# neka-nat/probreg

Hardware: NVIDIA H100
Metric: cpd_em_iterations_per_sec (higher is better)
Workload: dtype f32

## Files before the change

probreg_b200/csrc/cpd_b200.cu:

```cuda
#include "cpd_b200.h"
#include "kernels.cuh"
#include "lowrank.cuh"
#include "gram_i8.cuh"
#include "bcpd.cuh"

#include <cub/device/device_radix_sort.cuh>
#ifdef CPD_HOST_EMU
#include "emu_nccl.h"
#include "emu_solver.h"
#endif

#include <dlfcn.h>
#include <math.h>
#include <stdarg.h>
#include <stdio.h>
#include <stdlib.h>
#include <string.h>

#include <algorithm>
#include <vector>

using namespace cpd;

static thread_local char g_err[512] = "";
static int fail(int code, const char* fmt, ...) {
    va_list ap;
    va_start(ap, fmt);
    vsnprintf(g_err, sizeof(g_err), fmt, ap);
    va_end(ap);
    return code;
}
#define CU(call)                                                                                   \
    do {                                                                                           \
        cudaError_t e_ = (call);                                                                   \
        if (e_ != cudaSuccess)                                                                     \
            return fail(CPD_ERR_CUDA, "%s failed at %s:%d: %s", #call, __FILE__, __LINE__, cudaGetErrorString(e_)); \
    } while (0)
#define KCHECK() CU(cudaGetLastError())

extern "C" const char* cpd_last_error(void) { return g_err; }
extern "C" int cpd_version(void) { return 100; }
extern "C" int cpd_device_count(void) {
    int n = 0;
    if (cudaGetDeviceCount(&n) != cudaSuccess) { cudaGetLastError(); return 0; }
    return n;
}

namespace {
typedef struct { char internal[128]; } nccl_uid;
typedef void* nccl_comm;
struct NcclApi {
    void* lib = nullptr;
    int (*GetUniqueId)(nccl_uid*) = nullptr;
    int (*CommInitRank)(nccl_comm*, int, nccl_uid, int) = nullptr;
    int (*AllReduce)(const void*, void*, size_t, int, int, nccl_comm, cudaStream_t) = nullptr;
    int (*CommDestroy)(nccl_comm) = nullptr;
    const char* (*GetErrorString)(int) = nullptr;
};
NcclApi g_nccl;
int load_nccl() {
    if (g_nccl.lib) return CPD_OK;
#ifdef CPD_HOST_EMU
    static_assert(sizeof(nccl_uid) == sizeof(emu::nccl_uid_t), "unique id layout");
    g_nccl.GetUniqueId = reinterpret_cast<int (*)(nccl_uid*)>(emu::ncclGetUniqueId);
    g_nccl.CommInitRank = reinterpret_cast<int (*)(nccl_comm*, int, nccl_uid, int)>(emu::ncclCommInitRank);
    g_nccl.AllReduce = emu::ncclAllReduce;
    g_nccl.CommDestroy = emu::ncclCommDestroy;
    g_nccl.GetErrorString = emu::ncclGetErrorString;
    g_nccl.lib = (void*)&g_nccl;
    return CPD_OK;
#endif
    const char* names[] = {"libnccl.so.2", "libnccl.so"};
    void* lib = nullptr;
    for (const char* nm : names) { lib = dlopen(nm, RTLD_NOW | RTLD_GLOBAL); if (lib) break; }
    if (!lib) return fail(CPD_ERR_NCCL, "cannot dlopen libnccl.so.2: %s", dlerror());
    g_nccl.GetUniqueId = (int (*)(nccl_uid*))dlsym(lib, "ncclGetUniqueId");
    g_nccl.CommInitRank = (int (*)(nccl_comm*, int, nccl_uid, int))dlsym(lib, "ncclCommInitRank");
    g_nccl.AllReduce = (int (*)(const void*, void*, size_t, int, int, nccl_comm, cudaStream_t))dlsym(lib, "ncclAllReduce");
    g_nccl.CommDestroy = (int (*)(nccl_comm))dlsym(lib, "ncclCommDestroy");
    g_nccl.GetErrorString = (const char* (*)(int))dlsym(lib, "ncclGetErrorString");
    if (!g_nccl.GetUniqueId || !g_nccl.CommInitRank || !g_nccl.AllReduce || !g_nccl.CommDestroy)
        return fail(CPD_ERR_NCCL, "libnccl lacks an expected symbol");
    g_nccl.lib = lib;
    return CPD_OK;
}
constexpr int NCCL_DOUBLE = 8, NCCL_SUM = 0;

struct SolverApi {
    void* lib = nullptr;
    int (*Create)(void**) = nullptr;
    int (*Destroy)(void*) = nullptr;
    int (*SetStream)(void*, cudaStream_t) = nullptr;
    int (*CreateParams)(void**) = nullptr;
    int (*DestroyParams)(void*) = nullptr;
    int (*XgetrfBuf)(void*, void*, int64_t, int64_t, int, const void*, int64_t, int, size_t*, size_t*) = nullptr;
    int (*Xgetrf)(void*, void*, int64_t, int64_t, int, void*, int64_t, int64_t*, int, void*, size_t, void*, size_t, int*) = nullptr;
    int (*Xgetrs)(void*, void*, int, int64_t, int64_t, int, const void*, int64_t, const int64_t*, int, void*, int64_t, int*) = nullptr;
};
SolverApi g_sol;
int load_cusolver() {
    if (g_sol.lib) return CPD_OK;
#ifdef CPD_HOST_EMU
    g_sol.Create = emu::solverCreate; g_sol.Destroy = emu::solverDestroy; g_sol.SetStream = emu::solverSetStream;
    g_sol.CreateParams = emu::solverCreateParams; g_sol.DestroyParams = emu::solverDestroyParams;
    g_sol.XgetrfBuf = emu::solverXgetrfBuf; g_sol.Xgetrf = emu::solverXgetrf; g_sol.Xgetrs = emu::solverXgetrs;
    g_sol.lib = (void*)&g_sol;
    return CPD_OK;
#endif
    const char* names[] = {"libcusolver.so.11", "/usr/local/cuda/lib64/libcusolver.so.11", "libcusolver.so"};
    void* lib = nullptr;
    for (const char* nm : names) { lib = dlopen(nm, RTLD_NOW | RTLD_GLOBAL); if (lib) break; }
    if (!lib) return fail(CPD_ERR_CUDA, "cannot dlopen libcusolver.so.11: %s", dlerror());
#define SOLSYM(field, name) g_sol.field = (decltype(g_sol.field))dlsym(lib, name)
    SOLSYM(Create, "cusolverDnCreate");
    SOLSYM(Destroy, "cusolverDnDestroy");
    SOLSYM(SetStream, "cusolverDnSetStream");
    SOLSYM(CreateParams, "cusolverDnCreateParams");
    SOLSYM(DestroyParams, "cusolverDnDestroyParams");
    SOLSYM(XgetrfBuf, "cusolverDnXgetrf_bufferSize");
    SOLSYM(Xgetrf, "cusolverDnXgetrf");
    SOLSYM(Xgetrs, "cusolverDnXgetrs");
#undef SOLSYM
    if (!g_sol.Create || !g_sol.SetStream || !g_sol.CreateParams || !g_sol.XgetrfBuf || !g_sol.Xgetrf || !g_sol.Xgetrs)
        return fail(CPD_ERR_CUDA, "libcusolver lacks an expected symbol");
    g_sol.lib = lib;
    return CPD_OK;
}
constexpr int CUDA_R_64F_ = 1, CUBLAS_OP_T_ = 1;
}
#define SOLV(call)                                                                          \
    do {                                                                                    \
        int r_ = (call);                                                                    \
        if (r_ != 0) return fail(CPD_ERR_CUDA, "%s failed with cusolverStatus %d", #call, r_); \
    } while (0)
#define NC(call)                                                                                                   \
    do {                                                                                                           \
        int r_ = (call);                                                                                           \
        if (r_ != 0)                                                                                               \
            return fail(CPD_ERR_NCCL, "%s failed: %s", #call, g_nccl.GetErrorString ? g_nccl.GetErrorString(r_) : "?"); \
    } while (0)

struct cpd_ctx {
    int device = 0, dim = 3, sm_count = 132, slots1 = 264, slots2 = 264;
    cudaStream_t stream = nullptr;
    bool own_stream = false;
    long long m = 0, mpad = 0, n = 0, npad = 0, n_global = 0;
    double *d_yc = nullptr, *d_ts = nullptr, *d_xc = nullptr, *d_raw = nullptr;
    size_t raw_cap = 0;
    float4 *d_srcP = nullptr, *d_srcJ = nullptr, *d_tgtP = nullptr, *d_tgtQ = nullptr;
    P1Part* d_part1 = nullptr;
    double* d_part2 = nullptr;
    size_t part1_cap = 0, part2_cap = 0;
    double *d_pt1 = nullptr, *d_p1 = nullptr, *d_pxc = nullptr, *d_px = nullptr;
    double *d_mom_src = nullptr, *d_mom_tgt = nullptr, *d_mom = nullptr, *d_sums = nullptr;
    size_t mom_src_cap = 0, mom_tgt_cap = 0, sums_cap = 0;
    DevState* d_state = nullptr;
    DevState h_state;
    double* h_pin = nullptr;
    double* d_frame = nullptr;
    double* h_stats = nullptr;
    cudaEvent_t stats_ev = nullptr, copy_ev = nullptr;
    int stats_pending = 0;
    long long stats_count[2] = {0, 0};
    bool origin_given = false;
    int it1 = 0, it2 = 0, j1 = 1, j2 = 1, g1 = 1, g2 = 1;
    float4 *d_sbox = nullptr, *d_tbox = nullptr, *d_ssub = nullptr, *d_tsub = nullptr;
    float *d_omax = nullptr, *d_omax_sub = nullptr;
    bool cull_on = true, cull_active = false;
    double extent = 0.0;
    int4 *d_work1 = nullptr, *d_work2 = nullptr;
    int *d_slots1 = nullptr, *d_slots2 = nullptr;
    bool have_source = false, have_target = false, have_state = false, prepared = false;
    nccl_comm comm = nullptr;
    int world = 1, rank = 0;
    int *d_perm_src = nullptr, *d_perm_tgt = nullptr, *d_idx_tmp = nullptr;
    unsigned *d_codes = nullptr, *d_codes_out = nullptr;
    size_t sort_cap = 0, sort_tmp_cap = 0;
    void* d_sort_tmp = nullptr;
    double *d_outN = nullptr, *d_outM = nullptr;
    float* d_G = nullptr;
    double *d_W = nullptr, *d_A = nullptr, *d_B = nullptr, *d_ts2 = nullptr, *d_nrpart = nullptr;
    int64_t* d_ipiv = nullptr;
    int* d_info = nullptr;
    void *d_work = nullptr, *h_work = nullptr, *sol = nullptr, *sol_params = nullptr;
    size_t work_dev = 0, work_host = 0;
    long long nr_m = 0;
    double nr_lmd = 0.0;
    bool nr_ready = false;
    float* d_la = nullptr;
    double *d_la64 = nullptr, *d_la_part = nullptr, *d_bc_es = nullptr;
    size_t la_cap = 0;
    double* d_log2c = nullptr;
    bool wgt_on = false;
    BcpdState* d_bc = nullptr;
    float* d_bc_ginv = nullptr;
    double *d_bc_A = nullptr, *d_bc_S = nullptr, *d_bc_v = nullptr, *d_bc_r = nullptr, *d_bc_alpha = nullptr, *d_bc_sdiag = nullptr,
           *d_bc_part = nullptr, *d_bc_sums = nullptr;
    int64_t* d_bc_ipiv = nullptr;
    int* d_bc_info = nullptr;
    long long bc_m = 0;
    size_t bc_part_cap = 0;
    double bc_sigma2 = 0.0;
    bool bc_ready = false;
    bool bc_stopped = false;
    cudaEvent_t bc_ev[6] = {nullptr, nullptr, nullptr, nullptr, nullptr, nullptr};
    float bc_ms[5] = {0.f, 0.f, 0.f, 0.f, 0.f};
    double *d_wgt = nullptr, *d_p1t = nullptr, *d_pxt = nullptr;
    long long prior_m = 0;
    double prior_alpha = 1.0;
    bool prior_on = false;
    int lr_rank = 0;
    bool lr_w_stale = false;
    float lr_setup_ms[3] = {0.f, 0.f, 0.f};
    long long lr_m = 0;
    int lr_cap = 0;
    float4* d_lr_pts = nullptr;
    double *d_lr_Q = nullptr, *d_lr_X = nullptr, *d_lr_coef = nullptr, *d_lr_part = nullptr, *d_lr_Bc = nullptr, *d_lr_S = nullptr,
           *d_lr_R = nullptr, *d_lr_sys = nullptr, *d_lr_rhs = nullptr, *d_lr_c = nullptr, *d_lr_out = nullptr, *d_lr_panel = nullptr, *d_lr_Lt = nullptr;
    bool lr_spd = true;
    size_t lr_part_cap = 0;
    unsigned char* d_gi_planes = nullptr;
    double *d_gi_part = nullptr, *d_gi_colmax = nullptr;
    size_t gi_planes_cap = 0, gi_part_cap = 0, gi_colmax_cap = 0;
    size_t lr_out_cap = 0;
    P2PMailbox* d_box = nullptr;
    P2PInfo* d_p2p = nullptr;
    void* peer_ptr[P2P_MAX] = {nullptr};
    cudaEvent_t ev0 = nullptr, ev1 = nullptr, sev[7] = {nullptr, nullptr, nullptr, nullptr, nullptr, nullptr, nullptr};
    bool profiling = false;
    int64_t launches = 0;
    DevState* h_state_ring = nullptr;
    cudaEvent_t state_ev[8] = {nullptr, nullptr, nullptr, nullptr, nullptr, nullptr, nullptr, nullptr};
    int state_slot = 0;
    bool graph_on = true;
    cudaGraphExec_t em_graph = nullptr;
    int em_graph_key = -1, em_graph_launches = 0, prepare_gen = 0;
    void* d_flush = nullptr;
    size_t flush_cap = 0;
    std::vector<cudaEvent_t> pool;
};

namespace {
constexpr int STATE_RING = 8;
template <typename T>
int dev_alloc(T** p, size_t count) {
    if (*p) { cudaFree(*p); *p = nullptr; }
    cudaError_t e = cudaMalloc((void**)p, std::max<size_t>(count, 1) * sizeof(T));
    if (e != cudaSuccess) return fail(CPD_ERR_CUDA, "cudaMalloc(%zu bytes) failed: %s", count * sizeof(T), cudaGetErrorString(e));
    return CPD_OK;
}
#define TRY(x) do { int r__ = (x); if (r__ != CPD_OK) return r__; } while (0)
template <typename T>
struct DevBuf {
    T* p = nullptr;
    ~DevBuf() { if (p) cudaFree(p); }
    int alloc(size_t count) { return dev_alloc(&p, count); }
};

inline unsigned blocks_for(long long n) { return (unsigned)((n + THREADS - 1) / THREADS); }

struct WorkList {
    std::vector<int4> items;
    std::vector<int> tile_slots;
    int max_slots = 1;
};
WorkList build_work(int ntiles, int nunits, int slots, double last_cost, double overhead) {
    const double OVERHEAD = overhead;
    WorkList w;
    nunits = std::max(1, nunits);
    auto cost_of = [&](int t) { return t == ntiles - 1 ? last_cost : 1.0; };
    auto span_of = [&](int t, int j) { return cost_of(t) * (double)((nunits + j - 1) / j) + OVERHEAD; };
    int best_j = 1;
    double best = 1e300;
    for (int j = 1; j <= nunits; ++j) {
        const long long items = (long long)ntiles * j;
        const double waves = ceil((double)items / slots);
        const double span = waves * ((double)((nunits + j - 1) / j) + OVERHEAD);
        if (span < best - 1e-9) { best = span; best_j = j; }
        if (items > 8LL * slots) break;
    }
    w.tile_slots.assign(ntiles, best_j);
    if (ntiles <= slots) {
        std::vector<int> cuts(ntiles, 1);
        int used = ntiles;
        while (used < slots) {
            int worst = -1;
            double wv = -1.0;
            for (int t = 0; t < ntiles; ++t) {
                const double v = span_of(t, cuts[t]);
                if (cuts[t] < nunits && v > wv) { wv = v; worst = t; }
            }
            if (worst < 0) break;
            ++cuts[worst];
            ++used;
        }
        double span = 0.0;
        for (int t = 0; t < ntiles; ++t) span = std::max(span, span_of(t, cuts[t]));
        if (span <= best + 1e-9) w.tile_slots = cuts;
    }
    for (int t = 0; t < ntiles; ++t) {
        const int j = w.tile_slots[t];
        for (int s = 0; s < j; ++s) {
            const int a = (int)((long long)nunits * s / j), b = (int)((long long)nunits * (s + 1) / j);
            w.items.push_back(make_int4(t, a, b, s));
        }
        w.max_slots = std::max(w.max_slots, j);
    }
    std::stable_sort(w.items.begin(), w.items.end(), [&](const int4& a, const int4& b) {
        return cost_of(a.x) * (a.z - a.y) > cost_of(b.x) * (b.z - b.y);
    });
    return w;
}

int ensure_stats(cpd_ctx* h);
int upload_state(cpd_ctx* h) {
    TRY(ensure_stats(h));
    if (!h->h_state_ring) {
        CU(cudaMallocHost((void**)&h->h_state_ring, STATE_RING * sizeof(DevState)));
        for (int k = 0; k < STATE_RING; ++k) CU(cudaEventCreateWithFlags(&h->state_ev[k], cudaEventDisableTiming));
    }
    const int k = h->state_slot;
    h->state_slot = (k + 1) % STATE_RING;
    CU(cudaEventSynchronize(h->state_ev[k]));
    h->h_state_ring[k] = h->h_state;
    CU(cudaMemcpyAsync(h->d_state, &h->h_state_ring[k], sizeof(DevState), cudaMemcpyHostToDevice, h->stream));
    CU(cudaEventRecord(h->state_ev[k], h->stream));
    return CPD_OK;
}

int upload_cloud(cpd_ctx* h, const double* src, long long count, double* dst3) {
    if (h->dim == 3) {
        CU(cudaMemcpyAsync(dst3, src, (size_t)count * 3 * sizeof(double), cudaMemcpyHostToDevice, h->stream));
    } else {
        CU(cudaMemsetAsync(dst3, 0, (size_t)count * 3 * sizeof(double), h->stream));
        CU(cudaMemcpy2DAsync(dst3, 3 * sizeof(double), src, 2 * sizeof(double), 2 * sizeof(double), (size_t)count,
                             cudaMemcpyHostToDevice, h->stream));
    }
    return CPD_OK;
}
int download_cloud(cpd_ctx* h, const double* src3, long long count, double* dst) {
    if (h->dim == 3) {
        CU(cudaMemcpyAsync(dst, src3, (size_t)count * 3 * sizeof(double), cudaMemcpyDeviceToHost, h->stream));
    } else {
        CU(cudaMemcpy2DAsync(dst, 2 * sizeof(double), src3, 3 * sizeof(double), 2 * sizeof(double), (size_t)count,
                             cudaMemcpyDeviceToHost, h->stream));
    }
    return CPD_OK;
}

int cloud_sums_dev(cpd_ctx* h, const double* d_pts, long long count, double* part, double* d_out) {
    const unsigned nb = blocks_for(count);
    cloud_sums_kernel<<<nb, THREADS, 0, h->stream>>>(d_pts, count, part);
    reduce_cols_kernel<<<1, 4 * 32, 0, h->stream>>>(part, (int)nb, 4, d_out);
    KCHECK();
    h->launches += 2;
    return CPD_OK;
}

int ingest_cloud(cpd_ctx* h, const double* host_pts, long long count, int is_target, long long n_global, const double* origin,
                 int* d_perm, double* d_out) {
    if (h->raw_cap < (size_t)count * 3) { TRY(dev_alloc(&h->d_raw, (size_t)count * 3)); h->raw_cap = (size_t)count * 3; }
    const unsigned nb = blocks_for(count);
    if (h->sums_cap < (size_t)nb * 9 + 16) {
        TRY(dev_alloc(&h->d_sums, (size_t)nb * 9 + 16));
        h->sums_cap = (size_t)nb * 9 + 16;
    }
    if (h->sort_cap < (size_t)count) {
        TRY(dev_alloc(&h->d_codes, (size_t)count));
        TRY(dev_alloc(&h->d_codes_out, (size_t)count));
        TRY(dev_alloc(&h->d_idx_tmp, (size_t)count));
        h->sort_cap = (size_t)count;
    }
    size_t need = 0;
    CU(cub::DeviceRadixSort::SortPairs(nullptr, need, h->d_codes, h->d_codes_out, h->d_idx_tmp, d_perm, (int)count, 0, 30, h->stream));
    if (need > h->sort_tmp_cap) {
        if (h->d_sort_tmp) cudaFree(h->d_sort_tmp);
        h->d_sort_tmp = nullptr;
        CU(cudaMalloc(&h->d_sort_tmp, need));
        h->sort_tmp_cap = need;
    }
    TRY(upload_cloud(h, host_pts, count, h->d_raw));
    CU(cudaEventRecord(h->copy_ev, h->stream));
    double* frame = h->d_frame + 8 * is_target;
    stats_kernel<<<nb, THREADS, 0, h->stream>>>(h->d_raw, count, h->d_sums + 16);
    stats_fold_kernel<<<1, 288, 0, h->stream>>>(h->d_sums + 16, (int)nb, h->d_sums);
    cloud_frame_kernel<<<1, 32, 0, h->stream>>>(h->d_sums, count, is_target, n_global, origin != nullptr, origin ? origin[0] : 0.0,
                                                origin ? origin[1] : 0.0, origin ? origin[2] : 0.0, h->d_state, frame);
    CU(cudaMemcpyAsync(h->h_stats + 9 * is_target, h->d_sums, 9 * sizeof(double), cudaMemcpyDeviceToHost, h->stream));
    CU(cudaEventRecord(h->stats_ev, h->stream));
    h->stats_pending |= 1 << is_target;
    h->stats_count[is_target] = count;
    morton_frame_kernel<<<nb, THREADS, 0, h->stream>>>(h->d_raw, count, frame, h->d_codes, h->d_idx_tmp);
    CU(cub::DeviceRadixSort::SortPairs(h->d_sort_tmp, need, h->d_codes, h->d_codes_out, h->d_idx_tmp, d_perm, (int)count, 0, 30,
                                       h->stream));
    gather3_frame_kernel<<<nb, THREADS, 0, h->stream>>>(h->d_raw, d_perm, count, frame, d_out);
    KCHECK();
    h->launches += 6;
    CU(cudaEventSynchronize(h->copy_ev));
    return CPD_OK;
}

int ensure_stats(cpd_ctx* h) {
    if (!h->stats_pending) return CPD_OK;
    CU(cudaEventSynchronize(h->stats_ev));
    if (h->stats_pending & 1)
        for (int a = 0; a < 3; ++a) h->h_state.cy[a] = h->h_stats[a] / (double)h->stats_count[0];
    if (h->stats_pending & 2) {
        const double* t = h->h_stats + 9;
        if (!h->origin_given) for (int a = 0; a < 3; ++a) h->h_state.cx[a] = t[a] / (double)h->stats_count[1];
        h->extent = std::max(t[6] - t[3], std::max(t[7] - t[4], t[8] - t[5]));
    }
    h->stats_pending = 0;
    return CPD_OK;
}

int prepare(cpd_ctx* h) {
    TRY(ensure_stats(h));
    if (h->prepared) return CPD_OK;
    if (!h->have_source || !h->have_target) return fail(CPD_ERR_STATE, "source and target must both be set");
    h->it1 = (int)((h->n + ITILE1 - 1) / ITILE1);
    h->it2 = (int)((h->m + ITILE2 - 1) / ITILE2);
    const long long in_last = h->n - (long long)(h->it1 - 1) * ITILE1;
    const int live = (int)((in_last + 32 * RI1 - 1) / (32 * RI1));
    double last_cost = live < THREADS / 32 ? std::max(0.6, live / (double)(THREADS / 32)) : 1.0;
    if (const char* e = getenv("CPD_B200_PLAN_LAST_COST")) { const double v = atof(e); if (v > 0.0 && v <= 1.0) last_cost = v; }
    WorkList w1;
    if (const char* e = getenv("CPD_B200_PLAN_UNIT"); e && !strcmp(e, "stage")) {
        w1 = build_work(h->it1, (int)(h->mpad / P1_STAGE), h->slots1, last_cost, 0.5);
        for (int4& it : w1.items) { it.y *= P1_STAGE / SUB; it.z *= P1_STAGE / SUB; }
    } else {
        w1 = build_work(h->it1, (int)(h->mpad / SUB), h->slots1, last_cost, 0.5 * (P1_STAGE / SUB));
    }
    const WorkList w2 = build_work(h->it2, (int)(h->npad / P2_STAGE), h->slots2, 1.0, 0.5);
    h->j1 = w1.max_slots; h->g1 = (int)w1.items.size();
    h->j2 = w2.max_slots; h->g2 = (int)w2.items.size();
    TRY(dev_alloc(&h->d_work1, w1.items.size()));
    TRY(dev_alloc(&h->d_work2, w2.items.size()));
    TRY(dev_alloc(&h->d_slots1, w1.tile_slots.size()));
    TRY(dev_alloc(&h->d_slots2, w2.tile_slots.size()));
    CU(cudaMemcpyAsync(h->d_work1, w1.items.data(), w1.items.size() * sizeof(int4), cudaMemcpyHostToDevice, h->stream));
    CU(cudaMemcpyAsync(h->d_work2, w2.items.data(), w2.items.size() * sizeof(int4), cudaMemcpyHostToDevice, h->stream));
    CU(cudaMemcpyAsync(h->d_slots1, w1.tile_slots.data(), w1.tile_slots.size() * sizeof(int), cudaMemcpyHostToDevice, h->stream));
    CU(cudaMemcpyAsync(h->d_slots2, w2.tile_slots.data(), w2.tile_slots.size() * sizeof(int), cudaMemcpyHostToDevice, h->stream));
    CU(cudaStreamSynchronize(h->stream));
    TRY(dev_alloc(&h->d_sbox, (size_t)(h->mpad / P1_STAGE) * 2));
    TRY(dev_alloc(&h->d_tbox, (size_t)(h->npad / P2_STAGE) * 2));
    TRY(dev_alloc(&h->d_omax, (size_t)(h->npad / P2_STAGE)));
    TRY(dev_alloc(&h->d_ssub, (size_t)(h->mpad / SUB) * 2));
    TRY(dev_alloc(&h->d_tsub, (size_t)(h->npad / SUB) * 2));
    TRY(dev_alloc(&h->d_omax_sub, (size_t)(h->npad / SUB)));
    const size_t need1 = (size_t)h->j1 * h->n, need2 = (size_t)h->j2 * h->m * 4;
    if (need1 > h->part1_cap) { TRY(dev_alloc(&h->d_part1, need1)); h->part1_cap = need1; }
    if (need2 > h->part2_cap) { TRY(dev_alloc(&h->d_part2, need2)); h->part2_cap = need2; }
    const size_t ms = (size_t)blocks_for(h->m) * MOM_SRC, mt = (size_t)blocks_for(h->npad) * MOM_TGT;
    if (ms > h->mom_src_cap) { TRY(dev_alloc(&h->d_mom_src, ms)); h->mom_src_cap = ms; }
    if (mt > h->mom_tgt_cap) { TRY(dev_alloc(&h->d_mom_tgt, mt)); h->mom_tgt_cap = mt; }
    h->prepared = true;
    h->prepare_gen += 1;
    return CPD_OK;
}

int allreduce(cpd_ctx* h, double* buf, size_t count) {
    if (!h->comm) return CPD_OK;
    NC(g_nccl.AllReduce(buf, buf, count, NCCL_DOUBLE, NCCL_SUM, h->comm, h->stream));
    return CPD_OK;
}

inline void mark(cpd_ctx* h, int k) {
    if (h->profiling) cudaEventRecord(h->sev[k], h->stream);
}

int launch_estep(cpd_ctx* h, const double* d_sigma2, const double* d_w, const double* d_ts) {
    TRY(prepare(h));
    const long long cover = std::max(h->mpad, h->n);
    mark(h, 0);
    pack_kernel<<<blocks_for(cover), THREADS, 0, h->stream>>>(h->d_state, d_sigma2, h->d_yc, d_ts, h->d_xc, h->m, h->mpad,
                                                              h->n, h->d_srcP, h->d_srcJ, h->d_tgtP);
    mark(h, 1);
    const bool cull = h->cull_on && h->cull_active;
    const int nst1 = (int)(h->mpad / P1_STAGE);
    stage_bbox_kernel<<<(unsigned)nst1, THREADS, 0, h->stream>>>(h->d_srcP, (int)h->m, P1_STAGE, h->d_sbox);
    h->launches += 1;
    const int nsub1 = (int)(h->mpad / SUB), nsub2 = (int)(h->npad / SUB);
    if (cull) {
        stage_bbox_kernel<<<(unsigned)(h->npad / P2_STAGE), THREADS, 0, h->stream>>>(h->d_tgtP, (int)h->n, P2_STAGE, h->d_tbox);
        sub_bbox_kernel<<<(unsigned)((nsub1 + 7) / 8), THREADS, 0, h->stream>>>(h->d_srcP, (int)h->m, nsub1, h->d_ssub);
        sub_bbox_kernel<<<(unsigned)((nsub2 + 7) / 8), THREADS, 0, h->stream>>>(h->d_tgtP, (int)h->n, nsub2, h->d_tsub);
        h->launches += 3;
    }
    const bool wgt = h->wgt_on;
    if (wgt) {
        weight_patch_kernel<<<blocks_for(h->m), THREADS, 0, h->stream>>>(h->d_la, h->m, h->d_srcP, h->d_srcJ);
        h->launches += 1;
    }
#define CPD_PASS1(C, W) pass1_kernel<C, W><<<h->g1, THREADS, PASS1_SMEM, h->stream>>>(h->d_tgtP, (int)h->n, h->d_srcJ, h->d_work1, h->d_part1, h->d_sbox, nst1, (C) ? h->d_ssub : nullptr)
    if (cull) { if (wgt) CPD_PASS1(true, true); else CPD_PASS1(true, false); }
    else { if (wgt) CPD_PASS1(false, true); else CPD_PASS1(false, false); }
#undef CPD_PASS1
    mark(h, 2);
    finalize1_kernel<<<blocks_for(h->npad), THREADS, 0, h->stream>>>(h->d_state, d_sigma2, d_w, h->d_part1, h->d_slots1, (int)h->n,
                                                                     h->d_tgtP, h->d_tgtQ, h->npad, h->d_pt1, h->d_mom_tgt,
                                                                     wgt ? h->d_log2c : nullptr);
    mark(h, 3);
    if (cull) {
        stage_omax_kernel<<<(unsigned)(h->npad / P2_STAGE), THREADS, 0, h->stream>>>(h->d_tgtQ, h->d_omax);
        sub_omax_kernel<<<(unsigned)((nsub2 + 7) / 8), THREADS, 0, h->stream>>>(h->d_tgtQ, nsub2, h->d_omax_sub);
        h->launches += 2;
    }
#define CPD_PASS2(C, W) pass2_kernel<C, W><<<h->g2, THREADS, PASS2_SMEM, h->stream>>>(h->d_srcP, (int)h->m, h->d_tgtQ, h->d_work2, h->d_part2, (C) ? h->d_tbox : nullptr, (C) ? h->d_omax : nullptr, (C) ? h->d_tsub : nullptr, (C) ? h->d_omax_sub : nullptr)
    if (cull) { if (wgt) CPD_PASS2(true, true); else CPD_PASS2(true, false); }
    else { if (wgt) CPD_PASS2(false, true); else CPD_PASS2(false, false); }
#undef CPD_PASS2
    mark(h, 4);
    finalize2_kernel<<<blocks_for(h->m), THREADS, 0, h->stream>>>(h->d_state, d_sigma2, h->d_part2, h->d_slots2, (int)h->m, h->d_yc,
                                                                  d_ts, h->d_p1, h->d_pxc, h->d_mom_src);
    mark(h, 5);
    mark(h, 6);
    KCHECK();
    h->launches += 5;
    return CPD_OK;
}

int read_params(cpd_ctx* h, cpd_params* out) {
    static_assert(sizeof(DevState) <= 48 * sizeof(double), "DevState outgrew the pinned staging buffer");
    CU(cudaMemcpyAsync(h->h_pin, h->d_state, sizeof(DevState), cudaMemcpyDeviceToHost, h->stream));
    CU(cudaStreamSynchronize(h->stream));
    if (reinterpret_cast<const DevState*>(h->h_pin)->err)
        return fail(CPD_ERR_STATE, "a peer rank did not deliver its moments within the P2P exchange timeout");
    const int d = h->dim;
    for (int i = 0; i < 9; ++i) out->lin[i] = 0.0;
    for (int i = 0; i < d; ++i)
        for (int j = 0; j < d; ++j) out->lin[i * d + j] = h->h_pin[3 * i + j];
    for (int i = 0; i < 3; ++i) out->t[i] = (i < d) ? h->h_pin[9 + i] : 0.0;
    out->scale = h->h_pin[12];
    out->sigma2 = h->h_pin[13];
    TRY(ensure_stats(h));
    h->cull_active = h->extent > 0.0 && 13.3 * sqrt(out->sigma2) < 0.25 * h->extent;
    out->q = h->h_pin[14];
    out->n_p = h->h_pin[15];
    return CPD_OK;
}
}

extern "C" int cpd_plan_work(int ntiles, int nunits, int slots, double last_tile_cost, int* items ,
                             int capacity, int* n_items, int* max_slots) {
    if (ntiles < 1 || nunits < 1 || slots < 1 || !(last_tile_cost > 0.0 && last_tile_cost <= 1.0) || !n_items || !max_slots)
        return fail(CPD_ERR_ARG, "bad argument");
    const WorkList w = build_work(ntiles, nunits, slots, last_tile_cost, 0.5 * (P1_STAGE / SUB));
    *n_items = (int)w.items.size();
    *max_slots = w.max_slots;
    if (items) {
        if (capacity < (int)w.items.size()) return fail(CPD_ERR_ARG, "capacity %d < %d work items", capacity, (int)w.items.size());
        for (size_t i = 0; i < w.items.size(); ++i) {
            items[4 * i] = w.items[i].x; items[4 * i + 1] = w.items[i].y; items[4 * i + 2] = w.items[i].z; items[4 * i + 3] = w.items[i].w;
        }
    }
    return CPD_OK;
}

extern "C" int cpd_create(cpd_ctx** out, int device, int dim, void* stream) {
    if (!out) return fail(CPD_ERR_ARG, "out is NULL");
    if (dim != 2 && dim != 3) return fail(CPD_ERR_ARG, "dim must be 2 or 3, got %d", dim);
    int ndev = 0;
    if (cudaGetDeviceCount(&ndev) != cudaSuccess || ndev == 0) {
        cudaGetLastError();
        return fail(CPD_ERR_CUDA, "no CUDA device: this library has no CPU path");
    }
    if (device < 0 || device >= ndev) return fail(CPD_ERR_ARG, "device %d out of range (%d visible)", device, ndev);
    CU(cudaSetDevice(device));
    cudaDeviceProp prop;
    CU(cudaGetDeviceProperties(&prop, device));
    if (prop.major != 9 || prop.minor != 0)
        return fail(CPD_ERR_CUDA, "device %d is sm_%d%d; this library is built for sm_90a (Hopper) only", device, prop.major, prop.minor);
    cpd_ctx* h = new cpd_ctx();
    h->device = device;
    h->dim = dim;
    h->sm_count = prop.multiProcessorCount;
    if (stream) { h->stream = (cudaStream_t)stream; h->own_stream = false; }
    else { CU(cudaStreamCreateWithFlags(&h->stream, cudaStreamNonBlocking)); h->own_stream = true; }
    CU(cudaFuncSetAttribute(pass1_kernel<false, false>, cudaFuncAttributeMaxDynamicSharedMemorySize, PASS1_SMEM));
    CU(cudaFuncSetAttribute(pass2_kernel<false, false>, cudaFuncAttributeMaxDynamicSharedMemorySize, PASS2_SMEM));
    CU(cudaFuncSetAttribute(pass1_kernel<true, false>, cudaFuncAttributeMaxDynamicSharedMemorySize, PASS1_SMEM));
    CU(cudaFuncSetAttribute(pass2_kernel<true, false>, cudaFuncAttributeMaxDynamicSharedMemorySize, PASS2_SMEM));
    CU(cudaFuncSetAttribute(pass1_kernel<false, true>, cudaFuncAttributeMaxDynamicSharedMemorySize, PASS1_SMEM));
    CU(cudaFuncSetAttribute(pass2_kernel<false, true>, cudaFuncAttributeMaxDynamicSharedMemorySize, PASS2_SMEM));
    CU(cudaFuncSetAttribute(pass1_kernel<true, true>, cudaFuncAttributeMaxDynamicSharedMemorySize, PASS1_SMEM));
    CU(cudaFuncSetAttribute(pass2_kernel<true, true>, cudaFuncAttributeMaxDynamicSharedMemorySize, PASS2_SMEM));
    int occ1 = 0, occ2 = 0;
    CU(cudaOccupancyMaxActiveBlocksPerMultiprocessor(&occ1, pass1_kernel<false, false>, THREADS, PASS1_SMEM));
    CU(cudaOccupancyMaxActiveBlocksPerMultiprocessor(&occ2, pass2_kernel<false, false>, THREADS, PASS2_SMEM));
    h->slots1 = h->sm_count * std::max(1, occ1);
    h->slots2 = h->sm_count * std::max(1, occ2);
    TRY(dev_alloc(&h->d_state, 1));
    TRY(dev_alloc(&h->d_mom, (size_t)MOM_PAD));
    CU(cudaMallocHost((void**)&h->h_pin, 64 * sizeof(double)));
    TRY(dev_alloc(&h->d_frame, 16));
    CU(cudaMallocHost((void**)&h->h_stats, 18 * sizeof(double)));
    CU(cudaEventCreateWithFlags(&h->stats_ev, cudaEventDisableTiming));
    CU(cudaEventCreateWithFlags(&h->copy_ev, cudaEventDisableTiming));
    CU(cudaEventCreate(&h->ev0));
    CU(cudaEventCreate(&h->ev1));
    for (int k = 0; k < 7; ++k) CU(cudaEventCreate(&h->sev[k]));
    { const char* e = getenv("CPD_B200_NO_CULL"); h->cull_on = !(e && e[0] == '1'); }
    { const char* e = getenv("CPD_B200_NO_GRAPH"); h->graph_on = !(e && e[0] == '1'); }
    memset(&h->h_state, 0, sizeof(DevState));
    h->h_state.dim = dim;
    h->h_state.scale = 1.0;
    h->h_state.lin[0] = h->h_state.lin[4] = h->h_state.lin[8] = 1.0;
    h->h_state.update_scale = 1;
    *out = h;
    return upload_state(h);
}

extern "C" void cpd_destroy(cpd_ctx* h) {
    if (!h) return;
    cudaSetDevice(h->device);
    cudaStreamSynchronize(h->stream);
    void* wl[] = {h->d_work1, h->d_work2, h->d_slots1, h->d_slots2, h->d_sbox, h->d_tbox, h->d_omax, h->d_ssub, h->d_tsub, h->d_omax_sub};
    for (void* p : wl) if (p) cudaFree(p);
    void* srt[] = {h->d_perm_src, h->d_perm_tgt, h->d_idx_tmp, h->d_codes, h->d_codes_out, h->d_sort_tmp, h->d_outN, h->d_outM};
    for (void* p : srt) if (p) cudaFree(p);
    void* nrp[] = {h->d_G, h->d_W, h->d_A, h->d_B, h->d_ts2, h->d_nrpart, h->d_ipiv, h->d_info, h->d_work};
    for (void* p : nrp) if (p) cudaFree(p);
    void* lrp[] = {h->d_lr_pts, h->d_lr_Q, h->d_lr_X, h->d_lr_coef, h->d_lr_part, h->d_lr_Bc, h->d_lr_S, h->d_lr_R, h->d_lr_sys, h->d_lr_rhs,
                   h->d_lr_c, h->d_lr_out, h->d_lr_panel, h->d_lr_Lt, h->d_gi_planes, h->d_gi_part, h->d_gi_colmax, h->d_wgt, h->d_p1t, h->d_pxt, h->d_la, h->d_log2c,
                   h->d_la64, h->d_la_part, h->d_bc_es};
    for (void* p : lrp) if (p) cudaFree(p);
    void* bcp[] = {h->d_bc, h->d_bc_ginv, h->d_bc_A, h->d_bc_S, h->d_bc_v, h->d_bc_r, h->d_bc_alpha, h->d_bc_sdiag, h->d_bc_part, h->d_bc_sums,
                   h->d_bc_ipiv, h->d_bc_info};
    for (void* p : bcp) if (p) cudaFree(p);
    for (cudaEvent_t e : h->bc_ev) if (e) cudaEventDestroy(e);
    if (h->h_work) free(h->h_work);
    if (h->sol_params && g_sol.DestroyParams) g_sol.DestroyParams(h->sol_params);
    if (h->sol && g_sol.Destroy) g_sol.Destroy(h->sol);
    for (int r = 0; r < P2P_MAX; ++r) if (h->peer_ptr[r]) cudaIpcCloseMemHandle(h->peer_ptr[r]);
    if (h->d_box) cudaFree(h->d_box);
    if (h->d_p2p) cudaFree(h->d_p2p);
    void* ptrs[] = {h->d_yc, h->d_ts, h->d_xc, h->d_raw, h->d_srcP, h->d_srcJ, h->d_tgtP, h->d_tgtQ, h->d_part1, h->d_part2, h->d_pt1, h->d_p1,
                    h->d_pxc, h->d_px, h->d_mom_src, h->d_mom_tgt, h->d_mom, h->d_sums, h->d_state, h->d_flush};
    for (void* p : ptrs) if (p) cudaFree(p);
    if (h->h_pin) cudaFreeHost(h->h_pin);
    if (h->h_stats) cudaFreeHost(h->h_stats);
    if (h->d_frame) cudaFree(h->d_frame);
    if (h->stats_ev) cudaEventDestroy(h->stats_ev);
    if (h->copy_ev) cudaEventDestroy(h->copy_ev);
#ifndef CPD_HOST_EMU
    if (h->em_graph) cudaGraphExecDestroy(h->em_graph);
#endif
    if (h->h_state_ring) cudaFreeHost(h->h_state_ring);
    for (int k = 0; k < 8; ++k) if (h->state_ev[k]) cudaEventDestroy(h->state_ev[k]);
    if (h->ev0) cudaEventDestroy(h->ev0);
    if (h->ev1) cudaEventDestroy(h->ev1);
    for (int k = 0; k < 7; ++k) if (h->sev[k]) cudaEventDestroy(h->sev[k]);
    for (cudaEvent_t e : h->pool) if (e) cudaEventDestroy(e);
    if (h->own_stream) cudaStreamDestroy(h->stream);
    delete h;
}

extern "C" int cpd_set_source(cpd_ctx* h, const double* source, int64_t m) {
    if (!h || !source) return fail(CPD_ERR_ARG, "null argument");
    if (m < 1 || m > 0x7fffffffLL - 65536) return fail(CPD_ERR_ARG, "source count %lld out of range", (long long)m);
    CU(cudaSetDevice(h->device));
    if (m != h->m || !h->d_yc) {
        h->m = m;
        h->mpad = (m + P1_STAGE - 1) / P1_STAGE * P1_STAGE;
        TRY(dev_alloc(&h->d_yc, (size_t)m * 3));
        TRY(dev_alloc(&h->d_ts, (size_t)m * 3));
        TRY(dev_alloc(&h->d_srcP, (size_t)h->mpad));
        TRY(dev_alloc(&h->d_srcJ, (size_t)h->mpad * 2));
        TRY(dev_alloc(&h->d_p1, (size_t)m));
        TRY(dev_alloc(&h->d_pxc, (size_t)m * 3));
        TRY(dev_alloc(&h->d_px, (size_t)m * 3));
        TRY(dev_alloc(&h->d_perm_src, (size_t)m));
        TRY(dev_alloc(&h->d_outM, (size_t)m * 3));
        h->prepared = false;
        h->nr_ready = false;
    }
    TRY(ingest_cloud(h, source, m, 0, 0, nullptr, h->d_perm_src, h->d_yc));
    h->bc_ready = false;
    h->bc_stopped = false;
    h->h_state.m = m;
    h->have_source = true;
    return CPD_OK;
}

extern "C" int cpd_set_target(cpd_ctx* h, const double* target, int64_t n_local, int64_t n_global, const double* frame_origin) {
    if (!h || !target) return fail(CPD_ERR_ARG, "null argument");
    if (n_local < 1 || n_local > 0x7fffffffLL - 65536) return fail(CPD_ERR_ARG, "target count %lld out of range", (long long)n_local);
    if (n_global < n_local) return fail(CPD_ERR_ARG, "n_global (%lld) < n_local (%lld)", (long long)n_global, (long long)n_local);
    if (!frame_origin && n_global != n_local) return fail(CPD_ERR_ARG, "a sharded target needs an explicit frame_origin");
    CU(cudaSetDevice(h->device));
    if (n_local != h->n || !h->d_xc) {
        h->n = n_local;
        h->npad = (n_local + P2_STAGE - 1) / P2_STAGE * P2_STAGE;
        TRY(dev_alloc(&h->d_xc, (size_t)n_local * 3));
        TRY(dev_alloc(&h->d_tgtP, (size_t)n_local));
        TRY(dev_alloc(&h->d_tgtQ, (size_t)h->npad * 3));
        TRY(dev_alloc(&h->d_pt1, (size_t)n_local));
        TRY(dev_alloc(&h->d_perm_tgt, (size_t)n_local));
        TRY(dev_alloc(&h->d_outN, (size_t)n_local));
        h->prepared = false;
    }
    h->n_global = n_global;
    double origin[3] = {0.0, 0.0, 0.0};
    if (frame_origin) for (int a = 0; a < h->dim; ++a) origin[a] = frame_origin[a];
    h->origin_given = frame_origin != nullptr;
    if (h->origin_given) for (int a = 0; a < 3; ++a) h->h_state.cx[a] = origin[a];
    TRY(ingest_cloud(h, target, n_local, 1, n_global, frame_origin ? origin : nullptr, h->d_perm_tgt, h->d_xc));
    h->h_state.n_global = n_global;
    h->have_target = true;
    return CPD_OK;
}

extern "C" int cpd_sigma2_init(cpd_ctx* h, double* sigma2) {
    if (!h || !sigma2) return fail(CPD_ERR_ARG, "null argument");
    if (!h->have_source || !h->have_target) return fail(CPD_ERR_STATE, "source and target must both be set");
    CU(cudaSetDevice(h->device));
    double sx[4], sy[4];
    const size_t pn = (size_t)blocks_for(h->n) * 4, pm = (size_t)blocks_for(h->m) * 4;
    if (h->sums_cap < 16 + pn + pm) { TRY(dev_alloc(&h->d_sums, 16 + pn + pm)); h->sums_cap = 16 + pn + pm; }
    TRY(cloud_sums_dev(h, h->d_xc, h->n, h->d_sums + 16, h->d_sums));
    if (h->comm) TRY(allreduce(h, h->d_sums, 4));
    TRY(cloud_sums_dev(h, h->d_yc, h->m, h->d_sums + 16 + pn, h->d_sums + 4));
    CU(cudaMemcpyAsync(h->h_pin, h->d_sums, 8 * sizeof(double), cudaMemcpyDeviceToHost, h->stream));
    CU(cudaStreamSynchronize(h->stream));
    TRY(ensure_stats(h));
    for (int k = 0; k < 4; ++k) { sx[k] = h->h_pin[k]; sy[k] = h->h_pin[4 + k]; }
    double dlt[3], d2 = 0.0, dsy = 0.0;
    for (int a = 0; a < 3; ++a) { dlt[a] = h->h_state.cy[a] - h->h_state.cx[a]; d2 += dlt[a] * dlt[a]; dsy += dlt[a] * sy[1 + a]; }
    const double M = (double)h->m, N = (double)h->n_global;
    const double syy = sy[0] + 2.0 * dsy + M * d2;
    double cross = 0.0;
    for (int a = 0; a < 3; ++a) cross += sx[1 + a] * (sy[1 + a] + M * dlt[a]);
    *sigma2 = (M * sx[0] + N * syy - 2.0 * cross) / (M * N * h->dim);
    return CPD_OK;
}

extern "C" int cpd_set_state(cpd_ctx* h, int tf_kind, int update_scale, double w, const cpd_params* init) {
    if (!h || !init) return fail(CPD_ERR_ARG, "null argument");
    if (tf_kind != CPD_TF_RIGID && tf_kind != CPD_TF_AFFINE) return fail(CPD_ERR_ARG, "tf_kind %d not supported by the fused EM loop", tf_kind);
    if (!(w >= 0.0 && w < 1.0)) return fail(CPD_ERR_ARG, "w must be in [0, 1), got %g", w);
    if (!(init->sigma2 > 0.0)) return fail(CPD_ERR_ARG, "sigma2 must be positive, got %g", init->sigma2);
    CU(cudaSetDevice(h->device));
    DevState& s = h->h_state;
    const int d = h->dim;
    for (int i = 0; i < 3; ++i)
        for (int j = 0; j < 3; ++j) s.lin[3 * i + j] = (i < d && j < d) ? init->lin[i * d + j] : (i == j ? 1.0 : 0.0);
    for (int i = 0; i < 3; ++i) s.t[i] = (i < d) ? init->t[i] : 0.0;
    s.scale = (tf_kind == CPD_TF_RIGID) ? init->scale : 1.0;
    s.sigma2 = init->sigma2;
    s.q = init->q;
    s.n_p = 0.0;
    s.w = w;
    s.tf_kind = tf_kind;
    s.update_scale = update_scale ? 1 : 0;
    s.dim = d;
    TRY(ensure_stats(h));
    h->cull_active = h->extent > 0.0 && 13.3 * sqrt(init->sigma2) < 0.25 * h->extent;
    h->have_state = true;
    return upload_state(h);
}

namespace {
int em_step_launches(cpd_ctx* h) {
    TRY(launch_estep(h, &h->d_state->sigma2, &h->d_state->w, nullptr));
    const int nbs = (int)blocks_for(h->m), nbt = (int)blocks_for(h->npad);
    if (h->d_p2p) {
        moments_p2p_kernel<<<1, 256, 0, h->stream>>>(h->d_state, h->d_mom_src, nbs, RM_SRC, h->d_mom_tgt, nbt, RM_TGT, h->d_mom,
                                                     h->d_p2p);
        h->launches += 1;
    } else if (h->comm) {
        moments_kernel<0><<<1, 256, 0, h->stream>>>(h->d_state, h->d_mom_src, nbs, RM_SRC, h->d_mom_tgt, nbt, RM_TGT, h->d_mom);
        TRY(allreduce(h, h->d_mom, MOM_PAD));
        mstep_residual_kernel<<<1, 32, 0, h->stream>>>(h->d_state, h->d_mom);
        h->launches += 2;
    } else {
        moments_kernel<1><<<1, 256, 0, h->stream>>>(h->d_state, h->d_mom_src, nbs, RM_SRC, h->d_mom_tgt, nbt, RM_TGT, h->d_mom);
        h->launches += 1;
    }
    mark(h, 6);
    KCHECK();
    return CPD_OK;
}
}

extern "C" int cpd_em_step(cpd_ctx* h, cpd_params* out) {
    if (!h) return fail(CPD_ERR_ARG, "null handle");
    if (!h->have_state) return fail(CPD_ERR_STATE, "cpd_set_state has not been called");
    CU(cudaSetDevice(h->device));
#ifndef CPD_HOST_EMU
    const bool use_graph = h->graph_on && !h->profiling && !(h->comm && !h->d_p2p) && !h->wgt_on;
#else
    const bool use_graph = false;
#endif
    if (!use_graph) {
        TRY(em_step_launches(h));
    }
#ifndef CPD_HOST_EMU
    else {
        TRY(prepare(h));
        const int key = h->prepare_gen * 2 + ((h->cull_on && h->cull_active) ? 1 : 0);
        if (!h->em_graph || h->em_graph_key != key) {
            if (h->em_graph) { cudaGraphExecDestroy(h->em_graph); h->em_graph = nullptr; }
            const int64_t before = h->launches;
            cudaGraph_t g = nullptr;
            CU(cudaStreamBeginCapture(h->stream, cudaStreamCaptureModeThreadLocal));
            const int rc = em_step_launches(h);
            const cudaError_t ce = cudaStreamEndCapture(h->stream, &g);
            h->em_graph_launches = (int)(h->launches - before);
            h->launches = before;
            if (rc != CPD_OK) { if (g) cudaGraphDestroy(g); return rc; }
            if (ce != cudaSuccess) return fail(CPD_ERR_CUDA, "cudaStreamEndCapture failed: %s", cudaGetErrorString(ce));
            const cudaError_t ie = cudaGraphInstantiate(&h->em_graph, g, 0);
            cudaGraphDestroy(g);
            if (ie != cudaSuccess) { h->em_graph = nullptr; return fail(CPD_ERR_CUDA, "cudaGraphInstantiate failed: %s", cudaGetErrorString(ie)); }
            h->em_graph_key = key;
        }
        CU(cudaGraphLaunch(h->em_graph, h->stream));
        h->launches += h->em_graph_launches;
    }
#endif
    if (out) return read_params(h, out);
    return CPD_OK;
}

extern "C" int cpd_em_run(cpd_ctx* h, int maxiter, double tol, cpd_params* out, int* iters_run, double* trace) {
    if (!h || !out) return fail(CPD_ERR_ARG, "null argument");
    if (!h->have_state) return fail(CPD_ERR_STATE, "cpd_set_state has not been called");
    double q = h->h_state.q;
    int it = 0;
    cpd_params cur;
    memset(&cur, 0, sizeof(cur));
    for (it = 0; it < maxiter; ++it) {
        TRY(cpd_em_step(h, &cur));
        if (trace) { trace[2 * it] = cur.sigma2; trace[2 * it + 1] = cur.q; }
        if (fabs(cur.q - q) < tol) { ++it; break; }
        q = cur.q;
    }
    if (maxiter <= 0) TRY(read_params(h, &cur));
    *out = cur;
    if (iters_run) *iters_run = it;
    return CPD_OK;
}

extern "C" int cpd_estep(cpd_ctx* h, const double* t_source, double sigma2, double w, double* pt1, double* p1, double* px, double* n_p) {
    if (!h || !t_source) return fail(CPD_ERR_ARG, "null argument");
    if (!(sigma2 > 0.0)) return fail(CPD_ERR_ARG, "sigma2 must be positive, got %g", sigma2);
    if (!(w >= 0.0 && w < 1.0)) return fail(CPD_ERR_ARG, "w must be in [0, 1), got %g", w);
    if (!h->have_source || !h->have_target) return fail(CPD_ERR_STATE, "source and target must both be set");
    CU(cudaSetDevice(h->device));
    if (h->raw_cap < (size_t)h->m * 3) { TRY(dev_alloc(&h->d_raw, (size_t)h->m * 3)); h->raw_cap = (size_t)h->m * 3; }
    TRY(upload_cloud(h, t_source, h->m, h->d_raw));
    gather3_kernel<<<blocks_for(h->m), THREADS, 0, h->stream>>>(h->d_raw, h->d_perm_src, h->m, 0.0, 0.0, 0.0, h->d_ts);
    h->launches += 1;
    TRY(ensure_stats(h));
    h->cull_active = h->extent > 0.0 && 13.3 * sqrt(sigma2) < 0.25 * h->extent;
    h->h_pin[32] = sigma2;
    h->h_pin[33] = w;
    CU(cudaMemcpyAsync(&h->d_state->es_sigma2, h->h_pin + 32, 2 * sizeof(double), cudaMemcpyHostToDevice, h->stream));
    TRY(launch_estep(h, &h->d_state->es_sigma2, &h->d_state->es_w, h->d_ts));
    if (h->comm) {
        TRY(allreduce(h, h->d_p1, (size_t)h->m));
        TRY(allreduce(h, h->d_pxc, (size_t)h->m * 3));
    }
    return cpd_last_estep(h, pt1, p1, px, n_p);
}

namespace {
int bcpd_weights(cpd_ctx* h, const double* alpha, const double* sdiag, const int* perm, const double* ssw) {
    const long long m = h->m;
    const unsigned nb = blocks_for(m);
    bcpd_la_kernel<<<nb, THREADS, 0, h->stream>>>(alpha, sdiag, m, ssw, h->dim, h->d_la64, h->d_la_part);
    bcpd_la_finish_kernel<<<1, 32, 0, h->stream>>>(h->d_la_part, (int)nb, ssw, h->dim, h->n_global, h->d_log2c);
    bcpd_la_apply_kernel<<<nb, THREADS, 0, h->stream>>>(h->d_la64, perm, m, h->d_log2c, h->d_la);
    KCHECK();
    h->launches += 3;
    return CPD_OK;
}
int ensure_weight_buffers(cpd_ctx* h) {
    const long long m = h->m;
    if (h->la_cap < (size_t)m) {
        TRY(dev_alloc(&h->d_la, (size_t)m));
        TRY(dev_alloc(&h->d_la64, (size_t)m));
        TRY(dev_alloc(&h->d_la_part, (size_t)blocks_for(m)));
        h->la_cap = (size_t)m;
    }
    if (!h->d_log2c) TRY(dev_alloc(&h->d_log2c, 3));
    if (!h->d_bc_es) TRY(dev_alloc(&h->d_bc_es, 3));
    return CPD_OK;
}
}

extern "C" int cpd_bcpd_estep(cpd_ctx* h, const double* t_source, double scale, const double* alpha, const double* sigma_diag,
                              double sigma2, double w, double* nu_d, double* nu, double* px, double* n_p) {
    if (!h || !t_source || !alpha || !sigma_diag) return fail(CPD_ERR_ARG, "null argument");
    if (!(sigma2 > 0.0)) return fail(CPD_ERR_ARG, "sigma2 must be positive, got %g", sigma2);
    if (!(w >= 0.0 && w < 1.0)) return fail(CPD_ERR_ARG, "w must be in [0, 1), got %g", w);
    if (!h->have_source || !h->have_target) return fail(CPD_ERR_STATE, "source and target must both be set");
    CU(cudaSetDevice(h->device));
    const long long m = h->m;
    bool any_weight = false;
    for (long long i = 0; i < m; ++i) {
        if (!(alpha[i] >= 0.0) || !(sigma_diag[i] >= 0.0)) return fail(CPD_ERR_ARG, "alpha and diag(sigma_mat) must be non-negative");
        any_weight = any_weight || (alpha[i] > 0.0 && sigma_diag[i] < INFINITY);
    }
    if (!any_weight) return fail(CPD_ERR_ARG, "every source has zero weight");
    TRY(ensure_weight_buffers(h));
    h->h_pin[44] = scale;
    h->h_pin[45] = sigma2;
    h->h_pin[46] = w;
    CU(cudaMemcpyAsync(h->d_bc_es, h->h_pin + 44, 3 * sizeof(double), cudaMemcpyHostToDevice, h->stream));
    CU(cudaMemcpyAsync(h->d_outM, alpha, (size_t)m * sizeof(double), cudaMemcpyHostToDevice, h->stream));
    CU(cudaMemcpyAsync(h->d_outM + m, sigma_diag, (size_t)m * sizeof(double), cudaMemcpyHostToDevice, h->stream));
    TRY(bcpd_weights(h, h->d_outM, h->d_outM + m, h->d_perm_src, h->d_bc_es));
    if (h->raw_cap < (size_t)m * 3) { TRY(dev_alloc(&h->d_raw, (size_t)m * 3)); h->raw_cap = (size_t)m * 3; }
    TRY(upload_cloud(h, t_source, m, h->d_raw));
    gather3_kernel<<<blocks_for(m), THREADS, 0, h->stream>>>(h->d_raw, h->d_perm_src, m, 0.0, 0.0, 0.0, h->d_ts);
    h->launches += 1;
    TRY(ensure_stats(h));
    h->cull_active = h->extent > 0.0 && 13.3 * sqrt(sigma2) < 0.25 * h->extent;
    h->h_pin[32] = sigma2;
    h->h_pin[33] = w;
    CU(cudaMemcpyAsync(&h->d_state->es_sigma2, h->h_pin + 32, 2 * sizeof(double), cudaMemcpyHostToDevice, h->stream));
    h->wgt_on = true;
    const int r = launch_estep(h, &h->d_state->es_sigma2, &h->d_state->es_w, h->d_ts);
    h->wgt_on = false;
    TRY(r);
    if (h->comm) {
        TRY(allreduce(h, h->d_p1, (size_t)m));
        TRY(allreduce(h, h->d_pxc, (size_t)m * 3));
    }
    return cpd_last_estep(h, nu_d, nu, px, n_p);
}

extern "C" int cpd_last_estep(cpd_ctx* h, double* pt1, double* p1, double* px, double* n_p) {
    if (!h) return fail(CPD_ERR_ARG, "null handle");
    if (!h->prepared) return fail(CPD_ERR_STATE, "no E-step has run on this handle");
    CU(cudaSetDevice(h->device));
    if (pt1) {
        scatter_kernel<<<blocks_for(h->n), THREADS, 0, h->stream>>>(h->d_pt1, h->d_perm_tgt, h->n, 1, h->d_outN);
        CU(cudaMemcpyAsync(pt1, h->d_outN, (size_t)h->n * sizeof(double), cudaMemcpyDeviceToHost, h->stream));
        h->launches += 1;
    }
    if (p1) {
        scatter_kernel<<<blocks_for(h->m), THREADS, 0, h->stream>>>(h->d_p1, h->d_perm_src, h->m, 1, h->d_outM);
        CU(cudaMemcpyAsync(p1, h->d_outM, (size_t)h->m * sizeof(double), cudaMemcpyDeviceToHost, h->stream));
        CU(cudaStreamSynchronize(h->stream));
        h->launches += 1;
    }
    if (px) {
        uncentre_px_kernel<<<blocks_for(h->m), THREADS, 0, h->stream>>>(h->d_state, h->d_p1, h->d_pxc, (int)h->m, h->d_px);
        scatter_kernel<<<blocks_for(h->m), THREADS, 0, h->stream>>>(h->d_px, h->d_perm_src, h->m, 3, h->d_outM);
        KCHECK();
        h->launches += 2;
        TRY(download_cloud(h, h->d_outM, h->m, px));
    }
    if (n_p) {
        const unsigned nb = blocks_for(h->m);
        if (h->sums_cap < (size_t)nb * 4 + 4) { TRY(dev_alloc(&h->d_sums, (size_t)nb * 4 + 4)); h->sums_cap = (size_t)nb * 4 + 4; }
        src_moments_api_kernel<<<nb, THREADS, 0, h->stream>>>((int)h->m, h->d_yc, h->d_p1, h->d_pxc, h->d_mom_src);
        reduce_cols_kernel<<<1, MOM_SRC * 32, 0, h->stream>>>(h->d_mom_src, (int)nb, MOM_SRC, h->d_mom);
        KCHECK();
        h->launches += 2;
        CU(cudaMemcpyAsync(h->h_pin + 40, h->d_mom, sizeof(double), cudaMemcpyDeviceToHost, h->stream));
    }
    CU(cudaStreamSynchronize(h->stream));
    if (n_p) *n_p = h->h_pin[40];
    return CPD_OK;
}

extern "C" int cpd_mstep(cpd_ctx* h, int tf_kind, int update_scale, const double* pt1, const double* p1, const double* px, double n_p,
                         cpd_params* out) {
    (void)n_p;
    if (!h || !pt1 || !p1 || !px || !out) return fail(CPD_ERR_ARG, "null argument");
    if (tf_kind != CPD_TF_RIGID && tf_kind != CPD_TF_AFFINE) return fail(CPD_ERR_ARG, "tf_kind %d not supported", tf_kind);
    if (!h->have_source || !h->have_target) return fail(CPD_ERR_STATE, "source and target must both be set");
    CU(cudaSetDevice(h->device));
    TRY(prepare(h));
    h->h_state.tf_kind = tf_kind;
    h->h_state.update_scale = update_scale ? 1 : 0;
    CU(cudaMemcpyAsync(&h->d_state->tf_kind, &h->h_state.tf_kind, 2 * sizeof(int), cudaMemcpyHostToDevice, h->stream));
    CU(cudaMemcpyAsync(h->d_outN, pt1, (size_t)h->n * sizeof(double), cudaMemcpyHostToDevice, h->stream));
    gather1_kernel<<<blocks_for(h->n), THREADS, 0, h->stream>>>(h->d_outN, h->d_perm_tgt, h->n, h->d_pt1);
    CU(cudaMemcpyAsync(h->d_outM, p1, (size_t)h->m * sizeof(double), cudaMemcpyHostToDevice, h->stream));
    gather1_kernel<<<blocks_for(h->m), THREADS, 0, h->stream>>>(h->d_outM, h->d_perm_src, h->m, h->d_p1);
    if (h->raw_cap < (size_t)h->m * 3) { TRY(dev_alloc(&h->d_raw, (size_t)h->m * 3)); h->raw_cap = (size_t)h->m * 3; }
    TRY(upload_cloud(h, px, h->m, h->d_raw));
    gather3_kernel<<<blocks_for(h->m), THREADS, 0, h->stream>>>(h->d_raw, h->d_perm_src, h->m, 0.0, 0.0, 0.0, h->d_px);
    h->launches += 3;
    const int nbs = (int)blocks_for(h->m), nbt = (int)blocks_for(h->n);
    centre_px_kernel<<<nbs, THREADS, 0, h->stream>>>(h->d_state, h->d_p1, h->d_px, (int)h->m, h->d_pxc);
    src_moments_api_kernel<<<nbs, THREADS, 0, h->stream>>>((int)h->m, h->d_yc, h->d_p1, h->d_pxc, h->d_mom_src);
    tgt_moments_api_kernel<<<nbt, THREADS, 0, h->stream>>>(h->d_pt1, h->d_xc, (int)h->n, h->d_mom_tgt);
    moments_kernel<0><<<1, 256, 0, h->stream>>>(h->d_state, h->d_mom_src, nbs, MOM_SRC, h->d_mom_tgt, nbt, MOM_TGT, h->d_mom);
    KCHECK();
    if (h->comm) TRY(allreduce(h, h->d_mom + MOM_SRC, MOM_TGT));
    mstep_api_kernel<<<1, 32, 0, h->stream>>>(h->d_state, h->d_mom);
    KCHECK();
    h->launches += 5;
    return read_params(h, out);
}

#include "host_nonrigid.inl"
#include "host_bcpd.inl"
#include "host_stateless.inl"
#include "host_multi.inl"
#include "host_measure.inl"
```

probreg_b200/csrc/kernels.cuh:

```cuda
#pragma once
#include <cuda_runtime.h>
#include <stdint.h>

namespace cpd {

#ifndef CPD_RI1
#define CPD_RI1 4
#endif
#ifndef CPD_RI2
#define CPD_RI2 4
#endif
#ifndef CPD_MINB1
#define CPD_MINB1 2
#endif
#ifndef CPD_MINB2
#define CPD_MINB2 2
#endif
#ifndef CPD_UNROLL1
#define CPD_UNROLL1 4
#endif
#ifndef CPD_UNROLL2
#define CPD_UNROLL2 4
#endif
#ifndef CPD_SUB
#define CPD_SUB 64
#endif
#ifndef CPD_GRP
#define CPD_GRP 8
#endif
constexpr int UNROLL1 = CPD_UNROLL1, UNROLL2 = CPD_UNROLL2;
constexpr int THREADS = 256;
constexpr int RI1 = CPD_RI1, RI2 = CPD_RI2;
constexpr int ITILE1 = THREADS * RI1, ITILE2 = THREADS * RI2;
constexpr int NPAIR1 = RI1 / 2, NPAIR2 = RI2 / 2;
#ifndef CPD_P1_STAGE
#define CPD_P1_STAGE 512
#endif
#ifndef CPD_P2_STAGE
#define CPD_P2_STAGE 512
#endif
constexpr int P1_STAGE = CPD_P1_STAGE;
constexpr int P2_STAGE = CPD_P2_STAGE;
static_assert(P1_STAGE % 256 == 0 && P2_STAGE % 256 == 0 && P1_STAGE >= 256 && P2_STAGE >= 256, "stage sizes are multiples of 256");
constexpr int P1_REC = 32, P2_REC = 48;
#ifndef CPD_NSTAGE
#define CPD_NSTAGE 3
#endif
constexpr int NSTAGE = CPD_NSTAGE;
constexpr int P1_STAGE_BYTES = P1_STAGE * P1_REC, P2_STAGE_BYTES = P2_STAGE * P2_REC;
constexpr int SUB = CPD_SUB;
constexpr int GRP = CPD_GRP;
constexpr int PASS1_SMEM = NSTAGE * P1_STAGE_BYTES + 64, PASS2_SMEM = NSTAGE * P2_STAGE_BYTES + 64;

#ifdef CPD_HOST_EMU
#define CPD_DYN_SMEM(name) unsigned char* const name = emu::g_dyn_smem
#else
#define CPD_DYN_SMEM(name) extern __shared__ __align__(128) unsigned char name[]
#endif

constexpr float O_INIT = 1048576.0f;
constexpr float TWO100 = 1.2676506002282294e30f;
constexpr float FAR_COORD = 1.0e18f;

constexpr double LOG2E = 1.4426950408889634074;
constexpr double DEAD_LOG2 = -1075.0;
constexpr double EPS32 = 1.1920928955078125e-07;

enum { RM_NP = 0, RM_SY = 1, RM_C = 4, RM_V1 = 10, RM_VY = 13, RM_SRC = 22, RM_SRR = 22, RM_NPT = 23, RM_TGT = 2,
       RM_COUNT = 24, MOM_PAD = 32 };
enum { MOM_NP = 0, MOM_SX = 1, MOM_SY = 4, MOM_B = 7, MOM_C = 16, MOM_NPT = 22, MOM_SXT = 23, MOM_TXX = 26,
       MOM_COUNT = 27, MOM_SRC = 22, MOM_TGT = 5 };

struct P1Part {
    double S;
    double SU;
    float o;
    float pad;
};

struct DevState {
    double lin[9];
    double t[3];
    double scale;
    double sigma2;
    double q;
    double n_p;
    double cx[3];
    double cy[3];
    double w;
    double es_sigma2;
    double es_w;
    long long m;
    long long n_global;
    int tf_kind;
    int update_scale;
    int dim;
    int err;
};

constexpr int P2P_MAX = 16;
struct P2PMailbox {
    double slots[2][P2P_MAX][MOM_PAD];
    unsigned long long flags[2][P2P_MAX];
};
struct P2PInfo {
    P2PMailbox* box[P2P_MAX];
    int world, rank;
    unsigned long long seq;
    unsigned long long timeout_ns;
};

#ifdef CPD_HOST_EMU
}
#include "emu_device.h"
namespace cpd {
#else
__device__ __forceinline__ float ex2(float x) {
    float y;
    asm("ex2.approx.ftz.f32 %0, %1;" : "=f"(y) : "f"(x));
    return y;
}
typedef unsigned long long u64;
__device__ __forceinline__ u64 pack2(float lo, float hi) { u64 r; asm("mov.b64 %0, {%1, %2};" : "=l"(r) : "f"(lo), "f"(hi)); return r; }
__device__ __forceinline__ float2 unpack2(u64 v) { float2 r; asm("mov.b64 {%0, %1}, %2;" : "=f"(r.x), "=f"(r.y) : "l"(v)); return r; }
__device__ __forceinline__ u64 fsub2(u64 a, u64 b) {
    const float2 x = unpack2(a), y = unpack2(b);
    return pack2(__fsub_rn(x.x, y.x), __fsub_rn(x.y, y.y));
}
__device__ __forceinline__ u64 fadd2(u64 a, u64 b) {
    const float2 x = unpack2(a), y = unpack2(b);
    return pack2(__fadd_rn(x.x, y.x), __fadd_rn(x.y, y.y));
}
__device__ __forceinline__ u64 fmul2(u64 a, u64 b) {
    const float2 x = unpack2(a), y = unpack2(b);
    return pack2(__fmul_rn(x.x, y.x), __fmul_rn(x.y, y.y));
}
__device__ __forceinline__ u64 ffma2(u64 a, u64 b, u64 c) {
    const float2 x = unpack2(a), y = unpack2(b), z = unpack2(c);
    return pack2(__fmaf_rn(x.x, y.x, z.x), __fmaf_rn(x.y, y.y, z.y));
}
__device__ __forceinline__ unsigned long long globaltimer_ns() {
    unsigned long long t;
    asm volatile("mov.u64 %0, %%globaltimer;" : "=l"(t));
    return t;
}
__device__ __forceinline__ uint32_t smem_u32(const void* p) { return (uint32_t)__cvta_generic_to_shared(p); }
__device__ __forceinline__ void mbar_init(uint64_t* bar, uint32_t count) {
    asm volatile("mbarrier.init.shared::cta.b64 [%0], %1;" ::"r"(smem_u32(bar)), "r"(count));
}
__device__ __forceinline__ void mbar_fence_init() { asm volatile("fence.mbarrier_init.release.cluster;" ::: "memory"); }
__device__ __forceinline__ void mbar_expect_tx(uint64_t* bar, uint32_t bytes) {
    asm volatile("mbarrier.arrive.expect_tx.shared::cta.b64 _, [%0], %1;" ::"r"(smem_u32(bar)), "r"(bytes) : "memory");
}
__device__ __forceinline__ void tma_load_1d(void* dst, const void* src, uint32_t bytes, uint64_t* bar) {
    asm volatile("cp.async.bulk.shared::cluster.global.mbarrier::complete_tx::bytes [%0], [%1], %2, [%3];" ::"r"(
                     smem_u32(dst)),
                 "l"(src), "r"(bytes), "r"(smem_u32(bar))
                 : "memory");
}
__device__ __forceinline__ void mbar_wait(uint64_t* bar, uint32_t parity) {
    asm volatile(
        "{\n"
        ".reg .pred P1;\n"
        "LAB_WAIT:\n"
        "mbarrier.try_wait.parity.shared::cta.b64 P1, [%0], %1;\n"
        "@P1 bra DONE;\n"
        "bra LAB_WAIT;\n"
        "DONE:\n"
        "}" ::"r"(smem_u32(bar)),
        "r"(parity)
        : "memory");
}
#endif
__device__ __forceinline__ double warp_sum(double v) {
#pragma unroll
    for (int o = 16; o > 0; o >>= 1) v += __shfl_xor_sync(0xffffffffu, v, o);
    return v;
}
template <int K>
__device__ __forceinline__ void block_reduce_store(double (&v)[K], double* out) {
    __shared__ double sh[K][THREADS / 32];
    const int lane = threadIdx.x & 31, wid = threadIdx.x >> 5;
#pragma unroll
    for (int k = 0; k < K; ++k) {
        double s = warp_sum(v[k]);
        if (lane == 0) sh[k][wid] = s;
    }
    __syncthreads();
    if (threadIdx.x < K) {
        double s = 0.0;
#pragma unroll
        for (int w = 0; w < THREADS / 32; ++w) s += sh[threadIdx.x][w];
        out[threadIdx.x] = s;
    }
}

__global__ void __launch_bounds__(THREADS)
pack_kernel(const DevState* __restrict__ st, const double* __restrict__ sigma2_ptr,
            const double* __restrict__ yc , const double* __restrict__ ts ,
            const double* __restrict__ xc , long long m, long long mpad, long long n,
            float4* __restrict__ srcP , float4* __restrict__ srcJ ,
            float4* __restrict__ tgtP ) {
    const long long i = (long long)blockIdx.x * THREADS + threadIdx.x;
    const double sk = sqrt(LOG2E / (2.0 * *sigma2_ptr));
    if (i < mpad) {
        float4 o;
        if (i < m) {
            double px, py, pz;
            if (ts != nullptr) {
                px = ts[3 * i + 0] - st->cx[0];
                py = ts[3 * i + 1] - st->cx[1];
                pz = ts[3 * i + 2] - st->cx[2];
            } else {
                const double s = (st->tf_kind == 0) ? st->scale : 1.0;
                double l[9], tp[3];
#pragma unroll
                for (int k = 0; k < 9; ++k) l[k] = s * st->lin[k];
#pragma unroll
                for (int a = 0; a < 3; ++a)
                    tp[a] = l[3 * a] * st->cy[0] + l[3 * a + 1] * st->cy[1] + l[3 * a + 2] * st->cy[2] + st->t[a] - st->cx[a];
                const double y0 = yc[3 * i], y1 = yc[3 * i + 1], y2 = yc[3 * i + 2];
                px = l[0] * y0 + l[1] * y1 + l[2] * y2 + tp[0];
                py = l[3] * y0 + l[4] * y1 + l[5] * y2 + tp[1];
                pz = l[6] * y0 + l[7] * y1 + l[8] * y2 + tp[2];
            }
            o = make_float4((float)(sk * px), (float)(sk * py), (float)(sk * pz), 0.0f);
        } else {
            o = make_float4(FAR_COORD, FAR_COORD, FAR_COORD, 0.0f);
        }
        srcP[i] = o;
        srcJ[2 * i] = make_float4(o.x, o.x, o.y, o.y);
        srcJ[2 * i + 1] = make_float4(o.z, o.z, 0.0f, 0.0f);
    }
    if (i < n) {
        tgtP[i] = make_float4((float)(sk * xc[3 * i]), (float)(sk * xc[3 * i + 1]), (float)(sk * xc[3 * i + 2]), 0.0f);
    }
}

__global__ void __launch_bounds__(THREADS)
weight_patch_kernel(const float* __restrict__ la, long long m, float4* __restrict__ srcP, float4* __restrict__ srcJ) {
    const long long i = (long long)blockIdx.x * THREADS + threadIdx.x;
    if (i < m) {
        const float v = la[i];
        srcP[i].w = v;
        float4 r = srcJ[2 * i + 1];
        r.z = v; r.w = v;
        srcJ[2 * i + 1] = r;
    }
}

constexpr float CULL_GAP = 130.0f;
__global__ void __launch_bounds__(THREADS)
stage_bbox_kernel(const float4* __restrict__ pts, int n, int blk, float4* __restrict__ box) {
    __shared__ float sh[6][THREADS / 32];
    const int b = blockIdx.x;
    float lo[3] = {3.0e38f, 3.0e38f, 3.0e38f}, hi[3] = {-3.0e38f, -3.0e38f, -3.0e38f};
    for (int i = b * blk + threadIdx.x; i < min(n, (b + 1) * blk); i += THREADS) {
        const float4 p = pts[i];
        lo[0] = fminf(lo[0], p.x); lo[1] = fminf(lo[1], p.y); lo[2] = fminf(lo[2], p.z);
        hi[0] = fmaxf(hi[0], p.x); hi[1] = fmaxf(hi[1], p.y); hi[2] = fmaxf(hi[2], p.z);
    }
    const int lane = threadIdx.x & 31, wid = threadIdx.x >> 5;
#pragma unroll
    for (int a = 0; a < 3; ++a) {
#pragma unroll
        for (int o = 16; o > 0; o >>= 1) {
            lo[a] = fminf(lo[a], __shfl_xor_sync(0xffffffffu, lo[a], o));
            hi[a] = fmaxf(hi[a], __shfl_xor_sync(0xffffffffu, hi[a], o));
        }
        if (lane == 0) { sh[a][wid] = lo[a]; sh[3 + a][wid] = hi[a]; }
    }
    __syncthreads();
    if (threadIdx.x == 0) {
        float l[3], h[3];
        for (int a = 0; a < 3; ++a) {
            l[a] = sh[a][0]; h[a] = sh[3 + a][0];
            for (int w = 1; w < THREADS / 32; ++w) { l[a] = fminf(l[a], sh[a][w]); h[a] = fmaxf(h[a], sh[3 + a][w]); }
        }
        box[2 * b] = make_float4(l[0], l[1], l[2], 0.f);
        box[2 * b + 1] = make_float4(h[0], h[1], h[2], 0.f);
    }
}
__global__ void __launch_bounds__(THREADS)
stage_omax_kernel(const float4* __restrict__ tgtQ, float* __restrict__ omax) {
    __shared__ float sh[THREADS / 32];
    const int b = blockIdx.x;
    float m = 3.0e38f;
    for (int i = threadIdx.x; i < P2_STAGE; i += THREADS) m = fminf(m, tgtQ[3 * ((size_t)b * P2_STAGE + i) + 1].z);
#pragma unroll
    for (int o = 16; o > 0; o >>= 1) m = fminf(m, __shfl_xor_sync(0xffffffffu, m, o));
    if ((threadIdx.x & 31) == 0) sh[threadIdx.x >> 5] = m;
    __syncthreads();
    if (threadIdx.x == 0) {
        for (int w = 1; w < THREADS / 32; ++w) m = fminf(m, sh[w]);
        omax[b] = -m;
    }
}
__global__ void __launch_bounds__(THREADS)
sub_bbox_kernel(const float4* __restrict__ pts, int n, int nsub, float4* __restrict__ box) {
    const int b = blockIdx.x * (THREADS / 32) + (threadIdx.x >> 5), lane = threadIdx.x & 31;
    if (b >= nsub) return;
    float lo[3] = {3.0e38f, 3.0e38f, 3.0e38f}, hi[3] = {-3.0e38f, -3.0e38f, -3.0e38f};
    for (int i = b * SUB + lane; i < min(n, (b + 1) * SUB); i += 32) {
        const float4 p = pts[i];
        lo[0] = fminf(lo[0], p.x); lo[1] = fminf(lo[1], p.y); lo[2] = fminf(lo[2], p.z);
        hi[0] = fmaxf(hi[0], p.x); hi[1] = fmaxf(hi[1], p.y); hi[2] = fmaxf(hi[2], p.z);
    }
#pragma unroll
    for (int a = 0; a < 3; ++a) {
#pragma unroll
        for (int o = 16; o > 0; o >>= 1) {
            lo[a] = fminf(lo[a], __shfl_xor_sync(0xffffffffu, lo[a], o));
            hi[a] = fmaxf(hi[a], __shfl_xor_sync(0xffffffffu, hi[a], o));
        }
    }
    if (lane == 0) {
        box[2 * b] = make_float4(lo[0], lo[1], lo[2], 0.f);
        box[2 * b + 1] = make_float4(hi[0], hi[1], hi[2], 0.f);
    }
}
__global__ void __launch_bounds__(THREADS)
sub_omax_kernel(const float4* __restrict__ tgtQ, int nsub, float* __restrict__ omax) {
    const int b = blockIdx.x * (THREADS / 32) + (threadIdx.x >> 5), lane = threadIdx.x & 31;
    if (b >= nsub) return;
    float m = 3.0e38f;
    for (int i = lane; i < SUB; i += 32) m = fminf(m, tgtQ[3 * ((size_t)b * SUB + i) + 1].z);
#pragma unroll
    for (int o = 16; o > 0; o >>= 1) m = fminf(m, __shfl_xor_sync(0xffffffffu, m, o));
    if (lane == 0) omax[b] = -m;
}
template <int NP>
__device__ __forceinline__ void warp_bbox(const u64 (&ax)[NP], const u64 (&ay)[NP], const u64 (&az)[NP], float* __restrict__ wbox) {
    float lo[3] = {3.0e38f, 3.0e38f, 3.0e38f}, hi[3] = {-3.0e38f, -3.0e38f, -3.0e38f};
#pragma unroll
    for (int p = 0; p < NP; ++p) {
        const float2 x = unpack2(ax[p]), y = unpack2(ay[p]), z = unpack2(az[p]);
        lo[0] = fminf(lo[0], fminf(x.x, x.y)); hi[0] = fmaxf(hi[0], fmaxf(x.x, x.y));
        lo[1] = fminf(lo[1], fminf(y.x, y.y)); hi[1] = fmaxf(hi[1], fmaxf(y.x, y.y));
        lo[2] = fminf(lo[2], fminf(z.x, z.y)); hi[2] = fmaxf(hi[2], fmaxf(z.x, z.y));
    }
#pragma unroll
    for (int a = 0; a < 3; ++a) {
#pragma unroll
        for (int o = 16; o > 0; o >>= 1) {
            lo[a] = fminf(lo[a], __shfl_xor_sync(0xffffffffu, lo[a], o));
            hi[a] = fmaxf(hi[a], __shfl_xor_sync(0xffffffffu, hi[a], o));
        }
    }
    if ((threadIdx.x & 31) == 0) {
#pragma unroll
        for (int a = 0; a < 3; ++a) { wbox[a] = lo[a]; wbox[3 + a] = hi[a]; }
    }
    __syncwarp();
}
__device__ __forceinline__ float box_gap2(const float* __restrict__ wbox, const float4 blo, const float4 bhi) {
    const float gx = fmaxf(0.f, fmaxf(blo.x - wbox[3], wbox[0] - bhi.x));
    const float gy = fmaxf(0.f, fmaxf(blo.y - wbox[4], wbox[1] - bhi.y));
    const float gz = fmaxf(0.f, fmaxf(blo.z - wbox[5], wbox[2] - bhi.z));
    return fmaf(gz, gz, fmaf(gy, gy, gx * gx)) * 0.9999f;
}

template <bool WGT>
__device__ __forceinline__ void pass1_sum(const ulonglong2* __restrict__ q, const u64 (&ax)[NPAIR1], const u64 (&ay)[NPAIR1],
                                          const u64 (&az)[NPAIR1], const u64 (&no)[NPAIR1], u64 (&Sc)[NPAIR1], u64 (&Uc)[NPAIR1]) {
    if (GRP > 0) {
#pragma unroll 1
        for (int g0 = 0; g0 < SUB; g0 += (GRP > 0 ? GRP : SUB)) {
            u64 gs[NPAIR1], gu[NPAIR1];
#pragma unroll
            for (int jj = 0; jj < (GRP > 0 ? GRP : 1); ++jj) {
                const ulonglong2 bxy = q[2 * (g0 + jj)];
                const u64 bz = q[2 * (g0 + jj) + 1].x;
                u64 la = 0ull;
                if (WGT) la = q[2 * (g0 + jj) + 1].y;
#pragma unroll
                for (int p = 0; p < NPAIR1; ++p) {
                    const u64 dx = fsub2(ax[p], bxy.x), dy = fsub2(ay[p], bxy.y), dz = fsub2(az[p], bz);
                    u64 t = ffma2(dx, dx, no[p]);
                    t = ffma2(dy, dy, t);
                    t = ffma2(dz, dz, t);
                    if (WGT) t = fadd2(t, la);
                    const float2 tt = unpack2(t);
                    const u64 e = pack2(ex2(-tt.x), ex2(-tt.y));
                    gs[p] = jj == 0 ? e : fadd2(gs[p], e);
                    gu[p] = jj == 0 ? fmul2(e, t) : ffma2(e, t, gu[p]);
                }
            }
#pragma unroll
            for (int p = 0; p < NPAIR1; ++p) { Sc[p] = fadd2(Sc[p], gs[p]); Uc[p] = fadd2(Uc[p], gu[p]); }
        }
    } else {
#pragma unroll UNROLL1
        for (int jj = 0; jj < SUB; ++jj) {
            const ulonglong2 bxy = q[2 * jj];
            const u64 bz = q[2 * jj + 1].x;
            u64 la = 0ull;
            if (WGT) la = q[2 * jj + 1].y;
#pragma unroll
            for (int p = 0; p < NPAIR1; ++p) {
                const u64 dx = fsub2(ax[p], bxy.x), dy = fsub2(ay[p], bxy.y), dz = fsub2(az[p], bz);
                u64 t = ffma2(dx, dx, no[p]);
                t = ffma2(dy, dy, t);
                t = ffma2(dz, dz, t);
                if (WGT) t = fadd2(t, la);
                const float2 tt = unpack2(t);
                const u64 e = pack2(ex2(-tt.x), ex2(-tt.y));
                Sc[p] = fadd2(Sc[p], e);
                Uc[p] = ffma2(e, t, Uc[p]);
            }
        }
    }
}

template <bool CULL, bool WGT>
__global__ void __launch_bounds__(THREADS, CPD_MINB1)
pass1_kernel(const float4* __restrict__ ipts, int ni, const float4* __restrict__ jrec, const int4* __restrict__ work,
             P1Part* __restrict__ part, const float4* __restrict__ sbox ,
             int nstages_total, const float4* __restrict__ ssub ) {
    __shared__ float wbox[THREADS / 32][8];
    CPD_DYN_SMEM(smraw);
    uint64_t* full = reinterpret_cast<uint64_t*>(smraw + NSTAGE * P1_STAGE_BYTES);
    const int tid = threadIdx.x;
    const int4 wk = work[blockIdx.x];
    constexpr int SPS = P1_STAGE / SUB;
    const int itile = wk.x, split = wk.w;
    const int st0 = wk.y / SPS, nst = (wk.z + SPS - 1) / SPS - st0;
    const int sc_first = wk.y - st0 * SPS, sc_last = wk.z - (st0 + nst - 1) * SPS;
    const unsigned char* jbytes = reinterpret_cast<const unsigned char*>(jrec);
    if (tid == 0) {
        for (int s = 0; s < NSTAGE; ++s) mbar_init(&full[s], 1);
        mbar_fence_init();
    }
    __syncthreads();
    if (tid == 0) {
        for (int s = 0; s < NSTAGE && s < nst; ++s) {
            mbar_expect_tx(&full[s], P1_STAGE_BYTES);
            tma_load_1d(smraw + s * P1_STAGE_BYTES, jbytes + (size_t)(st0 + s) * P1_STAGE_BYTES, P1_STAGE_BYTES, &full[s]);
        }
    }
    if (itile * ITILE1 + (tid >> 5) * (32 * RI1) >= ni) return;
    u64 ax[NPAIR1], ay[NPAIR1], az[NPAIR1], no[NPAIR1];
    double S[RI1], SU[RI1];
#pragma unroll
    for (int p = 0; p < NPAIR1; ++p) {
        int n0 = itile * ITILE1 + (tid >> 5) * (32 * RI1) + (2 * p) * 32 + (tid & 31), n1 = n0 + 32;
        n0 = n0 < ni ? n0 : ni - 1;
        n1 = n1 < ni ? n1 : ni - 1;
        const float4 p0 = ipts[n0], p1 = ipts[n1];
        ax[p] = pack2(p0.x, p1.x); ay[p] = pack2(p0.y, p1.y); az[p] = pack2(p0.z, p1.z);
        no[p] = pack2(-O_INIT, -O_INIT);
    }
    float* const mybox = wbox[tid >> 5];
    warp_bbox<NPAIR1>(ax, ay, az, mybox);
    {
        const int lane = tid & 31;
        float best = 3.0e38f;
        int bi = 0;
        for (int sidx = lane; sidx < nstages_total; sidx += 32) {
            const float g2 = box_gap2(mybox, sbox[2 * sidx], sbox[2 * sidx + 1]);
            if (g2 < best) { best = g2; bi = sidx; }
        }
#pragma unroll
        for (int o = 16; o > 0; o >>= 1) {
            const float ob = __shfl_xor_sync(0xffffffffu, best, o);
            const int oi = __shfl_xor_sync(0xffffffffu, bi, o);
            if (ob < best || (ob == best && oi < bi)) { best = ob; bi = oi; }
        }
        const ulonglong2* near = reinterpret_cast<const ulonglong2*>(jbytes + (size_t)bi * P1_STAGE_BYTES);
        float cm[RI1];
#pragma unroll
        for (int r = 0; r < RI1; ++r) cm[r] = 3.0e38f;
#pragma unroll 4
        for (int jj = 0; jj < 128; ++jj) {
            const ulonglong2 bxy = near[2 * jj];
            const u64 bz = near[2 * jj + 1].x;
            u64 la = 0ull;
            if (WGT) la = near[2 * jj + 1].y;
#pragma unroll
            for (int p = 0; p < NPAIR1; ++p) {
                const u64 dx = fsub2(ax[p], bxy.x), dy = fsub2(ay[p], bxy.y), dz = fsub2(az[p], bz);
                u64 uu = ffma2(dz, dz, ffma2(dy, dy, fmul2(dx, dx)));
                if (WGT) uu = fadd2(uu, la);
                const float2 u = unpack2(uu);
                cm[2 * p] = fminf(cm[2 * p], u.x);
                cm[2 * p + 1] = fminf(cm[2 * p + 1], u.y);
            }
        }
#pragma unroll
        for (int p = 0; p < NPAIR1; ++p)
            no[p] = pack2(-fminf(O_INIT, floorf(cm[2 * p])), -fminf(O_INIT, floorf(cm[2 * p + 1])));
    }
    float omax_w = O_INIT;
    if (CULL) {
        float om = -3.0e38f;
#pragma unroll
        for (int p = 0; p < NPAIR1; ++p) { const float2 nv = unpack2(no[p]); om = fmaxf(om, fmaxf(-nv.x, -nv.y)); }
#pragma unroll
        for (int o = 16; o > 0; o >>= 1) om = fmaxf(om, __shfl_xor_sync(0xffffffffu, om, o));
        omax_w = om;
    }
#pragma unroll
    for (int r = 0; r < RI1; ++r) { S[r] = 0.0; SU[r] = 0.0; }
    for (int it = 0; it < nst; ++it) {
        const int s = it % NSTAGE;
        mbar_wait(&full[s], (uint32_t)((it / NSTAGE) & 1));
        const ulonglong2* sp = reinterpret_cast<const ulonglong2*>(smraw + s * P1_STAGE_BYTES);
        bool skip = false;
        if (CULL) {
            const float4 blo = sbox[2 * (st0 + it)], bhi = sbox[2 * (st0 + it) + 1];
            skip = box_gap2(mybox, blo, bhi) - omax_w >= CULL_GAP;
        }
#pragma unroll 1
        for (int sc = (it == 0 ? sc_first : 0); sc < (skip ? 0 : (it == nst - 1 ? sc_last : SPS)); ++sc) {
            if (CULL) {
                const int sb = (st0 + it) * (P1_STAGE / SUB) + sc;
                if (box_gap2(mybox, ssub[2 * sb], ssub[2 * sb + 1]) - omax_w >= CULL_GAP) continue;
            }
            const ulonglong2* q = sp + sc * (2 * SUB);
            u64 Sc[NPAIR1], Uc[NPAIR1];
#pragma unroll
            for (int p = 0; p < NPAIR1; ++p) { Sc[p] = 0ull; Uc[p] = 0ull; }
            pass1_sum<WGT>(q, ax, ay, az, no, Sc, Uc);
            bool bad = false;
#pragma unroll
            for (int p = 0; p < NPAIR1; ++p) {
                const float2 v = unpack2(Sc[p]);
                bad |= !(v.x < TWO100) | !(v.y < TWO100);
            }
            if (__any_sync(0xffffffffu, bad)) {
                float cm[RI1];
#pragma unroll
                for (int r = 0; r < RI1; ++r) cm[r] = 3.0e38f;
#pragma unroll UNROLL1
                for (int jj = 0; jj < SUB; ++jj) {
                    const ulonglong2 bxy = q[2 * jj];
                    const u64 bz = q[2 * jj + 1].x;
                    u64 la = 0ull;
                    if (WGT) la = q[2 * jj + 1].y;
#pragma unroll
                    for (int p = 0; p < NPAIR1; ++p) {
                        const u64 dx = fsub2(ax[p], bxy.x), dy = fsub2(ay[p], bxy.y), dz = fsub2(az[p], bz);
                        u64 uu = ffma2(dz, dz, ffma2(dy, dy, fmul2(dx, dx)));
                        if (WGT) uu = fadd2(uu, la);
                        const float2 u = unpack2(uu);
                        cm[2 * p] = fminf(cm[2 * p], u.x);
                        cm[2 * p + 1] = fminf(cm[2 * p + 1], u.y);
                    }
                }
#pragma unroll
                for (int p = 0; p < NPAIR1; ++p) {
                    const float2 nv = unpack2(no[p]);
                    const float o0 = -nv.x, o1 = -nv.y;
                    const float on0 = fminf(o0, floorf(cm[2 * p])), on1 = fminf(o1, floorf(cm[2 * p + 1]));
                    const int sh0 = (int)fmaxf(on0 - o0, -4000.0f), sh1 = (int)fmaxf(on1 - o1, -4000.0f);
                    S[2 * p] = ldexp(S[2 * p], sh0); SU[2 * p] = ldexp(SU[2 * p], sh0);
                    S[2 * p + 1] = ldexp(S[2 * p + 1], sh1); SU[2 * p + 1] = ldexp(SU[2 * p + 1], sh1);
                    no[p] = pack2(-on0, -on1);
                    Sc[p] = 0ull; Uc[p] = 0ull;
                }
                if (CULL) {
                    float om = -3.0e38f;
#pragma unroll
                    for (int p = 0; p < NPAIR1; ++p) { const float2 nv = unpack2(no[p]); om = fmaxf(om, fmaxf(-nv.x, -nv.y)); }
#pragma unroll
                    for (int o = 16; o > 0; o >>= 1) om = fmaxf(om, __shfl_xor_sync(0xffffffffu, om, o));
                    omax_w = om;
                }
                pass1_sum<WGT>(q, ax, ay, az, no, Sc, Uc);
            }
#pragma unroll
            for (int p = 0; p < NPAIR1; ++p) {
                const float2 sv = unpack2(Sc[p]), uv = unpack2(Uc[p]), nv = unpack2(no[p]);
                S[2 * p] += (double)sv.x;
                S[2 * p + 1] += (double)sv.y;
                SU[2 * p] += (double)uv.x - (double)nv.x * (double)sv.x;
                SU[2 * p + 1] += (double)uv.y - (double)nv.y * (double)sv.y;
            }
        }
        __syncthreads();
        if (tid == 0 && it + NSTAGE < nst) {
            mbar_expect_tx(&full[s], P1_STAGE_BYTES);
            tma_load_1d(smraw + s * P1_STAGE_BYTES, jbytes + (size_t)(st0 + it + NSTAGE) * P1_STAGE_BYTES, P1_STAGE_BYTES, &full[s]);
        }
    }
#pragma unroll
    for (int p = 0; p < NPAIR1; ++p) {
        const float2 nv = unpack2(no[p]);
#pragma unroll
        for (int h = 0; h < 2; ++h) {
            const int n = itile * ITILE1 + (tid >> 5) * (32 * RI1) + (2 * p + h) * 32 + (tid & 31);
            if (n < ni) {
                P1Part out;
                out.S = S[2 * p + h]; out.SU = SU[2 * p + h]; out.o = h ? -nv.y : -nv.x; out.pad = 0.0f;
                part[(size_t)split * ni + n] = out;
            }
        }
    }
}

__global__ void __launch_bounds__(THREADS)
finalize1_kernel(const DevState* __restrict__ st, const double* __restrict__ sigma2_ptr, const double* __restrict__ w_ptr,
                 const P1Part* __restrict__ part, const int* __restrict__ tile_slots, int n, const float4* __restrict__ tgtP,
                 float4* __restrict__ tgtQ, long long npad, double* __restrict__ pt1, double* __restrict__ mom_part,
                 const double* __restrict__ log2c_ptr ) {
    const int i = blockIdx.x * THREADS + threadIdx.x;
    double v[RM_TGT] = {0.0, 0.0};
    if (i < n) {
        const int nsplit = tile_slots[i / ITILE1];
        float omin = 3.0e38f;
        for (int s = 0; s < nsplit; ++s) {
            const P1Part p = part[(size_t)s * n + i];
            if (p.S > 0.0) omin = fminf(omin, p.o);
        }
        double log2S = -INFINITY, SU = 0.0;
        if (omin < 3.0e38f) {
            double S = 0.0;
            for (int s = 0; s < nsplit; ++s) {
                const P1Part p = part[(size_t)s * n + i];
                if (p.S > 0.0) {
                    const int sh = (int)fmaxf(omin - p.o, -4000.0f);
                    S += ldexp(p.S, sh);
                    SU += ldexp(p.SU, sh);
                }
            }
            log2S = log2(S) - (double)omin;
        }
        const double sigma2 = *sigma2_ptr, w = *w_ptr;
        double c = 0.0;
        if (w > 0.0) {
            const double tps = 2.0 * 3.14159265358979323846 * sigma2;
            c = (st->dim == 3 ? tps * sqrt(tps) : tps) * (w / (1.0 - w) * (double)st->m / (double)st->n_global);
        }
        double lc = c > 0.0 ? log2(c) : -INFINITY, dead_shift = 0.0;
        if (log2c_ptr != nullptr) { lc = log2c_ptr[0]; dead_shift = log2c_ptr[1]; c = (lc > -INFINITY) ? 1.0 : 0.0; }
        const bool dead = !(log2S + dead_shift >= DEAD_LOG2);
        double L = 0.0, p1n = 0.0;
        if (!dead) {
            if (c > 0.0) {
                const double hi = fmax(log2S, lc), lo = fmin(log2S, lc);
                L = hi + log2(1.0 + exp2(lo - hi));
                p1n = exp2(log2S - L);
            } else {
                L = log2S; p1n = 1.0;
            }
        }
        pt1[i] = p1n;
        const float4 b = tgtP[i];
        float no = INFINITY, rnf = 0.0f;
        if (!dead) {
            const double rn = exp2(-(L + (double)omin));
            no = -omin;
            rnf = (float)rn;
            v[0] = SU * (double)rnf;
        }
        v[1] = p1n;
        tgtQ[3 * (size_t)i] = make_float4(b.x, b.x, b.y, b.y);
        tgtQ[3 * (size_t)i + 1] = make_float4(b.z, b.z, no, no);
        tgtQ[3 * (size_t)i + 2] = make_float4(rnf, rnf, 0.f, 0.f);
    } else if (i < npad) {
        tgtQ[3 * (size_t)i] = make_float4(0.f, 0.f, 0.f, 0.f);
        tgtQ[3 * (size_t)i + 1] = make_float4(0.f, 0.f, INFINITY, INFINITY);
        tgtQ[3 * (size_t)i + 2] = make_float4(0.f, 0.f, 0.f, 0.f);
    }
    block_reduce_store<RM_TGT>(v, mom_part + (size_t)blockIdx.x * RM_TGT);
}

template <bool CULL, bool WGT>
__global__ void __launch_bounds__(THREADS, CPD_MINB2)
pass2_kernel(const float4* __restrict__ ipts, int ni, const float4* __restrict__ jrec, const int4* __restrict__ work,
             double* __restrict__ part , const float4* __restrict__ tbox ,
             const float* __restrict__ omax_stage, const float4* __restrict__ tsub, const float* __restrict__ omax_sub) {
    __shared__ float wbox[THREADS / 32][8];
    CPD_DYN_SMEM(smraw);
    uint64_t* full = reinterpret_cast<uint64_t*>(smraw + NSTAGE * P2_STAGE_BYTES);
    const int tid = threadIdx.x;
    const int4 wk = work[blockIdx.x];
    const int itile = wk.x, st0 = wk.y, split = wk.w;
    const int nst = wk.z - wk.y;
    const unsigned char* jbytes = reinterpret_cast<const unsigned char*>(jrec);
    if (tid == 0) {
        for (int s = 0; s < NSTAGE; ++s) mbar_init(&full[s], 1);
        mbar_fence_init();
    }
    __syncthreads();
    if (tid == 0) {
        for (int s = 0; s < NSTAGE && s < nst; ++s) {
            mbar_expect_tx(&full[s], P2_STAGE_BYTES);
            tma_load_1d(smraw + s * P2_STAGE_BYTES, jbytes + (size_t)(st0 + s) * P2_STAGE_BYTES, P2_STAGE_BYTES, &full[s]);
        }
    }
    u64 ax[NPAIR2], ay[NPAIR2], az[NPAIR2], al[NPAIR2];
    double A1[RI2], AX[RI2], AY[RI2], AZ[RI2];
#pragma unroll
    for (int p = 0; p < NPAIR2; ++p) {
        int m0 = itile * ITILE2 + (tid >> 5) * (32 * RI2) + (2 * p) * 32 + (tid & 31), m1 = m0 + 32;
        m0 = m0 < ni ? m0 : ni - 1;
        m1 = m1 < ni ? m1 : ni - 1;
        const float4 p0 = ipts[m0], p1 = ipts[m1];
        ax[p] = pack2(p0.x, p1.x); ay[p] = pack2(p0.y, p1.y); az[p] = pack2(p0.z, p1.z);
        if (WGT) al[p] = pack2(p0.w, p1.w);
    }
    float* const mybox = wbox[tid >> 5];
    if (CULL) warp_bbox<NPAIR2>(ax, ay, az, mybox);
#pragma unroll
    for (int r = 0; r < RI2; ++r) { A1[r] = 0.0; AX[r] = 0.0; AY[r] = 0.0; AZ[r] = 0.0; }
    for (int it = 0; it < nst; ++it) {
        const int s = it % NSTAGE;
        mbar_wait(&full[s], (uint32_t)((it / NSTAGE) & 1));
        const ulonglong2* sp = reinterpret_cast<const ulonglong2*>(smraw + s * P2_STAGE_BYTES);
        bool skip = false;
        if (CULL) {
            const float4 blo = tbox[2 * (st0 + it)], bhi = tbox[2 * (st0 + it) + 1];
            skip = box_gap2(mybox, blo, bhi) - omax_stage[st0 + it] >= CULL_GAP;
        }
#pragma unroll 1
        for (int sc = 0; sc < (skip ? 0 : P2_STAGE / SUB); ++sc) {
            if (CULL) {
                const int sb = (st0 + it) * (P2_STAGE / SUB) + sc;
                if (box_gap2(mybox, tsub[2 * sb], tsub[2 * sb + 1]) - omax_sub[sb] >= CULL_GAP) continue;
            }
            const ulonglong2* q = sp + sc * (3 * SUB);
            u64 s1[NPAIR2], sx[NPAIR2], sy[NPAIR2], sz[NPAIR2];
#pragma unroll
            for (int p = 0; p < NPAIR2; ++p) { s1[p] = 0ull; sx[p] = 0ull; sy[p] = 0ull; sz[p] = 0ull; }
            if (GRP > 0) {
#pragma unroll 1
                for (int g0 = 0; g0 < SUB; g0 += (GRP > 0 ? GRP : SUB)) {
                    u64 g1[NPAIR2], gx[NPAIR2], gy[NPAIR2], gz[NPAIR2];
#pragma unroll
                    for (int jj = 0; jj < (GRP > 0 ? GRP : 1); ++jj) {
                        const ulonglong2 bxy = q[3 * (g0 + jj)];
                        const ulonglong2 bzo = q[3 * (g0 + jj) + 1];
                        const u64 rn = q[3 * (g0 + jj) + 2].x;
#pragma unroll
                        for (int p = 0; p < NPAIR2; ++p) {
                            const u64 dx = fsub2(ax[p], bxy.x), dy = fsub2(ay[p], bxy.y), dz = fsub2(az[p], bzo.x);
                            u64 t = ffma2(dx, dx, bzo.y);
                            t = ffma2(dy, dy, t);
                            t = ffma2(dz, dz, t);
                            if (WGT) t = fadd2(t, al[p]);
                            const float2 tt = unpack2(t);
                            const u64 pr = fmul2(pack2(ex2(-tt.x), ex2(-tt.y)), rn);
                            g1[p] = jj == 0 ? pr : fadd2(g1[p], pr);
                            gx[p] = jj == 0 ? fmul2(pr, dx) : ffma2(pr, dx, gx[p]);
                            gy[p] = jj == 0 ? fmul2(pr, dy) : ffma2(pr, dy, gy[p]);
                            gz[p] = jj == 0 ? fmul2(pr, dz) : ffma2(pr, dz, gz[p]);
                        }
                    }
#pragma unroll
                    for (int p = 0; p < NPAIR2; ++p) {
                        s1[p] = fadd2(s1[p], g1[p]); sx[p] = fadd2(sx[p], gx[p]);
                        sy[p] = fadd2(sy[p], gy[p]); sz[p] = fadd2(sz[p], gz[p]);
                    }
                }
            } else {
#pragma unroll UNROLL2
                for (int jj = 0; jj < SUB; ++jj) {
                    const ulonglong2 bxy = q[3 * jj];
                    const ulonglong2 bzo = q[3 * jj + 1];
                    const u64 rn = q[3 * jj + 2].x;
#pragma unroll
                    for (int p = 0; p < NPAIR2; ++p) {
                        const u64 dx = fsub2(ax[p], bxy.x), dy = fsub2(ay[p], bxy.y), dz = fsub2(az[p], bzo.x);
                        u64 t = ffma2(dx, dx, bzo.y);
                        t = ffma2(dy, dy, t);
                        t = ffma2(dz, dz, t);
                        if (WGT) t = fadd2(t, al[p]);
                        const float2 tt = unpack2(t);
                        const u64 pr = fmul2(pack2(ex2(-tt.x), ex2(-tt.y)), rn);
                        s1[p] = fadd2(s1[p], pr);
                        sx[p] = ffma2(pr, dx, sx[p]);
                        sy[p] = ffma2(pr, dy, sy[p]);
                        sz[p] = ffma2(pr, dz, sz[p]);
                    }
                }
            }
#pragma unroll
            for (int p = 0; p < NPAIR2; ++p) {
                const float2 v1 = unpack2(s1[p]), vx = unpack2(sx[p]), vy = unpack2(sy[p]), vz = unpack2(sz[p]);
                A1[2 * p] += (double)v1.x; AX[2 * p] += (double)vx.x; AY[2 * p] += (double)vy.x; AZ[2 * p] += (double)vz.x;
                A1[2 * p + 1] += (double)v1.y; AX[2 * p + 1] += (double)vx.y; AY[2 * p + 1] += (double)vy.y; AZ[2 * p + 1] += (double)vz.y;
            }
        }
        __syncthreads();
        if (tid == 0 && it + NSTAGE < nst) {
            mbar_expect_tx(&full[s], P2_STAGE_BYTES);
            tma_load_1d(smraw + s * P2_STAGE_BYTES, jbytes + (size_t)(st0 + it + NSTAGE) * P2_STAGE_BYTES, P2_STAGE_BYTES, &full[s]);
        }
    }
#pragma unroll
    for (int r = 0; r < RI2; ++r) {
        const int m = itile * ITILE2 + (tid >> 5) * (32 * RI2) + r * 32 + (tid & 31);
        if (m < ni) {
            double2* dst = reinterpret_cast<double2*>(part + ((size_t)split * ni + m) * 4);
            dst[0] = make_double2(A1[r], AX[r]);
            dst[1] = make_double2(AY[r], AZ[r]);
        }
    }
}

__global__ void __launch_bounds__(THREADS)
finalize2_kernel(const DevState* __restrict__ st, const double* __restrict__ sigma2_ptr, const double* __restrict__ part,
                 const int* __restrict__ tile_slots, int m, const double* __restrict__ yc, const double* __restrict__ ts, double* __restrict__ p1,
                 double* __restrict__ pxc, double* __restrict__ mom_part) {
    const int i = blockIdx.x * THREADS + threadIdx.x;
    double v[RM_SRC];
#pragma unroll
    for (int k = 0; k < RM_SRC; ++k) v[k] = 0.0;
    if (i < m) {
        double a1 = 0.0, a[3] = {0.0, 0.0, 0.0};
        const int nsplit = tile_slots[i / ITILE2];
        for (int s = 0; s < nsplit; ++s) {
            const double2* src = reinterpret_cast<const double2*>(part + ((size_t)s * m + i) * 4);
            const double2 u0 = src[0], u1 = src[1];
            a1 += u0.x; a[0] += u0.y; a[1] += u1.x; a[2] += u1.y;
        }
        const double inv_sk = 1.0 / sqrt(LOG2E / (2.0 * *sigma2_ptr));
        const double vv[3] = {-a[0] * inv_sk, -a[1] * inv_sk, -a[2] * inv_sk};
        const double y[3] = {yc[3 * (size_t)i], yc[3 * (size_t)i + 1], yc[3 * (size_t)i + 2]};
        double z[3];
        if (ts != nullptr) {
#pragma unroll
            for (int d = 0; d < 3; ++d) z[d] = ts[3 * (size_t)i + d] - st->cx[d];
        } else {
            const double sc = (st->tf_kind == 0) ? st->scale : 1.0;
#pragma unroll
            for (int d = 0; d < 3; ++d) {
                const double l0 = sc * st->lin[3 * d], l1 = sc * st->lin[3 * d + 1], l2 = sc * st->lin[3 * d + 2];
                const double tp = l0 * st->cy[0] + l1 * st->cy[1] + l2 * st->cy[2] + st->t[d] - st->cx[d];
                z[d] = l0 * y[0] + l1 * y[1] + l2 * y[2] + tp;
            }
        }
        p1[i] = a1;
#pragma unroll
        for (int d = 0; d < 3; ++d) pxc[3 * (size_t)i + d] = a1 * z[d] + vv[d];
        v[RM_NP] = a1;
#pragma unroll
        for (int d = 0; d < 3; ++d) {
            v[RM_SY + d] = a1 * y[d];
            v[RM_V1 + d] = vv[d];
#pragma unroll
            for (int e = 0; e < 3; ++e) v[RM_VY + 3 * d + e] = vv[d] * y[e];
        }
        v[RM_C + 0] = a1 * y[0] * y[0]; v[RM_C + 1] = a1 * y[0] * y[1]; v[RM_C + 2] = a1 * y[0] * y[2];
        v[RM_C + 3] = a1 * y[1] * y[1]; v[RM_C + 4] = a1 * y[1] * y[2]; v[RM_C + 5] = a1 * y[2] * y[2];
    }
    block_reduce_store<RM_SRC>(v, mom_part + (size_t)blockIdx.x * RM_SRC);
}

__global__ void __launch_bounds__(THREADS)
src_moments_api_kernel(int m, const double* __restrict__ yc, const double* __restrict__ p1, const double* __restrict__ pxc,
                       double* __restrict__ mom_part) {
    const int i = blockIdx.x * THREADS + threadIdx.x;
    double v[MOM_SRC];
#pragma unroll
    for (int k = 0; k < MOM_SRC; ++k) v[k] = 0.0;
    if (i < m) {
        const double a1 = p1[i];
        const double a[3] = {pxc[3 * (size_t)i], pxc[3 * (size_t)i + 1], pxc[3 * (size_t)i + 2]};
        const double y[3] = {yc[3 * (size_t)i], yc[3 * (size_t)i + 1], yc[3 * (size_t)i + 2]};
        v[MOM_NP] = a1;
#pragma unroll
        for (int d = 0; d < 3; ++d) {
            v[MOM_SX + d] = a[d];
            v[MOM_SY + d] = a1 * y[d];
#pragma unroll
            for (int e = 0; e < 3; ++e) v[MOM_B + 3 * d + e] = a[d] * y[e];
        }
        v[MOM_C + 0] = a1 * y[0] * y[0]; v[MOM_C + 1] = a1 * y[0] * y[1]; v[MOM_C + 2] = a1 * y[0] * y[2];
        v[MOM_C + 3] = a1 * y[1] * y[1]; v[MOM_C + 4] = a1 * y[1] * y[2]; v[MOM_C + 5] = a1 * y[2] * y[2];
    }
    block_reduce_store<MOM_SRC>(v, mom_part + (size_t)blockIdx.x * MOM_SRC);
}

__global__ void __launch_bounds__(THREADS)
tgt_moments_api_kernel(const double* __restrict__ pt1, const double* __restrict__ xc, int n, double* __restrict__ mom_part) {
    const int i = blockIdx.x * THREADS + threadIdx.x;
    double v[MOM_TGT] = {0.0, 0.0, 0.0, 0.0, 0.0};
    if (i < n) {
        const double p = pt1[i], x0 = xc[3 * (size_t)i], x1 = xc[3 * (size_t)i + 1], x2 = xc[3 * (size_t)i + 2];
        v[0] = p; v[1] = p * x0; v[2] = p * x1; v[3] = p * x2; v[4] = p * (x0 * x0 + x1 * x1 + x2 * x2);
    }
    block_reduce_store<MOM_TGT>(v, mom_part + (size_t)blockIdx.x * MOM_TGT);
}

__device__ inline void jacobi_svd(int n, const double a[3][3], double U[3][3], double s[3], double V[3][3]) {
    double W[3][3];
    for (int i = 0; i < 3; ++i)
        for (int j = 0; j < 3; ++j) { W[i][j] = (i < n && j < n) ? a[i][j] : 0.0; V[i][j] = (i == j) ? 1.0 : 0.0; }
    for (int sweep = 0; sweep < 60; ++sweep) {
        double off = 0.0;
        for (int p = 0; p < n - 1; ++p)
            for (int q = p + 1; q < n; ++q) {
                double al = 0, be = 0, ga = 0;
                for (int i = 0; i < n; ++i) { al += W[i][p] * W[i][p]; be += W[i][q] * W[i][q]; ga += W[i][p] * W[i][q]; }
                if (ga == 0.0) continue;
                const double lim = 1e-32 * al * be;
                if (ga * ga <= lim) continue;
                off = fmax(off, ga * ga / (al * be));
                const double zeta = (be - al) / (2.0 * ga);
                const double t = (zeta >= 0 ? 1.0 : -1.0) / (fabs(zeta) + sqrt(1.0 + zeta * zeta));
                const double c = 1.0 / sqrt(1.0 + t * t), sn = c * t;
                for (int i = 0; i < n; ++i) {
                    const double wp = W[i][p], wq = W[i][q];
                    W[i][p] = c * wp - sn * wq; W[i][q] = sn * wp + c * wq;
                    const double vp = V[i][p], vq = V[i][q];
                    V[i][p] = c * vp - sn * vq; V[i][q] = sn * vp + c * vq;
                }
            }
        if (off == 0.0) break;
    }
    int ord[3] = {0, 1, 2};
    double nrm[3] = {0, 0, 0};
    for (int j = 0; j < n; ++j) { double t = 0; for (int i = 0; i < n; ++i) t += W[i][j] * W[i][j]; nrm[j] = sqrt(t); }
    for (int i = 0; i < n - 1; ++i)
        for (int j = 0; j < n - 1 - i; ++j)
            if (nrm[ord[j]] < nrm[ord[j + 1]]) { int t = ord[j]; ord[j] = ord[j + 1]; ord[j + 1] = t; }
    double Vs[3][3];
    for (int j = 0; j < 3; ++j)
        for (int i = 0; i < 3; ++i) { U[i][j] = (i == j) ? 1.0 : 0.0; Vs[i][j] = (i == j) ? 1.0 : 0.0; }
    const double tiny = nrm[ord[0]] * 1e-300;
    for (int j = 0; j < n; ++j) {
        const int c = ord[j];
        s[j] = nrm[c];
        for (int i = 0; i < n; ++i) { Vs[i][j] = V[i][c]; U[i][j] = (nrm[c] > tiny) ? W[i][c] / nrm[c] : 0.0; }
    }
    for (int j = n; j < 3; ++j) s[j] = 0.0;
    if (n == 3) {
        if (!(s[2] > tiny) && s[1] > tiny) {
            U[0][2] = U[1][0] * U[2][1] - U[2][0] * U[1][1];
            U[1][2] = U[2][0] * U[0][1] - U[0][0] * U[2][1];
            U[2][2] = U[0][0] * U[1][1] - U[1][0] * U[0][1];
        }
    } else if (n == 2) {
        if (!(s[1] > tiny) && s[0] > tiny) { U[0][1] = -U[1][0]; U[1][1] = U[0][0]; }
    }
    for (int i = 0; i < 3; ++i) for (int j = 0; j < 3; ++j) V[i][j] = Vs[i][j];
}

__device__ inline double det_n(int n, const double a[3][3]) {
    if (n == 2) return a[0][0] * a[1][1] - a[0][1] * a[1][0];
    return a[0][0] * (a[1][1] * a[2][2] - a[1][2] * a[2][1]) - a[0][1] * (a[1][0] * a[2][2] - a[1][2] * a[2][0]) +
           a[0][2] * (a[1][0] * a[2][1] - a[1][1] * a[2][0]);
}

__device__ inline void solve_affine(int n, const double Y[3][3], const double A[3][3], double B[3][3]) {
    double Mx[3][6];
    for (int i = 0; i < n; ++i)
        for (int j = 0; j < n; ++j) { Mx[i][j] = Y[j][i]; Mx[i][n + j] = A[j][i]; }
    for (int k = 0; k < n; ++k) {
        int piv = k;
        for (int i = k + 1; i < n; ++i) if (fabs(Mx[i][k]) > fabs(Mx[piv][k])) piv = i;
        if (piv != k) for (int j = 0; j < 2 * n; ++j) { const double t = Mx[k][j]; Mx[k][j] = Mx[piv][j]; Mx[piv][j] = t; }
        for (int i = k + 1; i < n; ++i) {
            const double f = Mx[i][k] / Mx[k][k];
            for (int j = k; j < 2 * n; ++j) Mx[i][j] -= f * Mx[k][j];
        }
    }
    double Z[3][3];
    for (int c = 0; c < n; ++c)
        for (int i = n - 1; i >= 0; --i) {
            double t = Mx[i][n + c];
            for (int j = i + 1; j < n; ++j) t -= Mx[i][j] * Z[j][c];
            Z[i][c] = t / Mx[i][i];
        }
    for (int i = 0; i < 3; ++i) for (int j = 0; j < 3; ++j) B[i][j] = (i < n && j < n) ? Z[j][i] : (i == j ? 1.0 : 0.0);
}

__device__ inline void mstep_solve_api(DevState* st, const double* __restrict__ mom) {
    const int n = st->dim;
    const double Np = mom[MOM_NP];
    double mux[3], muy[3], A[3][3], Y[3][3];
    for (int a = 0; a < 3; ++a) { mux[a] = mom[MOM_SX + a] / Np; muy[a] = mom[MOM_SY + a] / Np; }
    const double Cs[3][3] = {{mom[MOM_C + 0], mom[MOM_C + 1], mom[MOM_C + 2]},
                             {mom[MOM_C + 1], mom[MOM_C + 3], mom[MOM_C + 4]},
                             {mom[MOM_C + 2], mom[MOM_C + 4], mom[MOM_C + 5]}};
    for (int a = 0; a < 3; ++a)
        for (int b = 0; b < 3; ++b) {
            A[a][b] = mom[MOM_B + 3 * a + b] - mom[MOM_SX + a] * mom[MOM_SY + b] / Np;
            Y[a][b] = Cs[a][b] - mom[MOM_SY + a] * mom[MOM_SY + b] / Np;
        }
    double tr_yp1y = 0.0;
    for (int a = 0; a < n; ++a) tr_yp1y += Y[a][a];
    double tr_xp1x = mom[MOM_TXX] + mom[MOM_NPT] * (mux[0] * mux[0] + mux[1] * mux[1] + mux[2] * mux[2]) -
                     2.0 * (mux[0] * mom[MOM_SXT] + mux[1] * mom[MOM_SXT + 1] + mux[2] * mom[MOM_SXT + 2]);
    double lin[3][3], scale = 1.0, sigma2, q;
    if (st->tf_kind == 0) {
        double U[3][3], s[3], V[3][3], UVt[3][3];
        jacobi_svd(n, A, U, s, V);
        for (int i = 0; i < 3; ++i)
            for (int j = 0; j < 3; ++j) { double t = 0; for (int k = 0; k < n; ++k) t += U[i][k] * V[j][k]; UVt[i][j] = t; }
        const double dt = det_n(n, UVt);
        for (int i = 0; i < 3; ++i)
            for (int j = 0; j < 3; ++j) {
                double t = 0;
                for (int k = 0; k < n; ++k) t += U[i][k] * (k == n - 1 ? dt : 1.0) * V[j][k];
                lin[i][j] = (i < n && j < n) ? t : (i == j ? 1.0 : 0.0);
            }
        double tr_atr = 0.0;
        for (int i = 0; i < n; ++i) for (int j = 0; j < n; ++j) tr_atr += A[i][j] * lin[i][j];
        scale = st->update_scale ? tr_atr / tr_yp1y : 1.0;
        if (st->update_scale) sigma2 = (tr_xp1x - scale * tr_atr) / (Np * n);
        else sigma2 = (tr_xp1x + tr_yp1y - scale * tr_atr) / (Np * n);
        sigma2 = fmax(sigma2, EPS32);
        q = (tr_xp1x - 2.0 * scale * tr_atr + scale * scale * tr_yp1y) / (2.0 * sigma2) + n * Np * 0.5 * log(sigma2);
    } else {
        solve_affine(n, Y, A, lin);
        double tr_abt = 0.0;
        for (int i = 0; i < n; ++i) for (int j = 0; j < n; ++j) tr_abt += A[i][j] * lin[i][j];
        sigma2 = fmax((tr_xp1x - tr_abt) / (Np * n), EPS32);
        q = (tr_xp1x - 2.0 * tr_abt + tr_abt) / (2.0 * sigma2) + n * Np * 0.5 * log(sigma2);
    }
    for (int a = 0; a < 3; ++a) {
        double r = 0.0;
        for (int b = 0; b < 3; ++b) r += lin[a][b] * (st->cy[b] + muy[b]);
        st->t[a] = (a < n) ? (st->cx[a] + mux[a]) - scale * r : 0.0;
        for (int b = 0; b < 3; ++b) st->lin[3 * a + b] = lin[a][b];
    }
    st->scale = scale; st->sigma2 = sigma2; st->q = q; st->n_p = Np;
}

__device__ inline void mstep_solve_residual(DevState* st, const double* __restrict__ mom) {
    const int n = st->dim;
    const double Np = mom[RM_NP];
    const double sk2 = LOG2E / (2.0 * st->sigma2);
    const double Srr = mom[RM_SRR] / sk2;
    double muy[3], V1[3], Aold[3][3], Y[3][3], Vc[3][3], Am[3][3], told[3];
    const double sc = (st->tf_kind == 0) ? st->scale : 1.0;
    for (int a = 0; a < 3; ++a) {
        muy[a] = mom[RM_SY + a] / Np;
        V1[a] = mom[RM_V1 + a];
        for (int b = 0; b < 3; ++b) Aold[a][b] = sc * st->lin[3 * a + b];
    }
    for (int a = 0; a < 3; ++a)
        told[a] = Aold[a][0] * st->cy[0] + Aold[a][1] * st->cy[1] + Aold[a][2] * st->cy[2] + st->t[a] - st->cx[a];
    const double Cs[3][3] = {{mom[RM_C + 0], mom[RM_C + 1], mom[RM_C + 2]},
                             {mom[RM_C + 1], mom[RM_C + 3], mom[RM_C + 4]},
                             {mom[RM_C + 2], mom[RM_C + 4], mom[RM_C + 5]}};
    for (int a = 0; a < 3; ++a)
        for (int b = 0; b < 3; ++b) {
            Y[a][b] = Cs[a][b] - mom[RM_SY + a] * mom[RM_SY + b] / Np;
            Vc[a][b] = mom[RM_VY + 3 * a + b] - V1[a] * mom[RM_SY + b] / Np;
        }
    for (int a = 0; a < 3; ++a)
        for (int b = 0; b < 3; ++b) {
            double t = Vc[a][b];
            for (int k = 0; k < 3; ++k) t += Aold[a][k] * Y[k][b];
            Am[a][b] = (a < n && b < n) ? t : 0.0;
        }
    double tr_yp1y = 0.0;
    for (int a = 0; a < n; ++a) tr_yp1y += Y[a][a];
    double lin[3][3], Anew[3][3], scale = 1.0, tr_atr = 0.0;
    if (st->tf_kind == 0) {
        double U[3][3], s[3], V[3][3], UVt[3][3];
        jacobi_svd(n, Am, U, s, V);
        for (int i = 0; i < 3; ++i)
            for (int j = 0; j < 3; ++j) { double t = 0; for (int k = 0; k < n; ++k) t += U[i][k] * V[j][k]; UVt[i][j] = t; }
        const double dt = det_n(n, UVt);
        for (int i = 0; i < 3; ++i)
            for (int j = 0; j < 3; ++j) {
                double t = 0;
                for (int k = 0; k < n; ++k) t += U[i][k] * (k == n - 1 ? dt : 1.0) * V[j][k];
                lin[i][j] = (i < n && j < n) ? t : (i == j ? 1.0 : 0.0);
            }
        for (int i = 0; i < n; ++i) for (int j = 0; j < n; ++j) tr_atr += Am[i][j] * lin[i][j];
        scale = st->update_scale ? tr_atr / tr_yp1y : 1.0;
    } else {
        solve_affine(n, Y, Am, lin);
    }
    for (int i = 0; i < 3; ++i) for (int j = 0; j < 3; ++j) Anew[i][j] = scale * lin[i][j];
    double Q = Srr - (V1[0] * V1[0] + V1[1] * V1[1] + V1[2] * V1[2]) / Np;
    for (int a = 0; a < n; ++a)
        for (int b = 0; b < n; ++b) {
            const double dab = Aold[a][b] - Anew[a][b];
            Q += 2.0 * dab * Vc[a][b];
            double t = 0.0;
            for (int k = 0; k < n; ++k) t += (Aold[a][k] - Anew[a][k]) * Y[k][b];
            Q += t * dab;
        }
    double sigma2;
    if (st->tf_kind == 0 && !st->update_scale) sigma2 = (Q + tr_atr) / (Np * n);
    else sigma2 = Q / (Np * n);
    sigma2 = fmax(sigma2, EPS32);
    const double q = Q / (2.0 * sigma2) + n * Np * 0.5 * log(sigma2);
    for (int a = 0; a < 3; ++a) {
        double mux = st->cx[a] + told[a] + V1[a] / Np, r = 0.0;
        for (int b = 0; b < 3; ++b) { mux += Aold[a][b] * muy[b]; r += Anew[a][b] * (st->cy[b] + muy[b]); }
        st->t[a] = (a < n) ? mux - r : 0.0;
    }
    for (int a = 0; a < 3; ++a) for (int b = 0; b < 3; ++b) st->lin[3 * a + b] = lin[a][b];
    st->scale = scale; st->sigma2 = sigma2; st->q = q; st->n_p = Np;
}

__device__ __forceinline__ void mstep_staged(DevState* st, const double* mom) {
    __shared__ DevState sst;
    __shared__ double smom[MOM_PAD];
    static_assert(sizeof(DevState) % 8 == 0, "DevState is copied as 8-byte words");
    const int nw = (int)(sizeof(DevState) / 8);
    for (int e = threadIdx.x; e < nw; e += blockDim.x) reinterpret_cast<double*>(&sst)[e] = reinterpret_cast<const double*>(st)[e];
    for (int e = threadIdx.x; e < MOM_PAD; e += blockDim.x) smom[e] = mom[e];
    __syncthreads();
    if (threadIdx.x == 0) mstep_solve_residual(&sst, smom);
    __syncthreads();
    if (threadIdx.x < 16) reinterpret_cast<double*>(st)[threadIdx.x] = reinterpret_cast<const double*>(&sst)[threadIdx.x];
}

template <int SOLVE>
__global__ void __launch_bounds__(256)
moments_kernel(DevState* st, const double* __restrict__ part_a, int nb_a, int ka, const double* __restrict__ part_b, int nb_b,
               int kb, double* __restrict__ mom) {
    __shared__ double sh[8][32];
    const int k = threadIdx.x & 31, w = threadIdx.x >> 5;
    double s = 0.0;
    if (k < ka) {
#pragma unroll 8
        for (int b = w; b < nb_a; b += 8) s += part_a[(size_t)b * ka + k];
    } else if (k < ka + kb) {
#pragma unroll 8
        for (int b = w; b < nb_b; b += 8) s += part_b[(size_t)b * kb + (k - ka)];
    }
    sh[w][k] = s;
    __syncthreads();
    if (w == 0) {
        double t = 0.0;
#pragma unroll
        for (int i = 0; i < 8; ++i) t += sh[i][k];
        mom[k] = t;
    }
    if (SOLVE) {
        __syncthreads();
        mstep_staged(st, mom);
    }
}
__global__ void mstep_residual_kernel(DevState* st, const double* __restrict__ mom) {
    mstep_staged(st, mom);
}
__global__ void mstep_api_kernel(DevState* st, const double* __restrict__ mom) {
    if (threadIdx.x == 0) mstep_solve_api(st, mom);
}

#ifndef CPD_HOST_EMU
__device__ __forceinline__ void st_release_sys(unsigned long long* p, unsigned long long v) {
    asm volatile("st.release.sys.global.u64 [%0], %1;" ::"l"(p), "l"(v) : "memory");
}
__device__ __forceinline__ unsigned long long ld_acquire_sys(const unsigned long long* p) {
    unsigned long long v;
    asm volatile("ld.acquire.sys.global.u64 %0, [%1];" : "=l"(v) : "l"(p) : "memory");
    return v;
}
__device__ __forceinline__ double ld_relaxed_sys(const double* p) {
    double v;
    asm volatile("ld.relaxed.sys.global.f64 %0, [%1];" : "=d"(v) : "l"(p) : "memory");
    return v;
}
#endif
__global__ void __launch_bounds__(256)
moments_p2p_kernel(DevState* st, const double* __restrict__ part_a, int nb_a, int ka, const double* __restrict__ part_b,
                   int nb_b, int kb, double* __restrict__ mom, P2PInfo* info) {
    __shared__ double sh[8][32];
    __shared__ double loc[32];
    __shared__ int timeout;
    const int k = threadIdx.x & 31, w = threadIdx.x >> 5;
    double s = 0.0;
    if (k < ka) {
#pragma unroll 8
        for (int b = w; b < nb_a; b += 8) s += part_a[(size_t)b * ka + k];
    } else if (k < ka + kb) {
#pragma unroll 8
        for (int b = w; b < nb_b; b += 8) s += part_b[(size_t)b * kb + (k - ka)];
    }
    sh[w][k] = s;
    if (threadIdx.x == 0) timeout = 0;
    __syncthreads();
    if (w == 0) {
        double t = 0.0;
#pragma unroll
        for (int i = 0; i < 8; ++i) t += sh[i][k];
        loc[k] = t;
    }
    __syncthreads();
    const int world = info->world, rank = info->rank;
    const unsigned long long seq = info->seq + 1;
    const int par = (int)(seq & 1ull);
    for (int r = w; r < world; r += 8) info->box[r]->slots[par][rank][k] = loc[k];
    __threadfence_system();
    __syncthreads();
    if ((int)threadIdx.x < world) {
        st_release_sys(&info->box[threadIdx.x]->flags[par][rank], seq);
        const unsigned long long* f = &info->box[rank]->flags[par][threadIdx.x];
        const unsigned long long t0 = globaltimer_ns(), limit = info->timeout_ns;
        while (ld_acquire_sys(f) < seq) {
            __nanosleep(64);
            if (globaltimer_ns() - t0 > limit) { timeout = 1; break; }
        }
    }
    __syncthreads();
    if (w == 0) {
        double t = 0.0;
        for (int r = 0; r < world; ++r) t += ld_relaxed_sys(&info->box[rank]->slots[par][r][k]);
        mom[k] = t;
        if (k == 0) {
            info->seq = seq;
            if (timeout) st->err = 1;
        }
    }
    __syncthreads();
    if (!timeout && st->err == 0) mstep_staged(st, mom);
}

__device__ __forceinline__ unsigned spread3(unsigned v) {
    v &= 0x3ffu;
    v = (v | (v << 16)) & 0x030000ffu;
    v = (v | (v << 8)) & 0x0300f00fu;
    v = (v | (v << 4)) & 0x030c30c3u;
    v = (v | (v << 2)) & 0x09249249u;
    return v;
}
__global__ void __launch_bounds__(THREADS)
morton_kernel(const double* __restrict__ pts, long long n, double lo0, double lo1, double lo2, double inv_range,
              unsigned* __restrict__ codes, int* __restrict__ idx) {
    const long long i = (long long)blockIdx.x * THREADS + threadIdx.x;
    if (i < n) {
        const double q0 = (pts[3 * i] - lo0) * inv_range, q1 = (pts[3 * i + 1] - lo1) * inv_range, q2 = (pts[3 * i + 2] - lo2) * inv_range;
        const unsigned a = (unsigned)fmin(fmax(q0 * 1023.0, 0.0), 1023.0), b = (unsigned)fmin(fmax(q1 * 1023.0, 0.0), 1023.0),
                       c = (unsigned)fmin(fmax(q2 * 1023.0, 0.0), 1023.0);
        codes[i] = spread3(a) | (spread3(b) << 1) | (spread3(c) << 2);
        idx[i] = (int)i;
    }
}
__global__ void __launch_bounds__(THREADS)
morton_frame_kernel(const double* __restrict__ pts, long long n, const double* __restrict__ frame, unsigned* __restrict__ codes,
                    int* __restrict__ idx) {
    const long long i = (long long)blockIdx.x * THREADS + threadIdx.x;
    if (i < n) {
        const double inv_range = frame[3];
        const double q0 = (pts[3 * i] - frame[0]) * inv_range, q1 = (pts[3 * i + 1] - frame[1]) * inv_range,
                     q2 = (pts[3 * i + 2] - frame[2]) * inv_range;
        const unsigned a = (unsigned)fmin(fmax(q0 * 1023.0, 0.0), 1023.0), b = (unsigned)fmin(fmax(q1 * 1023.0, 0.0), 1023.0),
                       c = (unsigned)fmin(fmax(q2 * 1023.0, 0.0), 1023.0);
        codes[i] = spread3(a) | (spread3(b) << 1) | (spread3(c) << 2);
        idx[i] = (int)i;
    }
}
__global__ void __launch_bounds__(THREADS)
gather3_frame_kernel(const double* __restrict__ in, const int* __restrict__ perm, long long n, const double* __restrict__ frame,
                     double* __restrict__ out) {
    const long long k = (long long)blockIdx.x * THREADS + threadIdx.x;
    if (k < n) {
        const long long j = perm[k];
        out[3 * k] = in[3 * j] - frame[4]; out[3 * k + 1] = in[3 * j + 1] - frame[5]; out[3 * k + 2] = in[3 * j + 2] - frame[6];
    }
}
__global__ void __launch_bounds__(THREADS)
gather3_kernel(const double* __restrict__ in, const int* __restrict__ perm, long long n, double o0, double o1, double o2,
               double* __restrict__ out) {
    const long long k = (long long)blockIdx.x * THREADS + threadIdx.x;
    if (k < n) {
        const long long j = perm[k];
        out[3 * k] = in[3 * j] - o0; out[3 * k + 1] = in[3 * j + 1] - o1; out[3 * k + 2] = in[3 * j + 2] - o2;
    }
}
__global__ void __launch_bounds__(THREADS)
gather1_kernel(const double* __restrict__ in, const int* __restrict__ perm, long long n, double* __restrict__ out) {
    const long long k = (long long)blockIdx.x * THREADS + threadIdx.x;
    if (k < n) out[k] = in[perm[k]];
}
__global__ void __launch_bounds__(THREADS)
gather_f32_kernel(const double* __restrict__ in, const int* __restrict__ perm, long long n, float* __restrict__ out) {
    const long long k = (long long)blockIdx.x * THREADS + threadIdx.x;
    if (k < n) out[k] = (float)in[perm[k]];
}
__global__ void __launch_bounds__(THREADS)
scatter_kernel(const double* __restrict__ in, const int* __restrict__ perm, long long n, int ncomp, double* __restrict__ out) {
    const long long k = (long long)blockIdx.x * THREADS + threadIdx.x;
    if (k < n) {
        const long long j = perm[k];
        for (int c = 0; c < ncomp; ++c) out[ncomp * j + c] = in[ncomp * k + c];
    }
}

__global__ void __launch_bounds__(THREADS)
stats_kernel(const double* __restrict__ pts, long long n, double* __restrict__ part) {
    __shared__ double sh[9][THREADS / 32];
    const long long i = (long long)blockIdx.x * THREADS + threadIdx.x;
    double v[9];
    if (i < n) {
        for (int a = 0; a < 3; ++a) { v[a] = pts[3 * i + a]; v[3 + a] = v[a]; v[6 + a] = v[a]; }
    } else {
        for (int a = 0; a < 3; ++a) { v[a] = 0.0; v[3 + a] = 1.0e300; v[6 + a] = -1.0e300; }
    }
    const int lane = threadIdx.x & 31, wid = threadIdx.x >> 5;
#pragma unroll
    for (int k = 0; k < 9; ++k) {
        double x = v[k];
#pragma unroll
        for (int o = 16; o > 0; o >>= 1) {
            const double y = __shfl_xor_sync(0xffffffffu, x, o);
            x = k < 3 ? x + y : (k < 6 ? fmin(x, y) : fmax(x, y));
        }
        if (lane == 0) sh[k][wid] = x;
    }
    __syncthreads();
    if (threadIdx.x < 9) {
        const int k = threadIdx.x;
        double x = sh[k][0];
        for (int w = 1; w < THREADS / 32; ++w) x = k < 3 ? x + sh[k][w] : (k < 6 ? fmin(x, sh[k][w]) : fmax(x, sh[k][w]));
        part[(size_t)blockIdx.x * 9 + k] = x;
    }
}
__global__ void __launch_bounds__(288)
stats_fold_kernel(const double* __restrict__ part, int nb, double* __restrict__ out) {
    const int k = threadIdx.x >> 5, lane = threadIdx.x & 31;
    double x = k < 3 ? 0.0 : (k < 6 ? 1.0e300 : -1.0e300);
    for (int b = lane; b < nb; b += 32) {
        const double y = part[(size_t)b * 9 + k];
        x = k < 3 ? x + y : (k < 6 ? fmin(x, y) : fmax(x, y));
    }
#pragma unroll
    for (int o = 16; o > 0; o >>= 1) {
        const double y = __shfl_xor_sync(0xffffffffu, x, o);
        x = k < 3 ? x + y : (k < 6 ? fmin(x, y) : fmax(x, y));
    }
    if (lane == 0) out[k] = x;
}

__global__ void cloud_frame_kernel(const double* __restrict__ sums9, long long count, int is_target, long long n_global, int origin_given,
                                   double o0, double o1, double o2, DevState* __restrict__ st, double* __restrict__ frame) {
    if (threadIdx.x != 0 || blockIdx.x != 0) return;
    double range = 0.0;
    for (int a = 0; a < 3; ++a) { frame[a] = sums9[3 + a]; range = fmax(range, sums9[6 + a] - sums9[3 + a]); }
    frame[3] = range > 0.0 ? 1.0 / range : 0.0;
    const double og[3] = {o0, o1, o2};
    for (int a = 0; a < 3; ++a) {
        const double o = origin_given ? og[a] : sums9[a] / (double)count;
        frame[4 + a] = o;
        if (is_target) st->cx[a] = o; else st->cy[a] = o;
    }
    if (is_target) st->n_global = n_global; else st->m = count;
}

__global__ void __launch_bounds__(THREADS)
cloud_sums_kernel(const double* __restrict__ pts, long long n, double* __restrict__ out) {
    const long long i = (long long)blockIdx.x * THREADS + threadIdx.x;
    double v[4] = {0.0, 0.0, 0.0, 0.0};
    if (i < n) {
        const double a = pts[3 * i], b = pts[3 * i + 1], c = pts[3 * i + 2];
        v[0] = a * a + b * b + c * c; v[1] = a; v[2] = b; v[3] = c;
    }
    block_reduce_store<4>(v, out + (size_t)blockIdx.x * 4);
}
__global__ void __launch_bounds__(1024)
reduce_cols_kernel(const double* __restrict__ part, int nb, int k, double* __restrict__ out) {
    const int c = threadIdx.x >> 5, lane = threadIdx.x & 31;
    if (c >= k) return;
    double s = 0.0;
    for (int b = lane; b < nb; b += 32) s += part[(size_t)b * k + c];
#pragma unroll
    for (int o = 16; o > 0; o >>= 1) s += __shfl_xor_sync(0xffffffffu, s, o);
    if (lane == 0) out[c] = s;
}

__global__ void __launch_bounds__(THREADS)
uncentre_px_kernel(const DevState* __restrict__ st, const double* __restrict__ p1, const double* __restrict__ pxc, int m,
                   double* __restrict__ px) {
    const int i = blockIdx.x * THREADS + threadIdx.x;
    if (i < m) {
#pragma unroll
        for (int d = 0; d < 3; ++d) px[3 * (size_t)i + d] = pxc[3 * (size_t)i + d] + st->cx[d] * p1[i];
    }
}
__global__ void __launch_bounds__(THREADS)
centre_px_kernel(const DevState* __restrict__ st, const double* __restrict__ p1, const double* __restrict__ px, int m,
                 double* __restrict__ pxc) {
    const int i = blockIdx.x * THREADS + threadIdx.x;
    if (i < m) {
#pragma unroll
        for (int d = 0; d < 3; ++d) pxc[3 * (size_t)i + d] = px[3 * (size_t)i + d] - st->cx[d] * p1[i];
    }
}
__global__ void __launch_bounds__(THREADS)
rbf_kernel_kernel(const float* __restrict__ x, long long nx, const float* __restrict__ y, long long ny, int dim, float two_beta,
                  float* __restrict__ out) {
    const long long j = (long long)blockIdx.y * THREADS + threadIdx.x;
    const long long i = blockIdx.x;
    if (j < ny) {
        float d2 = 0.f;
        for (int a = 0; a < dim; ++a) { const float d = x[i * dim + a] - y[j * dim + a]; d2 += d * d; }
        out[i * ny + j] = expf(-d2 / two_beta);
    }
}

__global__ void __launch_bounds__(THREADS)
imq_kernel_kernel(const float* __restrict__ x, long long nx, const float* __restrict__ y, long long ny, int dim, float c,
                  float* __restrict__ out) {
    const long long j = (long long)blockIdx.y * THREADS + threadIdx.x;
    const long long i = blockIdx.x;
    if (j < ny) {
        float d2 = 0.f;
        for (int a = 0; a < dim; ++a) { const float d = __fsub_rn(x[i * dim + a], y[j * dim + a]); d2 = __fadd_rn(d2, __fmul_rn(d, d)); }
        out[i * ny + j] = __fdiv_rn(1.0f, __fsqrt_rn(__fadd_rn(d2, c)));
    }
}

__global__ void __launch_bounds__(THREADS)
nr_gram_kernel(const double* __restrict__ yc, double c0, double c1, double c2, long long m, int dim, float two_beta,
               float* __restrict__ G) {
    const long long j = (long long)blockIdx.y * THREADS + threadIdx.x;
    const long long i = blockIdx.x;
    if (j < m) {
        const double cc[3] = {c0, c1, c2};
        float d2 = 0.f;
        for (int a = 0; a < dim; ++a) {
            const float d = (float)(yc[3 * i + a] + cc[a]) - (float)(yc[3 * j + a] + cc[a]);
            d2 += d * d;
        }
        G[i * m + j] = expf(-d2 / two_beta);
    }
}
__global__ void __launch_bounds__(THREADS)
nr_apply_kernel(const float* __restrict__ G, const double* __restrict__ W, const double* __restrict__ yc, double c0, double c1,
                double c2, long long m, double* __restrict__ ts) {
    const long long i = (long long)blockIdx.x * (THREADS / 32) + (threadIdx.x >> 5);
    const int lane = threadIdx.x & 31;
    if (i >= m) return;
    const float* row = G + i * m;
    double a0 = 0.0, a1 = 0.0, a2 = 0.0;
    for (long long j = lane; j < m; j += 32) {
        const double g = (double)row[j];
        a0 += g * W[3 * j]; a1 += g * W[3 * j + 1]; a2 += g * W[3 * j + 2];
    }
    a0 = warp_sum(a0); a1 = warp_sum(a1); a2 = warp_sum(a2);
    if (lane == 0) {
        ts[3 * i] = yc[3 * i] + c0 + a0;
        ts[3 * i + 1] = yc[3 * i + 1] + c1 + a1;
        ts[3 * i + 2] = yc[3 * i + 2] + c2 + a2;
    }
}
__global__ void __launch_bounds__(THREADS)
nr_system_kernel(const float* __restrict__ G, const double* __restrict__ wgt ,
                 const double* __restrict__ sigma2_ptr, double lmd, long long m, double* __restrict__ A) {
    const long long j = (long long)blockIdx.y * THREADS + threadIdx.x;
    const long long i = blockIdx.x;
    if (j < m) A[i * m + j] = wgt[i] * (double)G[i * m + j] + (i == j ? lmd * *sigma2_ptr : 0.0);
}
__global__ void __launch_bounds__(THREADS)
nr_rhs_kernel(const DevState* __restrict__ st, const double* __restrict__ p1, const double* __restrict__ pxc,
              const double* __restrict__ yc, const double* __restrict__ p1t, const double* __restrict__ pxt, double alpha, long long m,
              double* __restrict__ B) {
    const long long i = (long long)blockIdx.x * THREADS + threadIdx.x;
    if (i < m) {
        const double k = p1t ? st->sigma2 / alpha : 0.0;
#pragma unroll
        for (int c = 0; c < 3; ++c) {
            const double y = yc[3 * i + c] + st->cy[c];
            double r = pxc[3 * i + c] + p1[i] * (st->cx[c] - y);
            if (p1t) r += k * (pxt[3 * i + c] - p1t[i] * y);
            B[c * m + i] = r;
        }
    }
}
__global__ void __launch_bounds__(THREADS)
nr_weight_kernel(const double* __restrict__ p1, const double* __restrict__ p1t, const double* __restrict__ sigma2_ptr, double alpha,
                 long long m, double* __restrict__ wgt) {
    const long long i = (long long)blockIdx.x * THREADS + threadIdx.x;
    if (i < m) wgt[i] = p1[i] + (*sigma2_ptr / alpha) * p1t[i];
}
__global__ void __launch_bounds__(THREADS)
nr_identity_kernel(const double* __restrict__ yc, double c0, double c1, double c2, long long m, double* __restrict__ ts) {
    const long long i = (long long)blockIdx.x * THREADS + threadIdx.x;
    if (i < m) { ts[3 * i] = yc[3 * i] + c0; ts[3 * i + 1] = yc[3 * i + 1] + c1; ts[3 * i + 2] = yc[3 * i + 2] + c2; }
}
__global__ void __launch_bounds__(THREADS)
nr_unpack_kernel(const double* __restrict__ B, long long m, double* __restrict__ W) {
    const long long i = (long long)blockIdx.x * THREADS + threadIdx.x;
    if (i < m) { W[3 * i] = B[i]; W[3 * i + 1] = B[m + i]; W[3 * i + 2] = B[2 * m + i]; }
}
__global__ void __launch_bounds__(THREADS)
nr_resid_kernel(const DevState* __restrict__ st, const double* __restrict__ p1, const double* __restrict__ pxc,
                const double* __restrict__ ts_old, const double* __restrict__ ts_new, long long m, double* __restrict__ part) {
    const long long i = (long long)blockIdx.x * THREADS + threadIdx.x;
    double v[2] = {0.0, 0.0};
    if (i < m) {
        double acc = 0.0;
#pragma unroll
        for (int c = 0; c < 3; ++c) {
            const double e = ts_old[3 * i + c] - ts_new[3 * i + c];
            const double vv = pxc[3 * i + c] - p1[i] * (ts_old[3 * i + c] - st->cx[c]);
            acc += 2.0 * e * vv + p1[i] * e * e;
        }
        v[0] = acc; v[1] = p1[i];
    }
    block_reduce_store<2>(v, part + (size_t)blockIdx.x * 2);
}
__global__ void __launch_bounds__(THREADS)
nr_traces_kernel(const DevState* __restrict__ st, const double* __restrict__ pt1, const double* __restrict__ xc, long long n,
                 const double* __restrict__ p1, const double* __restrict__ pxc, const double* __restrict__ ts, long long m,
                 double* __restrict__ part) {
    const long long i = (long long)blockIdx.x * THREADS + threadIdx.x;
    double v[4] = {0.0, 0.0, 0.0, 0.0};
    if (i < n) {
        double x2 = 0.0;
#pragma unroll
        for (int c = 0; c < 3; ++c) { const double x = xc[3 * i + c] + st->cx[c]; x2 += x * x; }
        v[0] = pt1[i] * x2;
    }
    if (i < m) {
        double pt = 0.0, t2 = 0.0;
#pragma unroll
        for (int c = 0; c < 3; ++c) {
            const double t = ts[3 * i + c];
            pt += (pxc[3 * i + c] + st->cx[c] * p1[i]) * t;
            t2 += t * t;
        }
        v[1] = pt; v[2] = p1[i] * t2; v[3] = p1[i];
    }
    block_reduce_store<4>(v, part + (size_t)blockIdx.x * 4);
}
__global__ void __launch_bounds__(32)
nr_sigma_api_kernel(DevState* st, const double* __restrict__ tr) {
    if (threadIdx.x == 0) {
        st->sigma2 = (tr[0] - 2.0 * tr[1] + tr[2]) / (tr[3] * st->dim);
        st->q = st->sigma2;
        st->n_p = tr[3];
    }
}
__global__ void __launch_bounds__(32)
nr_sigma_kernel(DevState* st, const double* __restrict__ part, int nb, const double* __restrict__ mom) {
    if (threadIdx.x == 0) {
        double a = 0.0, np_ = 0.0;
        for (int b = 0; b < nb; ++b) { a += part[2 * (size_t)b]; np_ += part[2 * (size_t)b + 1]; }
        const double sk2 = LOG2E / (2.0 * st->sigma2);
        const double q = mom[RM_SRR] / sk2 + a;
        st->sigma2 = q / (np_ * st->dim);
        st->q = st->sigma2;
        st->n_p = np_;
    }
}

constexpr int GT_K = 4, GT_TILE = 256;
__global__ void __launch_bounds__(THREADS)
gauss_transform_kernel(const float4* __restrict__ tg, int n, const float4* __restrict__ sc, const float* __restrict__ wts, int mpad,
                       int k0, int kn, double* __restrict__ out) {
    __shared__ float4 sp[GT_TILE];
    __shared__ float sw[GT_K][GT_TILE];
    const int i = blockIdx.x * THREADS + threadIdx.x;
    const float4 t = tg[i < n ? i : n - 1];
    double acc[GT_K];
#pragma unroll
    for (int c = 0; c < GT_K; ++c) acc[c] = 0.0;
    for (int j0 = 0; j0 < mpad; j0 += GT_TILE) {
        __syncthreads();
        sp[threadIdx.x] = sc[j0 + threadIdx.x];
#pragma unroll
        for (int c = 0; c < GT_K; ++c) sw[c][threadIdx.x] = c < kn ? wts[(size_t)(k0 + c) * mpad + j0 + threadIdx.x] : 0.0f;
        __syncthreads();
#pragma unroll 1
        for (int g = 0; g < GT_TILE; g += 32) {
            float a[GT_K];
#pragma unroll
            for (int c = 0; c < GT_K; ++c) a[c] = 0.0f;
#pragma unroll 8
            for (int jj = 0; jj < 32; ++jj) {
                const float4 b = sp[g + jj];
                const float dx = t.x - b.x, dy = t.y - b.y, dz = t.z - b.z;
                const float e = ex2(-fmaf(dz, dz, fmaf(dy, dy, dx * dx)));
#pragma unroll
                for (int c = 0; c < GT_K; ++c) a[c] = fmaf(e, sw[c][g + jj], a[c]);
            }
#pragma unroll
            for (int c = 0; c < GT_K; ++c) acc[c] += (double)a[c];
        }
    }
    if (i < n)
        for (int c = 0; c < kn; ++c) out[(size_t)(k0 + c) * n + i] = acc[c];
}

__global__ void __launch_bounds__(256)
probe_ffma_kernel(float* out, int iters, float seed) {
    float a[16];
#pragma unroll
    for (int k = 0; k < 16; ++k) a[k] = seed + k;
    const float m = 0.9999f + seed * 1e-9f, c = 1e-7f;
    for (int i = 0; i < iters; ++i) {
#pragma unroll
        for (int k = 0; k < 16; ++k) a[k] = fmaf(a[k], m, c);
    }
    float s = 0.f;
#pragma unroll
    for (int k = 0; k < 16; ++k) s += a[k];
    if (s == 123.456f) out[0] = s;
}
__global__ void __launch_bounds__(256)
probe_mufu_kernel(float* out, int iters, float seed) {
    float a[8];
#pragma unroll
    for (int k = 0; k < 8; ++k) a[k] = seed * 0.01f - k;
    for (int i = 0; i < iters; ++i) {
#pragma unroll
        for (int k = 0; k < 8; ++k) a[k] = ex2(a[k]) - 1.5f;
    }
    float s = 0.f;
#pragma unroll
    for (int k = 0; k < 8; ++k) s += a[k];
    if (s == 123.456f) out[0] = s;
}
__global__ void __launch_bounds__(256)
probe_ffma2_kernel(float* out, int iters, float seed) {
    u64 a[8];
#pragma unroll
    for (int k = 0; k < 8; ++k) a[k] = pack2(seed + k, seed - k);
    const u64 m = pack2(0.9999f + seed * 1e-9f, 0.9998f), c = pack2(1e-7f, 2e-7f);
    for (int i = 0; i < iters; ++i) {
#pragma unroll
        for (int k = 0; k < 8; ++k) a[k] = ffma2(a[k], m, c);
    }
    float s = 0.f;
#pragma unroll
    for (int k = 0; k < 8; ++k) { const float2 v = unpack2(a[k]); s += v.x + v.y; }
    if (s == 123.456f) out[0] = s;
}
__global__ void __launch_bounds__(256)
probe_ffma_mixed_kernel(float* out, int iters, float seed) {
    u64 a[6];
    float b[6];
#pragma unroll
    for (int k = 0; k < 6; ++k) { a[k] = pack2(seed + k, seed - k); b[k] = seed + 0.5f * k; }
    const u64 m2 = pack2(0.9999f + seed * 1e-9f, 0.9998f), c2 = pack2(1e-7f, 2e-7f);
    const float m = 0.9999f + seed * 1e-9f, c = 1e-7f;
    for (int i = 0; i < iters; ++i) {
#pragma unroll
        for (int k = 0; k < 6; ++k) { a[k] = ffma2(a[k], m2, c2); b[k] = fmaf(b[k], m, c); }
    }
    float s = 0.f;
#pragma unroll
    for (int k = 0; k < 6; ++k) { const float2 v = unpack2(a[k]); s += v.x + v.y + b[k]; }
    if (s == 123.456f) out[0] = s;
}
template <int NF, bool PACKED>
__global__ void __launch_bounds__(256)
probe_mix_kernel(float* out, int iters, float seed) {
    float x[8], acc[8];
    unsigned long long pa[4];
#pragma unroll
    for (int k = 0; k < 8; ++k) { x[k] = seed * 0.01f - 0.1f * k; acc[k] = 0.f; }
#pragma unroll
    for (int k = 0; k < 4; ++k) pa[k] = pack2(seed, seed + k);
    const float m = 0.999f + seed * 1e-9f;
    const unsigned long long pm = pack2(m, m);
    for (int i = 0; i < iters; ++i) {
        if (PACKED) {
#pragma unroll
            for (int k = 0; k < 4; ++k) {
#pragma unroll
                for (int f = 0; f < NF; ++f) pa[k] = ffma2(pa[k], pm, pm);
                const float2 v = unpack2(pa[k]);
                pa[k] = pack2(ex2(-v.x * v.x), ex2(-v.y * v.y));
            }
        } else {
#pragma unroll
            for (int k = 0; k < 8; ++k) {
                float t = x[k];
#pragma unroll
                for (int f = 0; f < NF - 1; ++f) t = fmaf(t, m, acc[k]);
                const float e = ex2(-t * t);
                acc[k] = e;
            }
        }
    }
    float s = 0.f;
#pragma unroll
    for (int k = 0; k < 8; ++k) s += acc[k];
#pragma unroll
    for (int k = 0; k < 4; ++k) { const float2 v = unpack2(pa[k]); s += v.x + v.y; }
    if (s == 123.456f) out[0] = s;
}
__global__ void probe_clock_kernel(long long* out) {
    const long long c0 = clock64();
    const unsigned long long t0 = globaltimer_ns();
    unsigned long long t1;
    do { t1 = globaltimer_ns(); } while (t1 - t0 < 2000000ull);
    out[0] = clock64() - c0;
    out[1] = (long long)(t1 - t0);
}

}
```

Baseline: 104.9.

## Replace packed float2 pair records with scalar float4 records and split target arrays

Drops the duplicated-pair source records (srcJ) and the three-float4 target records (tgtQ), so both passes read compact float4 point records plus a separate float array of target normalisers. Each stage is loaded as two TMA copies. The inner loops switch from emulated packed-pair arithmetic to plain scalar float ops, and the pass-1 rows per thread go from 4 to 6. The aim is to cut shared-memory and global traffic per stage and remove the pack/unpack overhead, at the cost of more registers per thread in pass 1.

```diff
diff --git a/probreg_b200/csrc/cpd_b200.cu b/probreg_b200/csrc/cpd_b200.cu
--- a/probreg_b200/csrc/cpd_b200.cu
+++ b/probreg_b200/csrc/cpd_b200.cu
@@ -147,7 +147,8 @@
     long long m = 0, mpad = 0, n = 0, npad = 0, n_global = 0;
     double *d_yc = nullptr, *d_ts = nullptr, *d_xc = nullptr, *d_raw = nullptr;
     size_t raw_cap = 0;
-    float4 *d_srcP = nullptr, *d_srcJ = nullptr, *d_tgtP = nullptr, *d_tgtQ = nullptr;
+    float4 *d_srcP = nullptr, *d_tgtP = nullptr;
+    float* d_tgtR = nullptr;
     P1Part* d_part1 = nullptr;
     double* d_part2 = nullptr;
     size_t part1_cap = 0, part2_cap = 0;
@@ -475,7 +476,7 @@
     const long long cover = std::max(h->mpad, h->n);
     mark(h, 0);
     pack_kernel<<<blocks_for(cover), THREADS, 0, h->stream>>>(h->d_state, d_sigma2, h->d_yc, d_ts, h->d_xc, h->m, h->mpad,
-                                                              h->n, h->d_srcP, h->d_srcJ, h->d_tgtP);
+                                                              h->n, h->d_srcP, h->d_tgtP);
     mark(h, 1);
     const bool cull = h->cull_on && h->cull_active;
     const int nst1 = (int)(h->mpad / P1_STAGE);
@@ -490,24 +491,24 @@
     }
     const bool wgt = h->wgt_on;
     if (wgt) {
-        weight_patch_kernel<<<blocks_for(h->m), THREADS, 0, h->stream>>>(h->d_la, h->m, h->d_srcP, h->d_srcJ);
+        weight_patch_kernel<<<blocks_for(h->m), THREADS, 0, h->stream>>>(h->d_la, h->m, h->d_srcP);
         h->launches += 1;
     }
-#define CPD_PASS1(C, W) pass1_kernel<C, W><<<h->g1, THREADS, PASS1_SMEM, h->stream>>>(h->d_tgtP, (int)h->n, h->d_srcJ, h->d_work1, h->d_part1, h->d_sbox, nst1, (C) ? h->d_ssub : nullptr)
+#define CPD_PASS1(C, W) pass1_kernel<C, W><<<h->g1, THREADS, PASS1_SMEM, h->stream>>>(h->d_tgtP, (int)h->n, h->d_srcP, h->d_work1, h->d_part1, h->d_sbox, nst1, (C) ? h->d_ssub : nullptr)
     if (cull) { if (wgt) CPD_PASS1(true, true); else CPD_PASS1(true, false); }
     else { if (wgt) CPD_PASS1(false, true); else CPD_PASS1(false, false); }
 #undef CPD_PASS1
     mark(h, 2);
     finalize1_kernel<<<blocks_for(h->npad), THREADS, 0, h->stream>>>(h->d_state, d_sigma2, d_w, h->d_part1, h->d_slots1, (int)h->n,
-                                                                     h->d_tgtP, h->d_tgtQ, h->npad, h->d_pt1, h->d_mom_tgt,
+                                                                     h->d_tgtP, h->d_tgtR, h->npad, h->d_pt1, h->d_mom_tgt,
                                                                      wgt ? h->d_log2c : nullptr);
     mark(h, 3);
     if (cull) {
-        stage_omax_kernel<<<(unsigned)(h->npad / P2_STAGE), THREADS, 0, h->stream>>>(h->d_tgtQ, h->d_omax);
-        sub_omax_kernel<<<(unsigned)((nsub2 + 7) / 8), THREADS, 0, h->stream>>>(h->d_tgtQ, nsub2, h->d_omax_sub);
+        stage_omax_kernel<<<(unsigned)(h->npad / P2_STAGE), THREADS, 0, h->stream>>>(h->d_tgtP, h->d_omax);
+        sub_omax_kernel<<<(unsigned)((nsub2 + 7) / 8), THREADS, 0, h->stream>>>(h->d_tgtP, nsub2, h->d_omax_sub);
         h->launches += 2;
     }
-#define CPD_PASS2(C, W) pass2_kernel<C, W><<<h->g2, THREADS, PASS2_SMEM, h->stream>>>(h->d_srcP, (int)h->m, h->d_tgtQ, h->d_work2, h->d_part2, (C) ? h->d_tbox : nullptr, (C) ? h->d_omax : nullptr, (C) ? h->d_tsub : nullptr, (C) ? h->d_omax_sub : nullptr)
+#define CPD_PASS2(C, W) pass2_kernel<C, W><<<h->g2, THREADS, PASS2_SMEM, h->stream>>>(h->d_srcP, (int)h->m, h->d_tgtP, h->d_tgtR, h->d_work2, h->d_part2, (C) ? h->d_tbox : nullptr, (C) ? h->d_omax : nullptr, (C) ? h->d_tsub : nullptr, (C) ? h->d_omax_sub : nullptr)
     if (cull) { if (wgt) CPD_PASS2(true, true); else CPD_PASS2(true, false); }
     else { if (wgt) CPD_PASS2(false, true); else CPD_PASS2(false, false); }
 #undef CPD_PASS2
@@ -636,7 +637,7 @@
     for (int r = 0; r < P2P_MAX; ++r) if (h->peer_ptr[r]) cudaIpcCloseMemHandle(h->peer_ptr[r]);
     if (h->d_box) cudaFree(h->d_box);
     if (h->d_p2p) cudaFree(h->d_p2p);
-    void* ptrs[] = {h->d_yc, h->d_ts, h->d_xc, h->d_raw, h->d_srcP, h->d_srcJ, h->d_tgtP, h->d_tgtQ, h->d_part1, h->d_part2, h->d_pt1, h->d_p1,
+    void* ptrs[] = {h->d_yc, h->d_ts, h->d_xc, h->d_raw, h->d_srcP, h->d_tgtP, h->d_tgtR, h->d_part1, h->d_part2, h->d_pt1, h->d_p1,
                     h->d_pxc, h->d_px, h->d_mom_src, h->d_mom_tgt, h->d_mom, h->d_sums, h->d_state, h->d_flush};
     for (void* p : ptrs) if (p) cudaFree(p);
     if (h->h_pin) cudaFreeHost(h->h_pin);
@@ -667,7 +668,6 @@
         TRY(dev_alloc(&h->d_yc, (size_t)m * 3));
         TRY(dev_alloc(&h->d_ts, (size_t)m * 3));
         TRY(dev_alloc(&h->d_srcP, (size_t)h->mpad));
-        TRY(dev_alloc(&h->d_srcJ, (size_t)h->mpad * 2));
         TRY(dev_alloc(&h->d_p1, (size_t)m));
         TRY(dev_alloc(&h->d_pxc, (size_t)m * 3));
         TRY(dev_alloc(&h->d_px, (size_t)m * 3));
@@ -694,8 +694,8 @@
         h->n = n_local;
         h->npad = (n_local + P2_STAGE - 1) / P2_STAGE * P2_STAGE;
         TRY(dev_alloc(&h->d_xc, (size_t)n_local * 3));
-        TRY(dev_alloc(&h->d_tgtP, (size_t)n_local));
-        TRY(dev_alloc(&h->d_tgtQ, (size_t)h->npad * 3));
+        TRY(dev_alloc(&h->d_tgtP, (size_t)h->npad));
+        TRY(dev_alloc(&h->d_tgtR, (size_t)h->npad));
         TRY(dev_alloc(&h->d_pt1, (size_t)n_local));
         TRY(dev_alloc(&h->d_perm_tgt, (size_t)n_local));
         TRY(dev_alloc(&h->d_outN, (size_t)n_local));
diff --git a/probreg_b200/csrc/kernels.cuh b/probreg_b200/csrc/kernels.cuh
--- a/probreg_b200/csrc/kernels.cuh
+++ b/probreg_b200/csrc/kernels.cuh
@@ -5,7 +5,7 @@
 namespace cpd {
 
 #ifndef CPD_RI1
-#define CPD_RI1 4
+#define CPD_RI1 6
 #endif
 #ifndef CPD_RI2
 #define CPD_RI2 4
@@ -32,7 +32,6 @@
 constexpr int THREADS = 256;
 constexpr int RI1 = CPD_RI1, RI2 = CPD_RI2;
 constexpr int ITILE1 = THREADS * RI1, ITILE2 = THREADS * RI2;
-constexpr int NPAIR1 = RI1 / 2, NPAIR2 = RI2 / 2;
 #ifndef CPD_P1_STAGE
 #define CPD_P1_STAGE 512
 #endif
@@ -42,12 +41,13 @@
 constexpr int P1_STAGE = CPD_P1_STAGE;
 constexpr int P2_STAGE = CPD_P2_STAGE;
 static_assert(P1_STAGE % 256 == 0 && P2_STAGE % 256 == 0 && P1_STAGE >= 256 && P2_STAGE >= 256, "stage sizes are multiples of 256");
-constexpr int P1_REC = 32, P2_REC = 48;
+constexpr int P1_REC = 16, P2_REC = 16 + 4;
 #ifndef CPD_NSTAGE
 #define CPD_NSTAGE 3
 #endif
 constexpr int NSTAGE = CPD_NSTAGE;
 constexpr int P1_STAGE_BYTES = P1_STAGE * P1_REC, P2_STAGE_BYTES = P2_STAGE * P2_REC;
+constexpr int P2_STAGE_PBYTES = P2_STAGE * 16;
 constexpr int SUB = CPD_SUB;
 constexpr int GRP = CPD_GRP;
 constexpr int PASS1_SMEM = NSTAGE * P1_STAGE_BYTES + 64, PASS2_SMEM = NSTAGE * P2_STAGE_BYTES + 64;
@@ -114,27 +114,23 @@
 }
 #include "emu_device.h"
 namespace cpd {
+static inline float sub_rn(float a, float b) { return a - b; }
+static inline float add_rn(float a, float b) { return a + b; }
+static inline float mul_rn(float a, float b) { return a * b; }
+static inline float fma_rn(float a, float b, float c) { return fmaf(a, b, c); }
 #else
 __device__ __forceinline__ float ex2(float x) {
     float y;
     asm("ex2.approx.ftz.f32 %0, %1;" : "=f"(y) : "f"(x));
     return y;
 }
+__device__ __forceinline__ float sub_rn(float a, float b) { return __fsub_rn(a, b); }
+__device__ __forceinline__ float add_rn(float a, float b) { return __fadd_rn(a, b); }
+__device__ __forceinline__ float mul_rn(float a, float b) { return __fmul_rn(a, b); }
+__device__ __forceinline__ float fma_rn(float a, float b, float c) { return __fmaf_rn(a, b, c); }
 typedef unsigned long long u64;
 __device__ __forceinline__ u64 pack2(float lo, float hi) { u64 r; asm("mov.b64 %0, {%1, %2};" : "=l"(r) : "f"(lo), "f"(hi)); return r; }
 __device__ __forceinline__ float2 unpack2(u64 v) { float2 r; asm("mov.b64 {%0, %1}, %2;" : "=f"(r.x), "=f"(r.y) : "l"(v)); return r; }
-__device__ __forceinline__ u64 fsub2(u64 a, u64 b) {
-    const float2 x = unpack2(a), y = unpack2(b);
-    return pack2(__fsub_rn(x.x, y.x), __fsub_rn(x.y, y.y));
-}
-__device__ __forceinline__ u64 fadd2(u64 a, u64 b) {
-    const float2 x = unpack2(a), y = unpack2(b);
-    return pack2(__fadd_rn(x.x, y.x), __fadd_rn(x.y, y.y));
-}
-__device__ __forceinline__ u64 fmul2(u64 a, u64 b) {
-    const float2 x = unpack2(a), y = unpack2(b);
-    return pack2(__fmul_rn(x.x, y.x), __fmul_rn(x.y, y.y));
-}
 __device__ __forceinline__ u64 ffma2(u64 a, u64 b, u64 c) {
     const float2 x = unpack2(a), y = unpack2(b), z = unpack2(c);
     return pack2(__fmaf_rn(x.x, y.x, z.x), __fmaf_rn(x.y, y.y, z.y));
@@ -199,8 +195,7 @@
 pack_kernel(const DevState* __restrict__ st, const double* __restrict__ sigma2_ptr,
             const double* __restrict__ yc , const double* __restrict__ ts ,
             const double* __restrict__ xc , long long m, long long mpad, long long n,
-            float4* __restrict__ srcP , float4* __restrict__ srcJ ,
-            float4* __restrict__ tgtP ) {
+            float4* __restrict__ srcP , float4* __restrict__ tgtP ) {
     const long long i = (long long)blockIdx.x * THREADS + threadIdx.x;
     const double sk = sqrt(LOG2E / (2.0 * *sigma2_ptr));
     if (i < mpad) {
@@ -229,8 +224,6 @@
             o = make_float4(FAR_COORD, FAR_COORD, FAR_COORD, 0.0f);
         }
         srcP[i] = o;
-        srcJ[2 * i] = make_float4(o.x, o.x, o.y, o.y);
-        srcJ[2 * i + 1] = make_float4(o.z, o.z, 0.0f, 0.0f);
     }
     if (i < n) {
         tgtP[i] = make_float4((float)(sk * xc[3 * i]), (float)(sk * xc[3 * i + 1]), (float)(sk * xc[3 * i + 2]), 0.0f);
@@ -238,15 +231,9 @@
 }
 
 __global__ void __launch_bounds__(THREADS)
-weight_patch_kernel(const float* __restrict__ la, long long m, float4* __restrict__ srcP, float4* __restrict__ srcJ) {
+weight_patch_kernel(const float* __restrict__ la, long long m, float4* __restrict__ srcP) {
     const long long i = (long long)blockIdx.x * THREADS + threadIdx.x;
-    if (i < m) {
-        const float v = la[i];
-        srcP[i].w = v;
-        float4 r = srcJ[2 * i + 1];
-        r.z = v; r.w = v;
-        srcJ[2 * i + 1] = r;
-    }
+    if (i < m) srcP[i].w = la[i];
 }
 
 constexpr float CULL_GAP = 130.0f;
@@ -282,11 +269,11 @@
     }
 }
 __global__ void __launch_bounds__(THREADS)
-stage_omax_kernel(const float4* __restrict__ tgtQ, float* __restrict__ omax) {
+stage_omax_kernel(const float4* __restrict__ tgtP, float* __restrict__ omax) {
     __shared__ float sh[THREADS / 32];
     const int b = blockIdx.x;
     float m = 3.0e38f;
-    for (int i = threadIdx.x; i < P2_STAGE; i += THREADS) m = fminf(m, tgtQ[3 * ((size_t)b * P2_STAGE + i) + 1].z);
+    for (int i = threadIdx.x; i < P2_STAGE; i += THREADS) m = fminf(m, tgtP[(size_t)b * P2_STAGE + i].w);
 #pragma unroll
     for (int o = 16; o > 0; o >>= 1) m = fminf(m, __shfl_xor_sync(0xffffffffu, m, o));
     if ((threadIdx.x & 31) == 0) sh[threadIdx.x >> 5] = m;
@@ -320,24 +307,23 @@
     }
 }
 __global__ void __launch_bounds__(THREADS)
-sub_omax_kernel(const float4* __restrict__ tgtQ, int nsub, float* __restrict__ omax) {
+sub_omax_kernel(const float4* __restrict__ tgtP, int nsub, float* __restrict__ omax) {
     const int b = blockIdx.x * (THREADS / 32) + (threadIdx.x >> 5), lane = threadIdx.x & 31;
     if (b >= nsub) return;
     float m = 3.0e38f;
-    for (int i = lane; i < SUB; i += 32) m = fminf(m, tgtQ[3 * ((size_t)b * SUB + i) + 1].z);
+    for (int i = lane; i < SUB; i += 32) m = fminf(m, tgtP[(size_t)b * SUB + i].w);
 #pragma unroll
     for (int o = 16; o > 0; o >>= 1) m = fminf(m, __shfl_xor_sync(0xffffffffu, m, o));
     if (lane == 0) omax[b] = -m;
 }
-template <int NP>
-__device__ __forceinline__ void warp_bbox(const u64 (&ax)[NP], const u64 (&ay)[NP], const u64 (&az)[NP], float* __restrict__ wbox) {
+template <int RI>
+__device__ __forceinline__ void warp_bbox(const float (&ax)[RI], const float (&ay)[RI], const float (&az)[RI], float* __restrict__ wbox) {
     float lo[3] = {3.0e38f, 3.0e38f, 3.0e38f}, hi[3] = {-3.0e38f, -3.0e38f, -3.0e38f};
 #pragma unroll
-    for (int p = 0; p < NP; ++p) {
-        const float2 x = unpack2(ax[p]), y = unpack2(ay[p]), z = unpack2(az[p]);
-        lo[0] = fminf(lo[0], fminf(x.x, x.y)); hi[0] = fmaxf(hi[0], fmaxf(x.x, x.y));
-        lo[1] = fminf(lo[1], fminf(y.x, y.y)); hi[1] = fmaxf(hi[1], fmaxf(y.x, y.y));
-        lo[2] = fminf(lo[2], fminf(z.x, z.y)); hi[2] = fmaxf(hi[2], fmaxf(z.x, z.y));
+    for (int r = 0; r < RI; ++r) {
+        lo[0] = fminf(lo[0], ax[r]); hi[0] = fmaxf(hi[0], ax[r]);
+        lo[1] = fminf(lo[1], ay[r]); hi[1] = fmaxf(hi[1], ay[r]);
+        lo[2] = fminf(lo[2], az[r]); hi[2] = fmaxf(hi[2], az[r]);
     }
 #pragma unroll
     for (int a = 0; a < 3; ++a) {
@@ -361,60 +347,68 @@
 }
 
 template <bool WGT>
-__device__ __forceinline__ void pass1_sum(const ulonglong2* __restrict__ q, const u64 (&ax)[NPAIR1], const u64 (&ay)[NPAIR1],
-                                          const u64 (&az)[NPAIR1], const u64 (&no)[NPAIR1], u64 (&Sc)[NPAIR1], u64 (&Uc)[NPAIR1]) {
+__device__ __forceinline__ void pass1_sum(const float4* __restrict__ q, const float (&ax)[RI1], const float (&ay)[RI1],
+                                          const float (&az)[RI1], const float (&no)[RI1], float (&Sc)[RI1], float (&Uc)[RI1]) {
     if (GRP > 0) {
 #pragma unroll 1
         for (int g0 = 0; g0 < SUB; g0 += (GRP > 0 ? GRP : SUB)) {
-            u64 gs[NPAIR1], gu[NPAIR1];
+            float gs[RI1], gu[RI1];
 #pragma unroll
             for (int jj = 0; jj < (GRP > 0 ? GRP : 1); ++jj) {
-                const ulonglong2 bxy = q[2 * (g0 + jj)];
-                const u64 bz = q[2 * (g0 + jj) + 1].x;
-                u64 la = 0ull;
-                if (WGT) la = q[2 * (g0 + jj) + 1].y;
-#pragma unroll
-                for (int p = 0; p < NPAIR1; ++p) {
-                    const u64 dx = fsub2(ax[p], bxy.x), dy = fsub2(ay[p], bxy.y), dz = fsub2(az[p], bz);
-                    u64 t = ffma2(dx, dx, no[p]);
-                    t = ffma2(dy, dy, t);
-                    t = ffma2(dz, dz, t);
-                    if (WGT) t = fadd2(t, la);
-                    const float2 tt = unpack2(t);
-                    const u64 e = pack2(ex2(-tt.x), ex2(-tt.y));
-                    gs[p] = jj == 0 ? e : fadd2(gs[p], e);
-                    gu[p] = jj == 0 ? fmul2(e, t) : ffma2(e, t, gu[p]);
+                const float4 b = q[g0 + jj];
+#pragma unroll
+                for (int r = 0; r < RI1; ++r) {
+                    const float dx = sub_rn(ax[r], b.x), dy = sub_rn(ay[r], b.y), dz = sub_rn(az[r], b.z);
+                    float t = fma_rn(dx, dx, no[r]);
+                    t = fma_rn(dy, dy, t);
+                    t = fma_rn(dz, dz, t);
+                    if (WGT) t = add_rn(t, b.w);
+                    const float e = ex2(-t);
+                    gs[r] = jj == 0 ? e : add_rn(gs[r], e);
+                    gu[r] = jj == 0 ? mul_rn(e, t) : fma_rn(e, t, gu[r]);
                 }
             }
 #pragma unroll
-            for (int p = 0; p < NPAIR1; ++p) { Sc[p] = fadd2(Sc[p], gs[p]); Uc[p] = fadd2(Uc[p], gu[p]); }
+            for (int r = 0; r < RI1; ++r) { Sc[r] = add_rn(Sc[r], gs[r]); Uc[r] = add_rn(Uc[r], gu[r]); }
         }
     } else {
 #pragma unroll UNROLL1
         for (int jj = 0; jj < SUB; ++jj) {
-            const ulonglong2 bxy = q[2 * jj];
-            const u64 bz = q[2 * jj + 1].x;
-            u64 la = 0ull;
-            if (WGT) la = q[2 * jj + 1].y;
-#pragma unroll
-            for (int p = 0; p < NPAIR1; ++p) {
-                const u64 dx = fsub2(ax[p], bxy.x), dy = fsub2(ay[p], bxy.y), dz = fsub2(az[p], bz);
-                u64 t = ffma2(dx, dx, no[p]);
-                t = ffma2(dy, dy, t);
-                t = ffma2(dz, dz, t);
-                if (WGT) t = fadd2(t, la);
-                const float2 tt = unpack2(t);
-                const u64 e = pack2(ex2(-tt.x), ex2(-tt.y));
-                Sc[p] = fadd2(Sc[p], e);
-                Uc[p] = ffma2(e, t, Uc[p]);
-            }
+            const float4 b = q[jj];
+#pragma unroll
+            for (int r = 0; r < RI1; ++r) {
+                const float dx = sub_rn(ax[r], b.x), dy = sub_rn(ay[r], b.y), dz = sub_rn(az[r], b.z);
+                float t = fma_rn(dx, dx, no[r]);
+                t = fma_rn(dy, dy, t);
+                t = fma_rn(dz, dz, t);
+                if (WGT) t = add_rn(t, b.w);
+                const float e = ex2(-t);
+                Sc[r] = add_rn(Sc[r], e);
+                Uc[r] = fma_rn(e, t, Uc[r]);
+            }
+        }
+    }
+}
+
+template <bool WGT>
+__device__ __forceinline__ void pass1_umin(const float4* __restrict__ q, int count, const float (&ax)[RI1], const float (&ay)[RI1],
+                                           const float (&az)[RI1], float (&cm)[RI1]) {
+#pragma unroll 4
+    for (int jj = 0; jj < count; ++jj) {
+        const float4 b = q[jj];
+#pragma unroll
+        for (int r = 0; r < RI1; ++r) {
+            const float dx = sub_rn(ax[r], b.x), dy = sub_rn(ay[r], b.y), dz = sub_rn(az[r], b.z);
+            float uu = fma_rn(dz, dz, fma_rn(dy, dy, mul_rn(dx, dx)));
+            if (WGT) uu = add_rn(uu, b.w);
+            cm[r] = fminf(cm[r], uu);
         }
     }
 }
 
 template <bool CULL, bool WGT>
 __global__ void __launch_bounds__(THREADS, CPD_MINB1)
-pass1_kernel(const float4* __restrict__ ipts, int ni, const float4* __restrict__ jrec, const int4* __restrict__ work,
+pass1_kernel(const float4* __restrict__ ipts, int ni, const float4* __restrict__ jrec , const int4* __restrict__ work,
              P1Part* __restrict__ part, const float4* __restrict__ sbox ,
              int nstages_total, const float4* __restrict__ ssub ) {
     __shared__ float wbox[THREADS / 32][8];
@@ -426,7 +420,6 @@
     const int itile = wk.x, split = wk.w;
     const int st0 = wk.y / SPS, nst = (wk.z + SPS - 1) / SPS - st0;
     const int sc_first = wk.y - st0 * SPS, sc_last = wk.z - (st0 + nst - 1) * SPS;
-    const unsigned char* jbytes = reinterpret_cast<const unsigned char*>(jrec);
     if (tid == 0) {
         for (int s = 0; s < NSTAGE; ++s) mbar_init(&full[s], 1);
         mbar_fence_init();
@@ -435,23 +428,22 @@
     if (tid == 0) {
         for (int s = 0; s < NSTAGE && s < nst; ++s) {
             mbar_expect_tx(&full[s], P1_STAGE_BYTES);
-            tma_load_1d(smraw + s * P1_STAGE_BYTES, jbytes + (size_t)(st0 + s) * P1_STAGE_BYTES, P1_STAGE_BYTES, &full[s]);
+            tma_load_1d(smraw + s * P1_STAGE_BYTES, jrec + (size_t)(st0 + s) * P1_STAGE, P1_STAGE_BYTES, &full[s]);
         }
     }
     if (itile * ITILE1 + (tid >> 5) * (32 * RI1) >= ni) return;
-    u64 ax[NPAIR1], ay[NPAIR1], az[NPAIR1], no[NPAIR1];
+    float ax[RI1], ay[RI1], az[RI1], no[RI1];
     double S[RI1], SU[RI1];
 #pragma unroll
-    for (int p = 0; p < NPAIR1; ++p) {
-        int n0 = itile * ITILE1 + (tid >> 5) * (32 * RI1) + (2 * p) * 32 + (tid & 31), n1 = n0 + 32;
+    for (int r = 0; r < RI1; ++r) {
+        int n0 = itile * ITILE1 + (tid >> 5) * (32 * RI1) + r * 32 + (tid & 31);
         n0 = n0 < ni ? n0 : ni - 1;
-        n1 = n1 < ni ? n1 : ni - 1;
-        const float4 p0 = ipts[n0], p1 = ipts[n1];
-        ax[p] = pack2(p0.x, p1.x); ay[p] = pack2(p0.y, p1.y); az[p] = pack2(p0.z, p1.z);
-        no[p] = pack2(-O_INIT, -O_INIT);
+        const float4 p0 = ipts[n0];
+        ax[r] = p0.x; ay[r] = p0.y; az[r] = p0.z;
+        no[r] = -O_INIT;
     }
     float* const mybox = wbox[tid >> 5];
-    warp_bbox<NPAIR1>(ax, ay, az, mybox);
+    warp_bbox<RI1>(ax, ay, az, mybox);
     {
         const int lane = tid & 31;
         float best = 3.0e38f;
@@ -466,35 +458,18 @@
             const int oi = __shfl_xor_sync(0xffffffffu, bi, o);
             if (ob < best || (ob == best && oi < bi)) { best = ob; bi = oi; }
         }
-        const ulonglong2* near = reinterpret_cast<const ulonglong2*>(jbytes + (size_t)bi * P1_STAGE_BYTES);
         float cm[RI1];
 #pragma unroll
         for (int r = 0; r < RI1; ++r) cm[r] = 3.0e38f;
-#pragma unroll 4
-        for (int jj = 0; jj < 128; ++jj) {
-            const ulonglong2 bxy = near[2 * jj];
-            const u64 bz = near[2 * jj + 1].x;
-            u64 la = 0ull;
-            if (WGT) la = near[2 * jj + 1].y;
-#pragma unroll
-            for (int p = 0; p < NPAIR1; ++p) {
-                const u64 dx = fsub2(ax[p], bxy.x), dy = fsub2(ay[p], bxy.y), dz = fsub2(az[p], bz);
-                u64 uu = ffma2(dz, dz, ffma2(dy, dy, fmul2(dx, dx)));
-                if (WGT) uu = fadd2(uu, la);
-                const float2 u = unpack2(uu);
-                cm[2 * p] = fminf(cm[2 * p], u.x);
-                cm[2 * p + 1] = fminf(cm[2 * p + 1], u.y);
-            }
-        }
-#pragma unroll
-        for (int p = 0; p < NPAIR1; ++p)
-            no[p] = pack2(-fminf(O_INIT, floorf(cm[2 * p])), -fminf(O_INIT, floorf(cm[2 * p + 1])));
+        pass1_umin<WGT>(jrec + (size_t)bi * P1_STAGE, 128, ax, ay, az, cm);
+#pragma unroll
+        for (int r = 0; r < RI1; ++r) no[r] = -fminf(O_INIT, floorf(cm[r]));
     }
     float omax_w = O_INIT;
     if (CULL) {
         float om = -3.0e38f;
 #pragma unroll
-        for (int p = 0; p < NPAIR1; ++p) { const float2 nv = unpack2(no[p]); om = fmaxf(om, fmaxf(-nv.x, -nv.y)); }
+        for (int r = 0; r < RI1; ++r) om = fmaxf(om, -no[r]);
 #pragma unroll
         for (int o = 16; o > 0; o >>= 1) om = fmaxf(om, __shfl_xor_sync(0xffffffffu, om, o));
         omax_w = om;
@@ -504,7 +479,7 @@
     for (int it = 0; it < nst; ++it) {
         const int s = it % NSTAGE;
         mbar_wait(&full[s], (uint32_t)((it / NSTAGE) & 1));
-        const ulonglong2* sp = reinterpret_cast<const ulonglong2*>(smraw + s * P1_STAGE_BYTES);
+        const float4* sp = reinterpret_cast<const float4*>(smraw + s * P1_STAGE_BYTES);
         bool skip = false;
         if (CULL) {
             const float4 blo = sbox[2 * (st0 + it)], bhi = sbox[2 * (st0 + it) + 1];
@@ -516,52 +491,32 @@
                 const int sb = (st0 + it) * (P1_STAGE / SUB) + sc;
                 if (box_gap2(mybox, ssub[2 * sb], ssub[2 * sb + 1]) - omax_w >= CULL_GAP) continue;
             }
-            const ulonglong2* q = sp + sc * (2 * SUB);
-            u64 Sc[NPAIR1], Uc[NPAIR1];
-#pragma unroll
-            for (int p = 0; p < NPAIR1; ++p) { Sc[p] = 0ull; Uc[p] = 0ull; }
+            const float4* q = sp + sc * SUB;
+            float Sc[RI1], Uc[RI1];
+#pragma unroll
+            for (int r = 0; r < RI1; ++r) { Sc[r] = 0.0f; Uc[r] = 0.0f; }
             pass1_sum<WGT>(q, ax, ay, az, no, Sc, Uc);
             bool bad = false;
 #pragma unroll
-            for (int p = 0; p < NPAIR1; ++p) {
-                const float2 v = unpack2(Sc[p]);
-                bad |= !(v.x < TWO100) | !(v.y < TWO100);
-            }
+            for (int r = 0; r < RI1; ++r) bad |= !(Sc[r] < TWO100);
             if (__any_sync(0xffffffffu, bad)) {
                 float cm[RI1];
 #pragma unroll
                 for (int r = 0; r < RI1; ++r) cm[r] = 3.0e38f;
-#pragma unroll UNROLL1
-                for (int jj = 0; jj < SUB; ++jj) {
-                    const ulonglong2 bxy = q[2 * jj];
-                    const u64 bz = q[2 * jj + 1].x;
-                    u64 la = 0ull;
-                    if (WGT) la = q[2 * jj + 1].y;
-#pragma unroll
-                    for (int p = 0; p < NPAIR1; ++p) {
-                        const u64 dx = fsub2(ax[p], bxy.x), dy = fsub2(ay[p], bxy.y), dz = fsub2(az[p], bz);
-                        u64 uu = ffma2(dz, dz, ffma2(dy, dy, fmul2(dx, dx)));
-                        if (WGT) uu = fadd2(uu, la);
-                        const float2 u = unpack2(uu);
-                        cm[2 * p] = fminf(cm[2 * p], u.x);
-                        cm[2 * p + 1] = fminf(cm[2 * p + 1], u.y);
-                    }
-                }
-#pragma unroll
-                for (int p = 0; p < NPAIR1; ++p) {
-                    const float2 nv = unpack2(no[p]);
-                    const float o0 = -nv.x, o1 = -nv.y;
-                    const float on0 = fminf(o0, floorf(cm[2 * p])), on1 = fminf(o1, floorf(cm[2 * p + 1]));
-                    const int sh0 = (int)fmaxf(on0 - o0, -4000.0f), sh1 = (int)fmaxf(on1 - o1, -4000.0f);
-                    S[2 * p] = ldexp(S[2 * p], sh0); SU[2 * p] = ldexp(SU[2 * p], sh0);
-                    S[2 * p + 1] = ldexp(S[2 * p + 1], sh1); SU[2 * p + 1] = ldexp(SU[2 * p + 1], sh1);
-                    no[p] = pack2(-on0, -on1);
-                    Sc[p] = 0ull; Uc[p] = 0ull;
+                pass1_umin<WGT>(q, SUB, ax, ay, az, cm);
+#pragma unroll
+                for (int r = 0; r < RI1; ++r) {
+                    const float o0 = -no[r];
+                    const float on0 = fminf(o0, floorf(cm[r]));
+                    const int sh0 = (int)fmaxf(on0 - o0, -4000.0f);
+                    S[r] = ldexp(S[r], sh0); SU[r] = ldexp(SU[r], sh0);
+                    no[r] = -on0;
+                    Sc[r] = 0.0f; Uc[r] = 0.0f;
                 }
                 if (CULL) {
                     float om = -3.0e38f;
 #pragma unroll
-                    for (int p = 0; p < NPAIR1; ++p) { const float2 nv = unpack2(no[p]); om = fmaxf(om, fmaxf(-nv.x, -nv.y)); }
+                    for (int r = 0; r < RI1; ++r) om = fmaxf(om, -no[r]);
 #pragma unroll
                     for (int o = 16; o > 0; o >>= 1) om = fmaxf(om, __shfl_xor_sync(0xffffffffu, om, o));
                     omax_w = om;
@@ -569,39 +524,32 @@
                 pass1_sum<WGT>(q, ax, ay, az, no, Sc, Uc);
             }
 #pragma unroll
-            for (int p = 0; p < NPAIR1; ++p) {
-                const float2 sv = unpack2(Sc[p]), uv = unpack2(Uc[p]), nv = unpack2(no[p]);
-                S[2 * p] += (double)sv.x;
-                S[2 * p + 1] += (double)sv.y;
-                SU[2 * p] += (double)uv.x - (double)nv.x * (double)sv.x;
-                SU[2 * p + 1] += (double)uv.y - (double)nv.y * (double)sv.y;
+            for (int r = 0; r < RI1; ++r) {
+                S[r] += (double)Sc[r];
+                SU[r] += (double)Uc[r] - (double)no[r] * (double)Sc[r];
             }
         }
         __syncthreads();
         if (tid == 0 && it + NSTAGE < nst) {
             mbar_expect_tx(&full[s], P1_STAGE_BYTES);
-            tma_load_1d(smraw + s * P1_STAGE_BYTES, jbytes + (size_t)(st0 + it + NSTAGE) * P1_STAGE_BYTES, P1_STAGE_BYTES, &full[s]);
-        }
-    }
-#pragma unroll
-    for (int p = 0; p < NPAIR1; ++p) {
-        const float2 nv = unpack2(no[p]);
-#pragma unroll
-        for (int h = 0; h < 2; ++h) {
-            const int n = itile * ITILE1 + (tid >> 5) * (32 * RI1) + (2 * p + h) * 32 + (tid & 31);
-            if (n < ni) {
-                P1Part out;
-                out.S = S[2 * p + h]; out.SU = SU[2 * p + h]; out.o = h ? -nv.y : -nv.x; out.pad = 0.0f;
-                part[(size_t)split * ni + n] = out;
-            }
+            tma_load_1d(smraw + s * P1_STAGE_BYTES, jrec + (size_t)(st0 + it + NSTAGE) * P1_STAGE, P1_STAGE_BYTES, &full[s]);
+        }
+    }
+#pragma unroll
+    for (int r = 0; r < RI1; ++r) {
+        const int n = itile * ITILE1 + (tid >> 5) * (32 * RI1) + r * 32 + (tid & 31);
+        if (n < ni) {
+            P1Part out;
+            out.S = S[r]; out.SU = SU[r]; out.o = -no[r]; out.pad = 0.0f;
+            part[(size_t)split * ni + n] = out;
         }
     }
 }
 
 __global__ void __launch_bounds__(THREADS)
 finalize1_kernel(const DevState* __restrict__ st, const double* __restrict__ sigma2_ptr, const double* __restrict__ w_ptr,
-                 const P1Part* __restrict__ part, const int* __restrict__ tile_slots, int n, const float4* __restrict__ tgtP,
-                 float4* __restrict__ tgtQ, long long npad, double* __restrict__ pt1, double* __restrict__ mom_part,
+                 const P1Part* __restrict__ part, const int* __restrict__ tile_slots, int n, float4* __restrict__ tgtP,
+                 float* __restrict__ tgtR, long long npad, double* __restrict__ pt1, double* __restrict__ mom_part,
                  const double* __restrict__ log2c_ptr ) {
     const int i = blockIdx.x * THREADS + threadIdx.x;
     double v[RM_TGT] = {0.0, 0.0};
@@ -645,7 +593,6 @@
             }
         }
         pt1[i] = p1n;
-        const float4 b = tgtP[i];
         float no = INFINITY, rnf = 0.0f;
         if (!dead) {
             const double rn = exp2(-(L + (double)omin));
@@ -654,22 +601,21 @@
             v[0] = SU * (double)rnf;
         }
         v[1] = p1n;
-        tgtQ[3 * (size_t)i] = make_float4(b.x, b.x, b.y, b.y);
-        tgtQ[3 * (size_t)i + 1] = make_float4(b.z, b.z, no, no);
-        tgtQ[3 * (size_t)i + 2] = make_float4(rnf, rnf, 0.f, 0.f);
+        tgtP[i].w = no;
+        tgtR[i] = rnf;
     } else if (i < npad) {
-        tgtQ[3 * (size_t)i] = make_float4(0.f, 0.f, 0.f, 0.f);
-        tgtQ[3 * (size_t)i + 1] = make_float4(0.f, 0.f, INFINITY, INFINITY);
-        tgtQ[3 * (size_t)i + 2] = make_float4(0.f, 0.f, 0.f, 0.f);
+        tgtP[i] = make_float4(0.f, 0.f, 0.f, INFINITY);
+        tgtR[i] = 0.0f;
     }
     block_reduce_store<RM_TGT>(v, mom_part + (size_t)blockIdx.x * RM_TGT);
 }
 
 template <bool CULL, bool WGT>
 __global__ void __launch_bounds__(THREADS, CPD_MINB2)
-pass2_kernel(const float4* __restrict__ ipts, int ni, const float4* __restrict__ jrec, const int4* __restrict__ work,
-             double* __restrict__ part , const float4* __restrict__ tbox ,
-             const float* __restrict__ omax_stage, const float4* __restrict__ tsub, const float* __restrict__ omax_sub) {
+pass2_kernel(const float4* __restrict__ ipts, int ni, const float4* __restrict__ jrec , const float* __restrict__ jrn ,
+             const int4* __restrict__ work, double* __restrict__ part ,
+             const float4* __restrict__ tbox , const float* __restrict__ omax_stage,
+             const float4* __restrict__ tsub, const float* __restrict__ omax_sub) {
     __shared__ float wbox[THREADS / 32][8];
     CPD_DYN_SMEM(smraw);
     uint64_t* full = reinterpret_cast<uint64_t*>(smraw + NSTAGE * P2_STAGE_BYTES);
@@ -677,37 +623,39 @@
     const int4 wk = work[blockIdx.x];
     const int itile = wk.x, st0 = wk.y, split = wk.w;
     const int nst = wk.z - wk.y;
-    const unsigned char* jbytes = reinterpret_cast<const unsigned char*>(jrec);
+    auto load_stage = [&](int slot, int stage) {
+        unsigned char* dst = smraw + slot * P2_STAGE_BYTES;
+        mbar_expect_tx(&full[slot], P2_STAGE_BYTES);
+        tma_load_1d(dst, jrec + (size_t)stage * P2_STAGE, P2_STAGE_PBYTES, &full[slot]);
+        tma_load_1d(dst + P2_STAGE_PBYTES, jrn + (size_t)stage * P2_STAGE, P2_STAGE_BYTES - P2_STAGE_PBYTES, &full[slot]);
+    };
     if (tid == 0) {
         for (int s = 0; s < NSTAGE; ++s) mbar_init(&full[s], 1);
         mbar_fence_init();
     }
     __syncthreads();
     if (tid == 0) {
-        for (int s = 0; s < NSTAGE && s < nst; ++s) {
-            mbar_expect_tx(&full[s], P2_STAGE_BYTES);
-            tma_load_1d(smraw + s * P2_STAGE_BYTES, jbytes + (size_t)(st0 + s) * P2_STAGE_BYTES, P2_STAGE_BYTES, &full[s]);
-        }
-    }
-    u64 ax[NPAIR2], ay[NPAIR2], az[NPAIR2], al[NPAIR2];
+        for (int s = 0; s < NSTAGE && s < nst; ++s) load_stage(s, st0 + s);
+    }
+    float ax[RI2], ay[RI2], az[RI2], al[RI2];
     double A1[RI2], AX[RI2], AY[RI2], AZ[RI2];
 #pragma unroll
-    for (int p = 0; p < NPAIR2; ++p) {
-        int m0 = itile * ITILE2 + (tid >> 5) * (32 * RI2) + (2 * p) * 32 + (tid & 31), m1 = m0 + 32;
+    for (int r = 0; r < RI2; ++r) {
+        int m0 = itile * ITILE2 + (tid >> 5) * (32 * RI2) + r * 32 + (tid & 31);
         m0 = m0 < ni ? m0 : ni - 1;
-        m1 = m1 < ni ? m1 : ni - 1;
-        const float4 p0 = ipts[m0], p1 = ipts[m1];
-        ax[p] = pack2(p0.x, p1.x); ay[p] = pack2(p0.y, p1.y); az[p] = pack2(p0.z, p1.z);
-        if (WGT) al[p] = pack2(p0.w, p1.w);
+        const float4 p0 = ipts[m0];
+        ax[r] = p0.x; ay[r] = p0.y; az[r] = p0.z;
+        al[r] = WGT ? p0.w : 0.0f;
     }
     float* const mybox = wbox[tid >> 5];
-    if (CULL) warp_bbox<NPAIR2>(ax, ay, az, mybox);
+    if (CULL) warp_bbox<RI2>(ax, ay, az, mybox);
 #pragma unroll
     for (int r = 0; r < RI2; ++r) { A1[r] = 0.0; AX[r] = 0.0; AY[r] = 0.0; AZ[r] = 0.0; }
     for (int it = 0; it < nst; ++it) {
         const int s = it % NSTAGE;
         mbar_wait(&full[s], (uint32_t)((it / NSTAGE) & 1));
-        const ulonglong2* sp = reinterpret_cast<const ulonglong2*>(smraw + s * P2_STAGE_BYTES);
+        const float4* sp = reinterpret_cast<const float4*>(smraw + s * P2_STAGE_BYTES);
+        const float* srn = reinterpret_cast<const float*>(smraw + s * P2_STAGE_BYTES + P2_STAGE_PBYTES);
         bool skip = false;
         if (CULL) {
             const float4 blo = tbox[2 * (st0 + it)], bhi = tbox[2 * (st0 + it) + 1];
@@ -719,74 +667,66 @@
                 const int sb = (st0 + it) * (P2_STAGE / SUB) + sc;
                 if (box_gap2(mybox, tsub[2 * sb], tsub[2 * sb + 1]) - omax_sub[sb] >= CULL_GAP) continue;
             }
-            const ulonglong2* q = sp + sc * (3 * SUB);
-            u64 s1[NPAIR2], sx[NPAIR2], sy[NPAIR2], sz[NPAIR2];
-#pragma unroll
-            for (int p = 0; p < NPAIR2; ++p) { s1[p] = 0ull; sx[p] = 0ull; sy[p] = 0ull; sz[p] = 0ull; }
+            const float4* q = sp + sc * SUB;
+            const float* qr = srn + sc * SUB;
+            float s1[RI2], sx[RI2], sy[RI2], sz[RI2];
+#pragma unroll
+            for (int r = 0; r < RI2; ++r) { s1[r] = 0.0f; sx[r] = 0.0f; sy[r] = 0.0f; sz[r] = 0.0f; }
             if (GRP > 0) {
 #pragma unroll 1
                 for (int g0 = 0; g0 < SUB; g0 += (GRP > 0 ? GRP : SUB)) {
-                    u64 g1[NPAIR2], gx[NPAIR2], gy[NPAIR2], gz[NPAIR2];
+                    float g1[RI2], gx[RI2], gy[RI2], gz[RI2];
 #pragma unroll
                     for (int jj = 0; jj < (GRP > 0 ? GRP : 1); ++jj) {
-                        const ulonglong2 bxy = q[3 * (g0 + jj)];
-                        const ulonglong2 bzo = q[3 * (g0 + jj) + 1];
-                        const u64 rn = q[3 * (g0 + jj) + 2].x;
-#pragma unroll
-                        for (int p = 0; p < NPAIR2; ++p) {
-                            const u64 dx = fsub2(ax[p], bxy.x), dy = fsub2(ay[p], bxy.y), dz = fsub2(az[p], bzo.x);
-                            u64 t = ffma2(dx, dx, bzo.y);
-                            t = ffma2(dy, dy, t);
-                            t = ffma2(dz, dz, t);
-                            if (WGT) t = fadd2(t, al[p]);
-                            const float2 tt = unpack2(t);
-                            const u64 pr = fmul2(pack2(ex2(-tt.x), ex2(-tt.y)), rn);
-                            g1[p] = jj == 0 ? pr : fadd2(g1[p], pr);
-                            gx[p] = jj == 0 ? fmul2(pr, dx) : ffma2(pr, dx, gx[p]);
-                            gy[p] = jj == 0 ? fmul2(pr, dy) : ffma2(pr, dy, gy[p]);
-                            gz[p] = jj == 0 ? fmul2(pr, dz) : ffma2(pr, dz, gz[p]);
+                        const float4 b = q[g0 + jj];
+                        const float rn = qr[g0 + jj];
+#pragma unroll
+                        for (int r = 0; r < RI2; ++r) {
+                            const float dx = sub_rn(ax[r], b.x), dy = sub_rn(ay[r], b.y), dz = sub_rn(az[r], b.z);
+                            float t = fma_rn(dx, dx, b.w);
+                            t = fma_rn(dy, dy, t);
+                            t = fma_rn(dz, dz, t);
+                            if (WGT) t = add_rn(t, al[r]);
+                            const float pr = mul_rn(ex2(-t), rn);
+                            g1[r] = jj == 0 ? pr : add_rn(g1[r], pr);
+                            gx[r] = jj == 0 ? mul_rn(pr, dx) : fma_rn(pr, dx, gx[r]);
+                            gy[r] = jj == 0 ? mul_rn(pr, dy) : fma_rn(pr, dy, gy[r]);
+                            gz[r] = jj == 0 ? mul_rn(pr, dz) : fma_rn(pr, dz, gz[r]);
                         }
                     }
 #pragma unroll
-                    for (int p = 0; p < NPAIR2; ++p) {
-                        s1[p] = fadd2(s1[p], g1[p]); sx[p] = fadd2(sx[p], gx[p]);
-                        sy[p] = fadd2(sy[p], gy[p]); sz[p] = fadd2(sz[p], gz[p]);
+                    for (int r = 0; r < RI2; ++r) {
+                        s1[r] = add_rn(s1[r], g1[r]); sx[r] = add_rn(sx[r], gx[r]);
+                        sy[r] = add_rn(sy[r], gy[r]); sz[r] = add_rn(sz[r], gz[r]);
                     }
                 }
             } else {
 #pragma unroll UNROLL2
                 for (int jj = 0; jj < SUB; ++jj) {
-                    const ulonglong2 bxy = q[3 * jj];
-                    const ulonglong2 bzo = q[3 * jj + 1];
-                    const u64 rn = q[3 * jj + 2].x;
-#pragma unroll
-                    for (int p = 0; p < NPAIR2; ++p) {
-                        const u64 dx = fsub2(ax[p], bxy.x), dy = fsub2(ay[p], bxy.y), dz = fsub2(az[p], bzo.x);
-                        u64 t = ffma2(dx, dx, bzo.y);
-                        t = ffma2(dy, dy, t);
-                        t = ffma2(dz, dz, t);
-                        if (WGT) t = fadd2(t, al[p]);
-                        const float2 tt = unpack2(t);
-                        const u64 pr = fmul2(pack2(ex2(-tt.x), ex2(-tt.y)), rn);
-                        s1[p] = fadd2(s1[p], pr);
-                        sx[p] = ffma2(pr, dx, sx[p]);
-                        sy[p] = ffma2(pr, dy, sy[p]);
-                        sz[p] = ffma2(pr, dz, sz[p]);
+                    const float4 b = q[jj];
+                    const float rn = qr[jj];
+#pragma unroll
+                    for (int r = 0; r < RI2; ++r) {
+                        const float dx = sub_rn(ax[r], b.x), dy = sub_rn(ay[r], b.y), dz = sub_rn(az[r], b.z);
+                        float t = fma_rn(dx, dx, b.w);
+                        t = fma_rn(dy, dy, t);
+                        t = fma_rn(dz, dz, t);
+                        if (WGT) t = add_rn(t, al[r]);
+                        const float pr = mul_rn(ex2(-t), rn);
+                        s1[r] = add_rn(s1[r], pr);
+                        sx[r] = fma_rn(pr, dx, sx[r]);
+                        sy[r] = fma_rn(pr, dy, sy[r]);
+                        sz[r] = fma_rn(pr, dz, sz[r]);
                     }
                 }
             }
 #pragma unroll
-            for (int p = 0; p < NPAIR2; ++p) {
-                const float2 v1 = unpack2(s1[p]), vx = unpack2(sx[p]), vy = unpack2(sy[p]), vz = unpack2(sz[p]);
-                A1[2 * p] += (double)v1.x; AX[2 * p] += (double)vx.x; AY[2 * p] += (double)vy.x; AZ[2 * p] += (double)vz.x;
-                A1[2 * p + 1] += (double)v1.y; AX[2 * p + 1] += (double)vx.y; AY[2 * p + 1] += (double)vy.y; AZ[2 * p + 1] += (double)vz.y;
+            for (int r = 0; r < RI2; ++r) {
+                A1[r] += (double)s1[r]; AX[r] += (double)sx[r]; AY[r] += (double)sy[r]; AZ[r] += (double)sz[r];
             }
         }
         __syncthreads();
-        if (tid == 0 && it + NSTAGE < nst) {
-            mbar_expect_tx(&full[s], P2_STAGE_BYTES);
-            tma_load_1d(smraw + s * P2_STAGE_BYTES, jbytes + (size_t)(st0 + it + NSTAGE) * P2_STAGE_BYTES, P2_STAGE_BYTES, &full[s]);
-        }
+        if (tid == 0 && it + NSTAGE < nst) load_stage(s, st0 + it + NSTAGE);
     }
 #pragma unroll
     for (int r = 0; r < RI2; ++r) {
```

Measured after the change: 111.6 (median of 6 runs). 1.06x the previous value.
